# ilya16/isp-tts

Hardware: AMD Instinct MI355X
Metric: mel-frames/s (whole node), batch=64 x 512-frame utterances per GPU, full forward incl. MAS (higher is better)
Workload: dtype bf16; 1 GPU; BASELINE config 3: AcousticModel.forward (TextEncoder + Aligner/MAS + TemporalAdaptor 1 flow eval + MelDecoder + to_mel), fixed-length synthetic random-phoneme batch, random-init weights of the recipe architecture (23.2 M params); batch_per_gpu=64, global_batch=64, text_len=100, mel_len=512, parallelism=single GPU, device=gfx950:sramecc+:xnack-, compute_units=256, launch=HIP graph replay, batches_in_flight=1

## Files before the change

include/ispk.h:

```cpp
#ifndef ISPK_H
#define ISPK_H

#include <stdint.h>

#ifdef __cplusplus
extern "C" {
#endif

typedef struct ihipStream_t* ispk_stream_t;

#define ISPK_ABI_VERSION 2

#define ISPK_E_NULL (-1)
#define ISPK_E_SHAPE (-2)
#define ISPK_E_ALIGN (-3)
#define ISPK_E_UNSUPPORTED (-4)

int32_t ispk_abi_version(void);
const char* ispk_last_error_string(void);
int32_t ispk_device_info(char* name, int32_t cap);

int32_t ispk_mas_f32(const float* logits, const int64_t* text_len, const int64_t* mel_len, int16_t* attn_hard,
                     int64_t* dur, int16_t* path, int32_t B, int32_t M_max, int32_t L_max, int64_t stride_b,
                     int64_t stride_m, ispk_stream_t stream);

int32_t ispk_layernorm_f32(const float* x, int64_t ldx, const float* gamma, const float* beta, const float* ada_scale,
                           const float* ada_shift, int64_t ada_stride, int32_t rows_per_batch,
                           const uint8_t* row_mask, float* y, int64_t ldy, int32_t rows, int32_t D, float eps,
                           ispk_stream_t stream);
int32_t ispk_layernorm_f32_bf16(const float* x, int64_t ldx, const float* gamma, const float* beta,
                                const float* ada_scale, const float* ada_shift, int64_t ada_stride,
                                int32_t rows_per_batch, const uint8_t* row_mask, uint16_t* y, int64_t ldy, int32_t rows,
                                int32_t D, float eps, ispk_stream_t stream);

#define ISPK_EP_GELU 1u
#define ISPK_EP_SILU 2u
#define ISPK_EP_MASK_ACC 4u
#define ISPK_EP_MASK_OUT 8u
#define ISPK_EP_BIAS_ROW 16u
#define ISPK_EP_MASK_COL 32u
#define ISPK_EP_OUT_BF16 64u
#define ISPK_EP_RESID_BF16 128u
#define ISPK_EP_DUAL_GELU 1024u
#define ISPK_EP_GELU_BWD 2048u
#define ISPK_EP_OUT_SPLIT 512u
#define ISPK_EP_ROWS_T 256u

int32_t ispk_gemm_f32_tile(int32_t M, int32_t N, int32_t K);
int32_t ispk_gemm_f32(const float* A, int64_t lda, const float* W, int64_t ldw, float* C, int64_t ldc, const float* bias,
                      const float* resid, int64_t ldr, const uint8_t* mask, int32_t M, int32_t N, int32_t K,
                      uint32_t flags, int32_t cols_per_batch, int64_t batch_stride, ispk_stream_t stream);
int32_t ispk_gemm_f32_batched(const float* A, int64_t lda, int64_t stride_a, const float* W, int64_t ldw, int64_t stride_w,
                              float* C, int64_t ldc, int64_t stride_c, int32_t batch, int32_t M, int32_t N, int32_t K,
                              ispk_stream_t stream);
int32_t ispk_gemm_bf16_gelu_train(const uint16_t* A, int64_t lda, const uint16_t* W, int64_t ldw, uint16_t* u, int64_t ldu,
                                  uint16_t* a, int64_t ld_a, int32_t M, int32_t N, int32_t K, float dropout_p, uint64_t seed,
                                  ispk_stream_t stream);
int32_t ispk_gemm_bf16_gelu_bwd(const uint16_t* dY, int64_t lddy, const uint16_t* W2t, int64_t ldw, const uint16_t* u,
                                int64_t ldu, uint16_t* du, int64_t lddu, const uint8_t* row_mask, int32_t M, int32_t N,
                                int32_t K, float dropout_p, uint64_t seed, ispk_stream_t stream);
int32_t ispk_gemm_bf16_last_variant(void);
int32_t ispk_gemm_bf16(const uint16_t* A, int64_t lda, const uint16_t* W, int64_t ldw, void* C, int64_t ldc,
                       const float* bias, const void* resid, int64_t ldr, const uint8_t* mask, int32_t M, int32_t N,
                       int32_t K, uint32_t flags, int32_t cols_per_batch, int64_t batch_stride, ispk_stream_t stream);
int32_t ispk_gemm_bf16_splitk_plan(int32_t M, int32_t N, int32_t K, uint32_t flags);
int32_t ispk_gemm_bf16_splitk(const uint16_t* A, int64_t lda, const uint16_t* W, int64_t ldw, void* C, int64_t ldc,
                              const float* bias, const void* resid, int64_t ldr, const uint8_t* mask, int32_t M, int32_t N,
                              int32_t K, uint32_t flags, float* workspace, int32_t ksplit, ispk_stream_t stream);

int32_t ispk_ffn_bf16(const uint16_t* x, int64_t ldx, const uint16_t* W1, int64_t ldw1, const float* bias1,
                      const uint16_t* W2, int64_t ldw2, const float* bias2, const float* resid, int64_t ldr,
                      const uint8_t* mask, float* out, int64_t ldo, int32_t rows, int32_t dim, int32_t inner, uint32_t flags,
                      ispk_stream_t stream);

int32_t ispk_ffn_bf16_prenorm(const float* x, int64_t ldx, const float* norm_gamma, const float* norm_beta, float norm_eps,
                              const uint16_t* W1, int64_t ldw1, const uint16_t* W2_packed, const float* bias2,
                              const uint8_t* mask, float* out, int64_t ldo, int32_t rows, int32_t dim, int32_t inner,
                              uint32_t flags, float* row_stats, float stats_eps, ispk_stream_t stream);

int32_t ispk_ffn_chunk_w2_bf16(const uint16_t* W2, int64_t ldw2, int32_t dim, int32_t inner, uint16_t* out,
                               ispk_stream_t stream);
int32_t ispk_ffn_bf16_prenorm2_split(const float* x, int64_t ldx, const float* norm_gamma, const float* norm_beta,
                                     float norm_eps, const uint16_t* W1, const uint16_t* W2_chunks, float* parts,
                                     int64_t part_stride, int32_t splits, int32_t rows, int32_t dim, int32_t inner,
                                     ispk_stream_t stream);
int32_t ispk_ffn_combine_ln_f32(const float* x, int64_t ldx, const float* parts, int64_t part_stride, int32_t splits,
                                const uint8_t* mask, float* y, int64_t ldy, const float* ln_gamma, const float* ln_beta,
                                float ln_eps, int32_t ln_mask, void* ln_out, int64_t ld_ln, int32_t ln_bf16, int32_t rows,
                                int32_t dim, ispk_stream_t stream);
int32_t ispk_ffn_bf16_prenorm2(const float* x, int64_t ldx, const float* norm_gamma, const float* norm_beta, float norm_eps,
                               const uint16_t* W1, const uint16_t* W2_chunks, const uint8_t* mask, float* out, int64_t ldo,
                               int32_t rows, int32_t dim, int32_t inner, uint32_t flags, float* row_stats, float stats_eps,
                               ispk_stream_t stream);
int32_t ispk_attn_out_ffn_bf16(const float* x, int64_t ldx, const uint16_t* attn_out, int64_t ld_attn,
                               const uint16_t* Wo_chunks, const float* norm_gamma, const float* norm_beta, float norm_eps,
                               const uint16_t* W1, const uint16_t* W2_chunks, const uint8_t* mask, float* out, int64_t ldo,
                               int32_t rows, int32_t dim, int32_t inner, uint32_t flags, float* row_stats, float stats_eps,
                               ispk_stream_t stream);

int32_t ispk_attn_out_ffn_norm_bf16(const float* x, int64_t ldx, const uint16_t* attn_out, int64_t ld_attn,
                                    const uint16_t* Wo_chunks, const float* norm_gamma, const float* norm_beta, float norm_eps,
                                    const uint16_t* W1, const uint16_t* W2_chunks, const uint8_t* mask, float* out, int64_t ldo,
                                    int32_t rows, int32_t dim, int32_t inner, uint32_t flags, const float* final_gamma,
                                    const float* final_beta, float final_eps, int32_t ln_mask, void* ln_out, int64_t ld_ln,
                                    int32_t ln_bf16, ispk_stream_t stream);
int32_t ispk_attn_out_ffn_split_bf16(const float* x, int64_t ldx, const uint16_t* attn_out, int64_t ld_attn,
                                     const uint16_t* Wo_chunks, const float* norm_gamma, const float* norm_beta, float norm_eps,
                                     const uint16_t* W1, const uint16_t* W2_chunks, const uint8_t* mask, uint32_t flags,
                                     float* parts, int64_t part_stride, int32_t splits, int32_t rows, int32_t dim, int32_t inner,
                                     ispk_stream_t stream);
int32_t ispk_chunk_k16_bf16(const uint16_t* W, int64_t ldw, int32_t N, int32_t K, uint16_t* out, ispk_stream_t stream);
int32_t ispk_attn_out_ffn_qkv_bf16(const float* x, int64_t ldx, const uint16_t* attn_out, int64_t ld_attn,
                                   const uint16_t* Wo_chunks, const float* norm_gamma, const float* norm_beta, float norm_eps,
                                   const uint16_t* W1, const uint16_t* W2_chunks, const uint8_t* mask, float* out, int64_t ldo,
                                   int32_t rows, int32_t dim, int32_t inner, uint32_t flags, const float* next_gamma,
                                   const float* next_beta, float next_eps, const uint16_t* Wqkv_chunks, uint16_t* qkv,
                                   int64_t ld_qkv, ispk_stream_t stream);

int32_t ispk_gemm_bf16_lnin(const float* x, int64_t ldx, const float* row_stats, const float* ln_gamma, const float* ln_beta,
                            float ln_eps, const uint16_t* W, int64_t ldw, void* C, int64_t ldc, const float* bias, const void* resid,
                            int64_t ldr, const uint8_t* mask, int32_t M, int32_t N, int32_t K, uint32_t flags,
                            ispk_stream_t stream);

int32_t ispk_ffn_pack_w2_bf16(const uint16_t* W2, int64_t ldw2, int32_t dim, int32_t inner, uint16_t* packed,
                              ispk_stream_t stream);

int32_t ispk_linear_small_f32(const float* a, int64_t lda, const float* w, int64_t ldw, const float* bias,
                              const float* resid, int64_t ldr, float* out, int64_t ldo, int32_t M, int32_t N, int32_t K,
                              uint32_t act, ispk_stream_t stream);

int32_t ispk_alibi_mqa_attn_f32(const float* q, int64_t ldq, const float* k, const float* v, int64_t ldkv,
                                const float* slopes, const int64_t* key_len, float* out, int64_t ldo, int32_t B,
                                int32_t N, int32_t H, ispk_stream_t stream);
int32_t ispk_alibi_mqa_attn_bf16(const uint16_t* q, int64_t ldq, const uint16_t* k, const uint16_t* v, int64_t ldkv,
                                 const float* slopes, const int64_t* key_len, uint16_t* out, int64_t ldo, int32_t B,
                                 int32_t N, int32_t H, ispk_stream_t stream);
int32_t ispk_alibi_mqa_attn_bf16_tiles(const uint16_t* q, int64_t ldq, const uint16_t* k, const uint16_t* v, int64_t ldkv,
                                       const float* slopes, const int64_t* key_len, uint16_t* out, int64_t ldo, int32_t B,
                                       int32_t N, int32_t H, int32_t q_tiles_per_workgroup, ispk_stream_t stream);

int32_t ispk_attn_block_short_bf16(const uint16_t* x, int64_t ldx, const uint16_t* Wqkv_chunks, uint16_t* qkv, int64_t ld_qkv,
                                   const float* slopes, const int64_t* key_len, const uint16_t* Wo_chunks, const float* resid,
                                   int64_t ldr, const uint8_t* mask, float* out, int64_t ldo, int32_t B, int32_t N, int32_t H,
                                   ispk_stream_t stream);

int32_t ispk_pad_rows_f32(const float* x, int64_t stride_b, int64_t stride_t, int64_t stride_c, const int64_t* len,
                          void* out, int32_t out_bf16, int32_t B, int32_t T, int32_t C, ispk_stream_t stream);
int32_t ispk_masked_instnorm_f32(const float* y, const float* weight, const float* bias, const int64_t* len, void* out,
                                 int32_t out_bf16, int32_t B, int32_t T, int32_t C, float eps, ispk_stream_t stream);
int32_t ispk_aligner_scores_f32(const float* q_enc, int64_t q_stride_b, const float* k_enc, int64_t k_stride_b,
                                const int64_t* text_len, const int64_t* mel_len, float* attn_logits, float* attn_soft,
                                int32_t B, int32_t M, int32_t L, int32_t D, ispk_stream_t stream);
int32_t ispk_aligner_scores_fast_f32(const float* q_enc, int64_t q_stride_b, const float* k_enc, int64_t k_stride_b,
                                const int64_t* text_len, const int64_t* mel_len, float* attn_logits, float* attn_soft,
                                int32_t B, int32_t M, int32_t L, int32_t D, ispk_stream_t stream);
int32_t ispk_soft_average_f32(const float* attn_soft, const float* pitch, const float* energy, const int64_t* duration,
                              const int64_t* text_len, float* feats, int32_t B, int32_t M, int32_t L,
                              ispk_stream_t stream);

int32_t ispk_flow_head_f32(const float* y, int64_t ldy, const float* norm_gamma, const float* norm_beta, float norm_eps,
                           const float* W, const float* bias, const float* flow, const float* x0, const uint8_t* mask,
                           float* pred, float* duration, float* loss_ratio, float* loss_mean, float* workspace, int32_t B,
                           int32_t L, int32_t D, int32_t C, ispk_stream_t stream);
int32_t ispk_flow_euler_f32(const float* x_t, const float* velocity, float dt, const uint8_t* mask, float* out, int32_t B,
                            int32_t L, int32_t C, ispk_stream_t stream);
int32_t ispk_infer_features_f32(const float* pred, const float* duration_target_f32, const int64_t* duration_target_i64,
                                const float* pitch_target, const float* energy_target, float duration_factor, float pitch_factor,
                                float pitch_delta, float energy_factor, float energy_delta, float* duration, float* features,
                                int32_t B, int32_t L, ispk_stream_t stream);
int32_t ispk_infer_features_round_f32(const float* pred, const float* duration_target_f32, const int64_t* duration_target_i64,
                                      const float* pitch_target, const float* energy_target, float duration_factor,
                                      float pitch_factor, float pitch_delta, float energy_factor, float energy_delta,
                                      float* duration, float* features, int32_t B, int32_t L, ispk_stream_t stream);
int32_t ispk_infer_features_items_f32(const float* pred, const float* duration_target_f32, const int64_t* duration_target_i64,
                                      const float* pitch_target, const float* energy_target, const float* controls,
                                      int32_t round, float* duration, float* features, int64_t* frames_wanted, int32_t B,
                                      int32_t L, ispk_stream_t stream);
int32_t ispk_infer_features_tokens_f32(const float* pred, const float* duration_target_f32, const int64_t* duration_target_i64,
                                       const float* pitch_target, const float* energy_target, const float* controls,
                                       int32_t round, float* duration, float* features, int64_t* frames_wanted, int32_t B,
                                       int32_t L, ispk_stream_t stream);
int32_t ispk_flow_mix_f32(const float* x0, const float* x1, const float* t, float sigma, float* x_t, float* flow, int32_t B,
                          int32_t L, int32_t C, ispk_stream_t stream);
int32_t ispk_flow_finish_f32(const float* pred_raw, const float* flow, const float* x0, const uint8_t* mask, float* pred,
                             float* duration, float* loss_ratio, float* loss_mean, int32_t B, int32_t L, int32_t C,
                             ispk_stream_t stream);

int32_t ispk_embed_tokens_f32(const int64_t* text, const float* table, int64_t ld_table, int32_t vocab,
                              const int64_t* text_len, float* emb, uint8_t* mask, int32_t B, int32_t L, int32_t D,
                              ispk_stream_t stream);
int32_t ispk_embed_tokens_qkv(const int64_t* text, const float* table, int64_t ld_table, int32_t vocab, const int64_t* text_len,
                              float* emb, uint8_t* mask, const uint16_t* qkv_table, int64_t ld_qkv_table, uint16_t* qkv,
                              int32_t B, int32_t L, int32_t D, int32_t N, ispk_stream_t stream);
int32_t ispk_add_speaker_f32(float* x, const float* table, int64_t ld_table, int32_t speakers, const int64_t* speaker,
                             int32_t id_stride, int32_t B, int32_t L, int32_t D, ispk_stream_t stream);
int32_t ispk_add_speaker_out_f32(const float* x, float* out, const float* table, int64_t ld_table, int32_t speakers,
                                 const int64_t* speaker, int32_t id_stride, int32_t B, int32_t L, int32_t D, ispk_stream_t stream);
int32_t ispk_speaker_grad_f32(const float* d_x, const int64_t* speaker, int32_t id_stride, const int64_t* text_len,
                              float* workspace, int64_t workspace_floats, float* d_table, int64_t ld_table, int32_t speakers,
                              int32_t B, int32_t L, int32_t D, int32_t accumulate, ispk_stream_t stream);
int32_t ispk_time_embedding_f32(const float* t, int32_t n, const float* inv_freq, const float* freq_scale, int32_t half_dim,
                                const float* w0, const float* b0, const float* w1, const float* b1, int32_t emb_dim,
                                float* out, ispk_stream_t stream);
int32_t ispk_length_regulate_f32(const float* alignment, const float* dur_f32, const int64_t* dur_i64, const int64_t* enc_len,
                                 const float* x, int64_t ldx, float* out, int64_t* dec_len, uint8_t* dec_mask, int32_t B,
                                 int32_t M, int32_t L, int32_t D, int32_t max_len, int32_t dur_cols, ispk_stream_t stream);
int32_t ispk_length_regulate_split_bf16(const float* alignment, const float* dur_f32, const int64_t* dur_i64, const int64_t* enc_len,
                                 const float* x, int64_t ldx, float* out, int64_t* dec_len, uint8_t* dec_mask, int32_t B,
                                 int32_t M, int32_t L, int32_t D, int32_t max_len, int32_t dur_cols, ispk_stream_t stream);
int32_t ispk_length_regulate_qkv_bf16(const float* alignment, const float* dur_f32, const int64_t* dur_i64, const int64_t* enc_len,
                                      const float* x, int64_t ldx, float* out, int64_t* dec_len, uint8_t* dec_mask,
                                      const float* norm_gamma, const float* norm_beta, float norm_eps, const uint16_t* Wqkv_chunks,
                                      uint16_t* qkv, int64_t ld_qkv, int32_t B, int32_t M, int32_t L, int32_t D, int32_t max_len,
                                      int32_t dur_cols, ispk_stream_t stream);
int32_t ispk_length_regulate_split_f16(const float* alignment, const float* dur_f32, const int64_t* dur_i64, const int64_t* enc_len,
                                const float* x, int64_t ldx, float* out, int64_t* dec_len, uint8_t* dec_mask, int32_t B,
                                int32_t M, int32_t L, int32_t D, int32_t max_len, int32_t dur_cols, ispk_stream_t stream);

int32_t ispk_hard_regulate_f32(const float* dur_f32, const int64_t* dur_i64, const float* x, int64_t ldx, float* out,
                               int64_t* dec_len, uint8_t* dec_mask, int32_t B, int32_t frames, int32_t L, int32_t D,
                               int32_t max_len, ispk_stream_t stream);
int32_t ispk_hard_regulate_bwd_f32(const float* dur_f32, const int64_t* dur_i64, const float* d_out, float* d_x, int32_t B,
                                   int32_t rows, int32_t L, int32_t D, int32_t max_len, ispk_stream_t stream);
int32_t ispk_hard_average_f32(const float* pitch, const float* energy, const int64_t* duration, const int64_t* text_len,
                              float* feats, int32_t B, int32_t M, int32_t L, ispk_stream_t stream);

int32_t ispk_transpose_f32(const float* x, int64_t ldx, float* y, int64_t ldy, int32_t rows, int32_t cols,
                           ispk_stream_t stream);
int32_t ispk_gemm_tn_f32(const float* A, int64_t lda, const float* B, int64_t ldb, float* C, int64_t ldc, int32_t M,
                         int32_t N1, int32_t N2, const uint8_t* row_mask, int32_t accumulate, float* workspace,
                         int64_t workspace_floats, ispk_stream_t stream);
int32_t ispk_gemm_tn_bf16(const float* A, int64_t lda, const float* B, int64_t ldb, float* C, int64_t ldc, int32_t M,
                          int32_t N1, int32_t N2, const uint8_t* row_mask, int32_t accumulate, float* workspace,
                          int64_t workspace_floats, ispk_stream_t stream);
int32_t ispk_gemm_tn_b16(const uint16_t* A, int64_t lda, const uint16_t* B, int64_t ldb, float* C, int64_t ldc, int32_t M,
                         int32_t N1, int32_t N2, const uint8_t* row_mask, int32_t accumulate, float* workspace,
                         int64_t workspace_floats, ispk_stream_t stream);
int32_t ispk_gemm_tn_last_plan(int32_t* splits, int32_t* rows_per_split);
int32_t ispk_gemm_tn_batched_f32(const float* A, int64_t lda, int64_t stride_a, const float* B, int64_t ldb, int64_t stride_b,
                                 float* C, int64_t ldc, int64_t stride_c, int32_t batch, int32_t M, int32_t N1, int32_t N2,
                                 const uint8_t* row_mask, int32_t accumulate, float* workspace, int64_t workspace_floats,
                                 ispk_stream_t stream);
int32_t ispk_layernorm_bwd_f32(const float* x, int64_t ldx, const float* dy, int64_t lddy, const float* gamma,
                               const uint8_t* row_mask, float* dx, int64_t lddx, int32_t add_to_dx, float* dgamma,
                               float* dbeta, float* workspace, int64_t workspace_floats, int64_t rows, int32_t dim,
                               float eps, ispk_stream_t stream);
int32_t ispk_layernorm_bwd_dual_f32(const float* x, int64_t ldx, const float* dy, int64_t lddy, const float* gamma,
                                    const uint8_t* row_mask, float* dx, int64_t lddx, int32_t add_to_dx, float* dgamma,
                                    float* dbeta, float* workspace, int64_t workspace_floats, int64_t rows, int32_t dim,
                                    float eps, uint16_t* dx_bf16, int64_t ld_dx_bf16, ispk_stream_t stream);
int32_t ispk_gelu_f32(const float* u, float* a, int64_t n, float dropout_p, uint64_t seed, ispk_stream_t stream);
int32_t ispk_gelu_bwd_f32(const float* da, const float* u, float* du, int64_t n, float dropout_p, uint64_t seed,
                          ispk_stream_t stream);
int32_t ispk_gelu_f32_bf16(const float* u, uint16_t* a, int64_t n, float dropout_p, uint64_t seed, ispk_stream_t stream);
int32_t ispk_gelu_bwd_bf16(const uint16_t* da, const float* u, uint16_t* du, int64_t n, float dropout_p, uint64_t seed,
                           ispk_stream_t stream);
int32_t ispk_gelu_bf16(const uint16_t* u, uint16_t* a, int64_t n, float dropout_p, uint64_t seed, ispk_stream_t stream);
int32_t ispk_gelu_bwd_b16(const uint16_t* da, const uint16_t* u, uint16_t* du, int64_t n, float dropout_p, uint64_t seed,
                          ispk_stream_t stream);
int32_t ispk_dropout_mask_u8(uint8_t* out, int64_t n, float dropout_p, uint64_t seed, ispk_stream_t stream);
int32_t ispk_alibi_mqa_attn_train_f32(const float* qkv, int64_t ld_qkv, const float* slopes, const int64_t* key_len, float* o,
                                      int64_t ld_o, float* lse, int32_t B, int32_t N, int32_t H, float dropout_p, uint64_t seed,
                                      ispk_stream_t stream);
int32_t ispk_alibi_mqa_attn_bwd_f32(const float* qkv, int64_t ld_qkv, const float* o, const float* d_o, int64_t ld_o,
                                    const float* slopes, const int64_t* key_len, float* dqkv, float* dlogslopes,
                                    float* workspace, int64_t workspace_floats, int32_t B, int32_t N, int32_t H,
                                    const float* lse_in, float dropout_p, uint64_t seed, ispk_stream_t stream);
int32_t ispk_alibi_mqa_attn_train_bf16(const uint16_t* qkv, int64_t ld_qkv, const float* slopes, const int64_t* key_len,
                                       uint16_t* o, int64_t ld_o, float* lse, int32_t B, int32_t N, int32_t H, float dropout_p,
                                       uint64_t seed, ispk_stream_t stream);
int32_t ispk_alibi_mqa_attn_bwd_bf16(const uint16_t* qkv, int64_t ld_qkv, const uint16_t* o, const uint16_t* d_o, int64_t ld_o,
                                     const float* slopes, const int64_t* key_len, const float* lse, uint16_t* dqkv,
                                     float* dlogslopes, float* workspace, int64_t workspace_floats, int32_t B, int32_t N,
                                     int32_t H, float dropout_p, uint64_t seed, ispk_stream_t stream);
int32_t ispk_mel_loss_f32(const float* mel_out, const float* mel_target, const int64_t* mel_len, float* ratio, float* loss,
                          float* grad, float grad_out, int32_t B, int32_t C, int32_t T, ispk_stream_t stream);
int32_t ispk_acoustic_metrics_f32(const float* mel_out, int64_t out_sb, int64_t out_sc, int64_t out_st, const float* mel_target,
                                  int64_t tgt_sb, int64_t tgt_sc, int64_t tgt_st, const int64_t* mel_len, const int64_t* text_len,
                                  const float* attn_soft, int64_t attn_sb, int64_t attn_st, const float* dct, float* workspace,
                                  int64_t workspace_floats, float* out, int32_t B, int32_t C, int32_t T, int32_t L,
                                  int32_t n_mfcc, ispk_stream_t stream);
int32_t ispk_dtw_f32(const float* cost, int64_t cost_sb, int64_t cost_sn, const int64_t* n_len, const int64_t* m_len,
                     float* total, int32_t* steps, int16_t* path, float* workspace, int64_t workspace_floats, int32_t B,
                     int32_t N, int32_t M, ispk_stream_t stream);
int32_t ispk_mcd_dtw_f32(const float* mel_out, int64_t out_sb, int64_t out_sc, int64_t out_st, const float* mel_target,
                         int64_t tgt_sb, int64_t tgt_sc, int64_t tgt_st, const float* dct, const int64_t* n_len,
                         const int64_t* m_len, const float* pitch_out, int64_t pitch_out_sb, const float* pitch_target,
                         int64_t pitch_target_sb, float* workspace, int64_t workspace_floats, float* per_item, float* means,
                         float* cost_out, int32_t B, int32_t C, int32_t N, int32_t M, int32_t n_mfcc, ispk_stream_t stream);
int32_t ispk_audio_features_f32(const float* audio, int64_t ld_audio, const int64_t* audio_len, const float* tables,
                                int64_t table_floats, const int32_t* fb_index, int32_t n_mels, float* mel, int64_t* mel_len, float* pitch, float* energy,
                                int32_t B, int32_t S, int32_t M, int32_t tau_min, int32_t tau_max, float sample_rate,
                                float threshold, float pitch_mean, float pitch_std, ispk_stream_t stream);
int32_t ispk_resample_f32(const float* audio, int64_t ld_b, int64_t ld_c, const int64_t* audio_len, const float* taps,
                          int64_t tap_floats, const int32_t* first, float* out, int64_t ld_out, int64_t* out_len, int32_t B,
                          int32_t C, int32_t S, int32_t S_out, int32_t orig, int32_t dest, int32_t width, int32_t T,
                          ispk_stream_t stream);
int32_t ispk_feature_stats_f64(const float* pitch, int64_t ld_pitch, const float* energy, int64_t ld_energy,
                               const int64_t* mel_len, double* partial, double* state, int32_t B, int32_t M, int32_t reset,
                               ispk_stream_t stream);
int32_t ispk_audio_measure_f64(const float* audio, int64_t ld_audio, const int64_t* audio_len, const double* table,
                               int64_t table_doubles, int64_t* bounds, double* loudness, float* peak, float* gain,
                               float* workspace, int64_t workspace_floats, int32_t B, int32_t S, int32_t sample_rate,
                               int32_t trim_mode, double trim_threshold, int32_t pad_frames, int32_t gain_mode,
                               double target_lufs, double peak_limit, ispk_stream_t stream);
int32_t ispk_audio_apply_f32(const float* audio, int64_t ld_audio, const int64_t* bounds, const float* gain, float* out,
                             int64_t ld_out, int64_t* out_len, int32_t B, int32_t S, int32_t S_out, ispk_stream_t stream);
int32_t ispk_pcm16(const float* audio, int64_t ld_audio, const int64_t* audio_len, int16_t* out, int64_t ld_out, int32_t B,
                   int32_t S, int32_t dither, uint64_t seed, ispk_stream_t stream);
int32_t ispk_vocoder_unfold(const void* mel, int32_t mel_f16, int64_t sb, int64_t sc, int64_t st, const int64_t* mel_len,
                            void* rows, int32_t rows_bf16, int64_t ldr, uint8_t* row_mask, int32_t B, int32_t C, int32_t T,
                            int32_t K, ispk_stream_t stream);
int32_t ispk_dwconv7_ln_f32(const float* x, int64_t ldx, const float* w, const float* bias, const float* gamma,
                            const float* beta, float eps, const int64_t* mel_len, void* y, int32_t y_bf16, int64_t ldy,
                            int32_t B, int32_t T, int32_t D, ispk_stream_t stream);
int32_t ispk_istft_head_f32(const float* h, int64_t ldh, const int64_t* mel_len, const float* tables, int64_t table_floats,
                            float* audio, int64_t ld_audio, int64_t* audio_len, int32_t B, int32_t T, int32_t S,
                            ispk_stream_t stream);
int32_t ispk_aligner_scores_bwd_f32(const float* attn_logits, const float* attn_soft, const float* d_soft, const float* d_logits,
                                    const int64_t* text_len, const int64_t* mel_len, float* dS, int64_t ld_s, float* dSt,
                                    int64_t ld_t, int32_t B, int32_t M, int32_t L, float scale, ispk_stream_t stream);
int32_t ispk_masked_instnorm_bwd_f32(const float* y, const float* d_out, const float* weight, const int64_t* lengths, float* d_y,
                                     float* d_weight, float* d_bias, float* workspace, int64_t workspace_floats, int32_t B,
                                     int32_t T, int32_t C, float eps, ispk_stream_t stream);
int32_t ispk_soft_average_bwd_f32(const float* attn_soft, const float* pitch, const float* energy, const float* d_feats,
                                  const int64_t* text_len, float* workspace, int64_t workspace_floats, float* d_attn,
                                  int32_t accumulate, int32_t B, int32_t M, int32_t L, ispk_stream_t stream);
int32_t ispk_flow_loss_bwd_f32(const float* pred_raw, const float* flow, const uint8_t* mask, float grad_out, float* d_raw, int32_t B,
                               int32_t L, int32_t C, ispk_stream_t stream);
int32_t ispk_adaln_bwd_f32(const float* x, int64_t ldx, const float* dy, int64_t lddy, const float* scale, int64_t ld_scale,
                           const uint8_t* row_mask, float* dx, int64_t lddx, int32_t add_to_dx, float* dscale, float* dshift,
                           int64_t ld_out, int32_t B, int32_t rows_per_batch, int32_t dim, float eps, ispk_stream_t stream);
int32_t ispk_time_embedding_bwd_f32(const float* t, int32_t n, const float* inv_freq, const float* freq_scale, int32_t half_dim,
                                    const float* w0, const float* b0, const float* w1, int32_t emb_dim, const float* d_out,
                                    float* dw0, float* db0, float* dw1, float* db1, ispk_stream_t stream);
int32_t ispk_attn_ctc_loss_f32(const float* attn_logits, const int64_t* text_len, const int64_t* mel_len, float blank_logprob,
                               float* workspace, int64_t workspace_floats, float* loss, float* grad, float grad_out, int32_t B,
                               int32_t M, int32_t L, ispk_stream_t stream);
int32_t ispk_attn_bin_loss_f32(const float* attn_soft, const int16_t* attn_hard, float eps, float* workspace, float* loss,
                               float* grad, float grad_out, int32_t B, int32_t M, int32_t L, ispk_stream_t stream);
int32_t ispk_mel_grad_rows_f32(const float* dmel, const uint8_t* mask, float* g, int32_t B, int32_t C, int32_t T,
                               ispk_stream_t stream);
int32_t ispk_colsum_f32(const float* x, int64_t ldx, int64_t rows, int32_t cols, const uint8_t* row_mask, float* workspace,
                        int64_t workspace_floats, float* out, ispk_stream_t stream);
int32_t ispk_smallk_wgrad_f32(const float* g, int64_t ldg, const float* x, int64_t ldx, int64_t rows, int32_t N, int32_t K,
                              float* workspace, int64_t workspace_floats, float* out, ispk_stream_t stream);
int32_t ispk_embedding_bwd_f32(const int64_t* ids, const float* d_emb, int64_t rows, int32_t dim, int32_t vocab,
                               int32_t padding_idx, float* d_table, int64_t ld_table, ispk_stream_t stream);
int32_t ispk_grad_sqnorm_f32(const float* g, int64_t n, float* partial, float* out, ispk_stream_t stream);
int32_t ispk_adamw_f32(float* p, const float* g, float* m, float* v, int64_t n, int64_t n_decay, float lr, float beta1,
                       float beta2, float eps, float weight_decay, int32_t step, const float* grad_sqnorm, float max_norm,
                       float grad_scale, ispk_stream_t stream);

int32_t ispk_split_f16(const float* x, int64_t ldx, uint16_t* hi, uint16_t* lo, int64_t ldy, int32_t rows, int32_t cols,
                       ispk_stream_t stream);
int32_t ispk_gemm_split_f16_tile(int32_t M, int32_t N, int32_t K);
int32_t ispk_gemm_split_f16(const uint16_t* A, int64_t lda, int64_t a_plane, const uint16_t* W, int64_t ldw, int64_t w_plane,
                            void* C, int64_t ldc, int64_t c_plane, const float* bias, const float* resid, int64_t ldr,
                            const uint8_t* mask, int32_t M, int32_t N, int32_t K, uint32_t flags, int32_t cols_per_batch,
                            int64_t batch_stride, ispk_stream_t stream);
int32_t ispk_layernorm_f32_split(const float* x, int64_t ldx, const float* gamma, const float* beta, const float* ada_scale,
                                 const float* ada_shift, int64_t ada_stride, int32_t rows_per_batch, const uint8_t* row_mask,
                                 uint16_t* y_hi, int64_t ldy, int64_t y_plane, int32_t rows, int32_t D, float eps,
                                 ispk_stream_t stream);
int32_t ispk_alibi_mqa_attn_split_f16(const float* q, int64_t ldq, const float* k, const float* v, int64_t ldkv,
                                      const float* slopes, const int64_t* key_len, void* out, int64_t ldo, int64_t o_plane,
                                      int32_t B, int32_t N, int32_t H, ispk_stream_t stream);

int32_t ispk_cast_f32_bf16(const float* x, int64_t ldx, uint16_t* y, int64_t ldy, int32_t rows, int32_t cols,
                           ispk_stream_t stream);

typedef struct { float f[10]; } ispk_adam_args_t;
int32_t ispk_set_dropout_seed_source(const uint64_t* device_word);
int32_t ispk_adam_args_f32(float lr, float beta1, float beta2, float eps, float weight_decay, int32_t step, float max_norm,
                           float grad_scale, ispk_adam_args_t* out);
int32_t ispk_adamw_f32_dev(float* p, const float* g, float* m, float* v, int64_t n, int64_t n_decay,
                           const ispk_adam_args_t* args_dev, const float* grad_sqnorm, ispk_stream_t stream);

typedef struct { const float* src; void* dst; int32_t rows, cols; int64_t ld_dst; int32_t flags; } ispk_stage_t;
int32_t ispk_stage_weights(const ispk_stage_t* segs, int32_t nseg, ispk_stream_t stream);
typedef struct { const float* src; void* dst; int64_t n; int32_t mode; } ispk_segment_t;
int32_t ispk_segments_f32(const ispk_segment_t* segs, int32_t nseg, ispk_stream_t stream);
int32_t ispk_fill_zero(void* p, int64_t bytes, ispk_stream_t stream);
int32_t ispk_scale_f32(float* x, int64_t n, const float* s_dev, float s_host, ispk_stream_t stream);
int32_t ispk_sum_scalars_f32(const float* const* terms, const float* weights, int32_t n, float* out, ispk_stream_t stream);
int32_t ispk_exp_pad_f32(const float* src, float* dst, int32_t n, int32_t total, ispk_stream_t stream);
int32_t ispk_sqrt_scale_f32(const float* src, float* dst, int32_t n, float scale, ispk_stream_t stream);
int32_t ispk_copy2d_f32(const float* src, int64_t ld_src, float* dst, int64_t ld_dst, int32_t rows, int32_t cols,
                        ispk_stream_t stream);
int32_t ispk_permute021_f32(const float* src, float* dst, int32_t A, int32_t B, int32_t C, ispk_stream_t stream);
int32_t ispk_conv_weight_flip_f32(const float* w, float* wf, int32_t O, int32_t C, int32_t K, ispk_stream_t stream);

int32_t ispk_hifigan_tile_rows(void);
int32_t ispk_hifigan_conv_f32(const float* x, int64_t ldx, const float* w, const float* bias, const float* resid, int64_t ldr,
                              float* out, int64_t ldo, const int64_t* len, int32_t len_mul, int32_t B, int32_t T, int32_t C_in,
                              int32_t C_out, int32_t k, int32_t dilation, float slope, float scale, int32_t accumulate,
                              ispk_stream_t stream);
int32_t ispk_hifigan_conv_bf16(const float* x, int64_t ldx, const uint16_t* w, const float* bias, const float* resid,
                               int64_t ldr, float* out, int64_t ldo, const int64_t* len, int32_t len_mul, int32_t B, int32_t T,
                               int32_t C_in, int32_t C_out, int32_t k, int32_t dilation, float slope, float scale,
                               int32_t accumulate, ispk_stream_t stream);
int32_t ispk_hifigan_upsample_f32(const float* x, int64_t ldx, const float* w, const float* bias, float* out, int64_t ldo,
                                  const int64_t* len, int32_t len_mul, int32_t B, int32_t T, int32_t C_in, int32_t C_out,
                                  int32_t k, int32_t stride, float slope, ispk_stream_t stream);
int32_t ispk_hifigan_upsample_bf16(const float* x, int64_t ldx, const uint16_t* w, const float* bias, float* out, int64_t ldo,
                                   const int64_t* len, int32_t len_mul, int32_t B, int32_t T, int32_t C_in, int32_t C_out,
                                   int32_t k, int32_t stride, float slope, ispk_stream_t stream);
int32_t ispk_hifigan_post_f32(const float* x, int64_t ldx, const float* w, const float* bias, const int64_t* len,
                              int32_t len_mul, float* audio, int64_t ld_audio, int64_t* audio_len, int32_t B, int32_t T,
                              int32_t S, int32_t C, float slope, ispk_stream_t stream);
int32_t ispk_hifigan_post_clamp_f32(const float* x, int64_t ldx, const float* w, const float* bias, const int64_t* len,
                                    int32_t len_mul, float* audio, int64_t ld_audio, int64_t* audio_len, int32_t B, int32_t T,
                                    int32_t S, int32_t C, float slope, ispk_stream_t stream);

int32_t ispk_istftnet_tile_frames(void);
int32_t ispk_istftnet_head_f32(const float* x, int64_t ldx, const float* w, const float* bias, const float* table,
                               int32_t table_floats, const int64_t* len, int32_t len_mul, float* audio, int64_t ld_audio,
                               int64_t* audio_len, int32_t B, int32_t T, int32_t S, int32_t C, int32_t n_fft, int32_t hop,
                               float slope, float phase_scale, ispk_stream_t stream);

int32_t ispk_snake_aa_tile_rows(void);
int32_t ispk_snake_aa_f32(const float* x, int64_t ldx, const float* al, const float* inv_b, const float* taps, float* out,
                          int64_t ldo, const int64_t* len, int32_t len_mul, int32_t B, int32_t T, int32_t C,
                          ispk_stream_t stream);

int32_t ispk_denoise_tile_samples(void);
int32_t ispk_denoise_f32(const float* audio, int64_t ld_audio, const int64_t* audio_len, const float* tables,
                         const float* bias, const float* strength_item, float strength, float* out, int64_t ld_out, int32_t B,
                         int32_t S, ispk_stream_t stream);

int32_t ispk_join_tile_samples(void);
int32_t ispk_join_plan_bytes(void);
int32_t ispk_join_plan(const int64_t* audio_len, const int64_t* doc, const int64_t* pos, const int64_t* pause,
                       const int64_t* bounds, void* plan, int64_t plan_bytes, int64_t* item_offset, int64_t* item_len,
                       int64_t* doc_len, int64_t* wanted_len, int32_t B, int32_t S, int32_t D, int32_t S_out, int32_t fade,
                       ispk_stream_t stream);
int32_t ispk_join_f32(const float* audio, int64_t ld_audio, const float* gain, const void* plan, const int64_t* doc_len,
                      float* out, int64_t ld_out, int32_t B, int32_t S, int32_t D, int32_t S_out, ispk_stream_t stream);

int32_t ispk_speech_marks(const float* duration, int64_t ld_duration, const int64_t* text_len, const int64_t* audio_len,
                          const int64_t* bounds, const int64_t* item_offset, const int64_t* doc, const int64_t* doc_len,
                          const int64_t* doc_bounds, const int64_t* word_id, int64_t* token_marks, int64_t* word_marks,
                          int32_t hop, int32_t round, int32_t B, int32_t L, int32_t S, int32_t D, int32_t W,
                          ispk_stream_t stream);

int32_t ispk_gain_envelope_tile_samples(void);
int32_t ispk_gain_envelope_f32(const float* audio, int64_t ld_audio, const int64_t* audio_len, const int64_t* token_marks,
                               const float* token_gain, int32_t ramp, float* out, int64_t ld_out, int32_t B, int32_t L,
                               int32_t S, ispk_stream_t stream);

int32_t ispk_limit_tile_samples(void);
int32_t ispk_limit_f32(const float* audio, int64_t ld_audio, const int64_t* audio_len, const int64_t* bounds, const float* gain,
                       const float* taps, float ceiling, int32_t lookahead, float* out, int64_t ld_out, int64_t* out_len,
                       float* true_peak, float* reduction, int32_t B, int32_t S, ispk_stream_t stream);

int32_t ispk_equalize_segment_samples(void);
int32_t ispk_equalize_f32(const float* audio, int64_t ld_audio, const int64_t* audio_len, const double* table,
                          int64_t table_doubles, int32_t sections, float* out, int64_t ld_out, int64_t* out_len,
                          double* workspace, int64_t workspace_doubles, int32_t B, int32_t S, ispk_stream_t stream);

int32_t ispk_segment_workspace_bytes(int32_t B, int32_t S, int64_t* bytes);
int32_t ispk_segment_plan(const float* audio, int64_t ld_audio, const int64_t* audio_len, double factor, int32_t ref_mode,
                          double ref, int32_t pad, int32_t min_silence_frames, int64_t target_samples, int64_t max_samples,
                          int64_t min_samples, int64_t* segments, int32_t* flags, int32_t* count, int32_t* wanted,
                          int32_t* frames, int32_t* speech_frames, double* speech_power, double* noise_power, void* workspace,
                          int64_t workspace_bytes, int32_t B, int32_t S, int32_t K, ispk_stream_t stream);
int32_t ispk_segment_gather_f32(const float* audio, int64_t ld_audio, const int64_t* segments, const int32_t* flags,
                                const int32_t* count, int32_t drop, float* out, int64_t ld_out, int64_t* out_len, int32_t* item,
                                int32_t* index, int64_t* bounds, int32_t* row_flags, int32_t* rows, int32_t* rows_wanted,
                                int32_t B, int32_t S, int32_t K, int32_t R, int32_t S_out, ispk_stream_t stream);

int32_t ispk_screen_tile_samples(void);
int32_t ispk_screen_workspace_bytes(int32_t B, int32_t S, int64_t* bytes);
int32_t ispk_screen_f64(const float* audio, int64_t ld_audio, const int64_t* audio_len, const float* tables, int32_t parts,
                        int32_t rail_mode, float rail, float rail_ratio, int32_t min_run, int32_t min_dropout, double band_factor,
                        int32_t min_band_bin, double max_dc, double min_peak, int32_t* nonfinite, float* peak, double* dc,
                        double* power, int32_t* clip_runs, int64_t* clip_samples, int64_t* clip_longest, int64_t* clip_first,
                        int32_t* dropout_runs, int64_t* dropout_samples, int64_t* dropout_longest, double* ltas, int32_t* band_bin,
                        int32_t* flags, void* workspace, int64_t workspace_bytes, int32_t B, int32_t S, ispk_stream_t stream);

int32_t ispk_declip_max_unknowns(void);
int32_t ispk_declip_workspace_bytes(int32_t B, int32_t S, int64_t* bytes);
int32_t ispk_declip_f64(const float* audio, int64_t ld_audio, const int64_t* audio_len, const int32_t* in_flags, int32_t rail_mode,
                        float rail, float rail_ratio, int32_t min_run, int32_t order, int32_t iterations, float* out, int64_t ld_out,
                        int64_t* out_len, float* thr, float* peak, int64_t* clip_samples, int64_t* restored, int32_t* windows,
                        int32_t* dense, int32_t* flags, void* workspace, int64_t workspace_bytes, int32_t B, int32_t S,
                        ispk_stream_t stream);

int32_t ispk_noise_tile_samples(void);
int32_t ispk_noise_workspace_bytes(int32_t B, int32_t S, int64_t* bytes);
int32_t ispk_noise_profile_f64(const float* audio, int64_t ld_audio, const int64_t* audio_len, const float* tables, double factor,
                               int32_t ref_mode, double ref, int32_t guard, int32_t min_noise_frames, double* noise,
                               int32_t* noise_frames, int32_t* frames, int32_t* flags, void* workspace, int64_t workspace_bytes,
                               int32_t B, int32_t S, ispk_stream_t stream);
int32_t ispk_noise_reduce_f32(const float* audio, int64_t ld_audio, const int64_t* audio_len, const float* tables,
                              const double* noise, int32_t P, const int32_t* index, const int32_t* flags, double over,
                              double g_min, int32_t smooth_frames, int32_t smooth_bins, float* out, int64_t ld_out, int32_t B,
                              int32_t S, ispk_stream_t stream);

int32_t ispk_stretch_tile_samples(void);
int32_t ispk_stretch_workspace_bytes(int32_t B, int32_t S, int32_t out_samples, int64_t* bytes);
int32_t ispk_stretch_f32(const float* audio, int64_t ld_audio, const int64_t* audio_len, const float* tables, double rate,
                         const double* rates, float* out, int64_t ld_out, int32_t out_samples, int64_t* out_len, int64_t* wanted,
                         int32_t* flags, void* workspace, int64_t workspace_bytes, int32_t B, int32_t S, ispk_stream_t stream);

#define ISPK_PYIN_THRESHOLDS 100
#define ISPK_PYIN_MAX_BINS 1024
#define ISPK_PYIN_TABLE_DOUBLES 1326
int32_t ispk_pyin_frames_per_block(void);
int32_t ispk_pyin_workspace_bytes(int32_t B, int32_t M, int32_t NB, int64_t* bytes);
int32_t ispk_pyin_observe_f32(const float* audio, int64_t ld_audio, const int64_t* audio_len, const float* tables,
                              const double* prior, float* obs, int64_t* frames, int32_t B, int32_t S, int32_t M, int32_t NB,
                              int32_t min_period, int32_t max_period, double sample_rate, double f_min,
                              int32_t bins_per_semitone, ispk_stream_t stream);
int32_t ispk_pyin_decode_f64(const void* obs, int32_t obs_is_log, const int64_t* obs_len, const double* trans, int32_t width,
                             double f_min, int32_t bins_per_semitone, float pitch_mean, float pitch_std, int32_t* state,
                             float* f0, int32_t* voiced, float* voiced_prob, float* pitch, int64_t* frames, double* log_prob,
                             void* workspace, int64_t workspace_bytes, int32_t B, int32_t M, int32_t NB, ispk_stream_t stream);

#define ISPK_GRIFFINLIM_STEP 0
#define ISPK_GRIFFINLIM_INIT 1
int32_t ispk_griffinlim_tile_samples(void);
int32_t ispk_mel_to_linear_f32(const void* mel, int32_t mel_f16, int64_t mel_sb, int64_t mel_sc, int64_t mel_st,
                               const int64_t* mel_len, const float* pinv_t, float* mag, int64_t ld_mag, int32_t B,
                               int32_t n_mels, int32_t T, ispk_stream_t stream);
int32_t ispk_griffinlim_step_f32(const float* audio, int64_t ld_audio, const float* mag, int64_t ld_mag,
                                 const int64_t* mel_len, const float* tables, float* out, int64_t ld_out, int64_t* audio_len,
                                 int32_t B, int32_t T, int32_t mode, uint64_t seed, ispk_stream_t stream);
int32_t ispk_griffinlim_fast_step_f32(const float* audio, int64_t ld_audio, const float* prev, int64_t ld_prev, float alpha,
                                      const float* mag, int64_t ld_mag, const int64_t* mel_len, const float* tables,
                                      float* out, int64_t ld_out, int64_t* audio_len, int32_t B, int32_t T, ispk_stream_t stream);
int32_t ispk_griffinlim_error_f32(const float* audio, int64_t ld_audio, const float* mag, int64_t ld_mag,
                                  const int64_t* mel_len, const float* tables, float* work, int64_t ld_work, float* err,
                                  int32_t B, int32_t T, ispk_stream_t stream);

#ifdef __cplusplus
}
#endif
#endif
```

isp_tts_amd/acoustic/alignment.py:

```python
from __future__ import annotations

from collections.abc import Sequence
from typing import NamedTuple, Optional

import torch
import torch.nn as nn
from torch import Tensor

from .. import runtime
from ..staging import StagedWeights
from ..modules.aligner import mas_device
from ..modules.constructor import Constructor


_NOT_A_PATH = ("{} only owns parameters (the reference's state_dict names); its arithmetic runs inside the fused HIP "
               "kernels that ConvAttention launches (csrc/aligner.hip) - there is no PyTorch/MIOpen path to fall back to")


class MaskedInstanceNorm1d(nn.Module):

    def __init__(self, num_features: int, eps: float = 1e-5):
        super().__init__()
        self.eps = eps
        self.weight = nn.Parameter(torch.ones(num_features))
        self.bias = nn.Parameter(torch.zeros(num_features))

    def forward(self, *args, **kwargs):
        raise NotImplementedError(_NOT_A_PATH.format("MaskedInstanceNorm1d"))


class ConvBlock1D(nn.Module):

    def __init__(self, in_channels: int, out_channels: int, kernel_size: int = 1, activation: str = "relu",
                 normalization: Optional[str] = "batch", bias: bool = True):
        super().__init__()
        if normalization not in (None, "instance"):
            raise NotImplementedError("only instance normalisation (the recipes' choice) is built")
        if activation not in ("gelu", "linear"):
            raise NotImplementedError("only gelu / linear activations (the recipes' choice) are built")
        self.conv = nn.Conv1d(in_channels, out_channels, kernel_size=kernel_size, padding=(kernel_size - 1) // 2,
                              bias=bias and normalization is None)
        self.gelu = activation == "gelu"
        self.norm = MaskedInstanceNorm1d(out_channels) if normalization is not None else None

    def forward(self, *args, **kwargs):
        raise NotImplementedError(_NOT_A_PATH.format("ConvBlock1D"))


class ConvAttention(nn.Module, Constructor):
    def __init__(self, mel_dim: int, text_dim: int = 512, attention_dim: int = 80, key_kernel_size: int = 3,
                 query_kernel_size=(3, 3), dropout: float = 0.0, normalization: Optional[str] = "instance",
                 activation: str = "relu", attention_prior: bool = True):
        super().__init__()
        self.mel_dim, self.text_dim = mel_dim, text_dim
        self.scale = attention_dim ** -0.5
        if isinstance(query_kernel_size, int):
            query_kernel_size = [query_kernel_size] * 2
        self.key_proj = nn.ModuleList([
            ConvBlock1D(text_dim, text_dim * 2, key_kernel_size, activation, normalization, bias=False),
            ConvBlock1D(text_dim * 2, attention_dim, 1, "linear", None, bias=False)])
        self.query_proj = nn.ModuleList([
            ConvBlock1D(mel_dim, mel_dim * 2, query_kernel_size[0], activation, normalization, bias=False),
            ConvBlock1D(mel_dim * 2, mel_dim, query_kernel_size[1], activation, normalization, bias=False),
            ConvBlock1D(mel_dim, attention_dim, 1, "linear", None, bias=False)])
        self.attention_prior = attention_prior
        self.compute_dtype = torch.float32
        self._cache = StagedWeights()

    def _staged(self):
        ps = [c.conv.weight for c in list(self.key_proj) + list(self.query_proj)]
        dt = self.compute_dtype

        def build():
            if dt == torch.float16:
                w2d = [runtime.split_f16(p.detach().permute(0, 2, 1).reshape(p.shape[0], -1).float().contiguous()) for p in ps]
            else:
                w2d = [p.detach().permute(0, 2, 1).reshape(p.shape[0], -1).to(dt).contiguous() for p in ps]
            return w2d[:2], w2d[2:]
        return self._cache.get(dt, ps, build)

    def project_queries(self, queries: Tensor, query_len: Tensor) -> Tensor:
        _, wq = self._staged()
        gelu, dt = runtime.EP_GELU, self.compute_dtype
        if dt == torch.float16:
            q = runtime.pad_rows(queries.float(), query_len, channel_first=True, out_dtype=dt)
            for i in (0, 1):
                q = runtime.conv5_padded_split(q, wq[i], gelu)
                q = runtime.masked_instnorm(q, self.query_proj[i].norm.weight, self.query_proj[i].norm.bias, query_len,
                                            out_dtype=dt)
            return runtime.conv5_padded_split(q, wq[2])
        q = runtime.pad_rows(queries.float(), query_len, channel_first=True, out_dtype=dt)
        q = runtime.conv5_padded(q, wq[0], gelu)
        q = runtime.masked_instnorm(q, self.query_proj[0].norm.weight, self.query_proj[0].norm.bias, query_len,
                                    out_dtype=dt)
        q = runtime.conv5_padded(q, wq[1], gelu)
        q = runtime.masked_instnorm(q, self.query_proj[1].norm.weight, self.query_proj[1].norm.bias, query_len,
                                    out_dtype=dt)
        return runtime.conv5_padded(q, wq[2])

    def forward(self, queries: Tensor, keys: Tensor, query_len: Tensor, key_len: Tensor, q_proj: Optional[Tensor] = None):
        if not self.attention_prior:
            raise NotImplementedError("the aligner is built with its diagonal prior (recipes: attention_prior default)")
        wk, _ = self._staged()
        max_q, max_k = queries.shape[2], keys.shape[2]
        gelu, dt = runtime.EP_GELU, self.compute_dtype
        if dt == torch.float16:
            k = runtime.pad_rows(keys.float(), key_len, channel_first=True, out_dtype=dt)
            k = runtime.conv5_padded_split(k, wk[0], gelu)
            k = runtime.masked_instnorm(k, self.key_proj[0].norm.weight, self.key_proj[0].norm.bias, key_len, out_dtype=dt)
            k = runtime.conv5_padded_split(k, wk[1])
            q = q_proj if q_proj is not None else self.project_queries(queries, query_len)
            return runtime.aligner_scores(q, k, key_len, query_len, max_q, max_k)
        k = runtime.pad_rows(keys.float(), key_len, channel_first=True, out_dtype=dt)
        k = runtime.conv5_padded(k, wk[0], gelu)
        k = runtime.masked_instnorm(k, self.key_proj[0].norm.weight, self.key_proj[0].norm.bias, key_len, out_dtype=dt)
        k = runtime.conv5_padded(k, wk[1])
        q = q_proj if q_proj is not None else self.project_queries(queries, query_len)
        return runtime.aligner_scores(q, k, key_len, query_len, max_q, max_k, fast=dt == torch.bfloat16)


class AlignerOutput(NamedTuple):
    attn_soft: Tensor
    attn_logits: Tensor
    attn_hard: Tensor
    attn_hard_duration: Tensor


class Aligner(nn.Module, Constructor):
    def __init__(self, mel_dim: int, text_dim: int = 512, attention_dim: int = 80, key_kernel_size: int = 3,
                 query_kernel_size=(3, 3), dropout: float = 0.0, normalization: Optional[str] = "instance",
                 activation: str = "relu", attention_prior: bool = True):
        super().__init__()
        self.attention = ConvAttention(mel_dim=mel_dim, text_dim=text_dim, attention_dim=attention_dim,
                                       key_kernel_size=key_kernel_size, query_kernel_size=query_kernel_size,
                                       dropout=dropout, normalization=normalization, activation=activation,
                                       attention_prior=attention_prior)

    def forward(self, mel: Tensor, enc_text: Tensor, mel_len: Tensor, text_len: Tensor,
                q_proj: Optional[Tensor] = None, mas_stream=None) -> AlignerOutput:
        attn_soft, attn_logits = self.attention(mel, enc_text, mel_len, text_len, q_proj=q_proj)
        if mas_stream is not None and attn_logits.is_cuda:
            mas_stream.wait_stream(torch.cuda.current_stream())
            with torch.cuda.stream(mas_stream):
                attn_hard, dur = self.binarize_attention_parallel(attn_logits, text_len, mel_len, return_duration=True)
            attn_logits.record_stream(mas_stream)
        else:
            attn_hard, dur = self.binarize_attention_parallel(attn_logits, text_len, mel_len, return_duration=True)
        return AlignerOutput(attn_soft=attn_soft, attn_logits=attn_logits, attn_hard=attn_hard, attn_hard_duration=dur)

    @torch.no_grad()
    def binarize_attention_parallel(self, attn_logits: Tensor, text_len: Tensor, mel_len: Tensor,
                                    return_duration: bool = False):
        hard, dur, _ = mas_device(attn_logits.detach(), text_len, mel_len, want_dur=return_duration)
        return (hard, dur) if return_duration else hard
```

isp_tts_amd/acoustic/model.py:

```python
from __future__ import annotations

import warnings
from typing import NamedTuple, Optional

import torch
import torch.nn as nn
import torch.nn.functional as F
from torch import Tensor

from .. import runtime
from ..staging import StagedWeights
from ..modules.constructor import Constructor
from ..modules.transformer import Transformer
from ..modules.transformer.plan import Hand, Handed
from ..utils import get_mask_from_lengths
from .alignment import Aligner, AlignerOutput
from .temporal_adaptor import FlowTemporalAdaptor, TemporalAdaptorOutput


class AcousticModelOutput(NamedTuple):
    mel: Tensor
    adaptor_output: TemporalAdaptorOutput
    aligner_output: AlignerOutput
    loss: Optional[Tensor] = None
    losses: Optional[dict] = None


class AcousticModel(nn.Module, Constructor):
    def __init__(self, encoding_map: dict, mel_dim: int, text_dim: int = 384, encoder=None, decoder=None,
                 temporal_adaptor=None, aligner=None, num_speakers: Optional[int] = 0, pitch_mean=None, pitch_std=None,
                 speaker_in_forward: bool = False):
        super().__init__()
        self.encoding_map = dict(encoding_map)
        self.mel_dim, self.text_dim = mel_dim, text_dim
        self.text_embedding = nn.Embedding(len(encoding_map), text_dim, padding_idx=0)
        self.encoder = Transformer.init(encoder, emb_dim=text_dim)
        enc_dim = self.encoder.dim
        self.aligner = Aligner.init(aligner, mel_dim=mel_dim, text_dim=enc_dim)
        self.speaker_embedding = None
        if (num_speakers or 0) > 0:
            self.speaker_embedding = nn.Embedding(num_speakers, enc_dim)
            nn.init.xavier_uniform_(self.speaker_embedding.weight)
        self.speaker_in_forward = bool(speaker_in_forward)
        self.train_amp: Optional[bool] = None
        self.temporal_adaptor = FlowTemporalAdaptor.init(temporal_adaptor, encoder_dim=enc_dim)
        self.decoder = Transformer.init(decoder, emb_dim=enc_dim)
        self.to_mel = nn.Linear(self.decoder.dim, mel_dim)
        self.token_qkv_table = True
        self.overlap_streams = True
        self._side_streams: dict = {}
        self.register_buffer("pitch_mean", torch.tensor(float(pitch_mean or 0.)))
        self.register_buffer("pitch_std", torch.tensor(float(pitch_std or 1.)))
        self.compute_dtype = torch.float32
        self._cache = StagedWeights()

    def set_compute_dtype(self, dtype: torch.dtype, *, alignment_dtype: Optional[torch.dtype] = None):
        chain = alignment_dtype if alignment_dtype is not None else dtype
        assert chain in (torch.float32, torch.bfloat16, torch.float16)
        self.encoder.set_compute_dtype(chain)
        self.decoder.set_compute_dtype(dtype)
        self.temporal_adaptor.predictor.transformer.set_compute_dtype(dtype)
        self.temporal_adaptor.embedding.transformer.set_compute_dtype(dtype)
        self.aligner.attention.compute_dtype = chain
        self.temporal_adaptor.length_regulator.split_bf16 = (True if dtype == torch.bfloat16 else
                                                             "f16" if dtype == torch.float16 else False)
        self.compute_dtype = dtype
        return self

    def _to_mel(self, dec_out: Tensor, dec_mask: Optional[Tensor]) -> Tensor:
        w = self.to_mel.weight
        if dec_out.dtype == torch.float16:
            ws = self._cache.get(torch.float16, (w,), lambda: runtime.split_f16(w.detach().float().contiguous()))
            return runtime.to_mel_split(dec_out, ws, self.to_mel.bias, dec_mask)
        if dec_out.dtype == torch.bfloat16:
            w = self._cache.get(torch.bfloat16, (w,), lambda: w.detach().to(torch.bfloat16).contiguous())
        return runtime.to_mel(dec_out, w, self.to_mel.bias, dec_mask)

    def _embed(self, text: Tensor, text_len: Optional[Tensor], want_mask: bool = True):
        table, enc = self.text_embedding.weight, self.encoder
        first = enc.layers[0]
        norm, att = first.attention_norm, first.attention
        if not (self.token_qkv_table and text.is_cuda and att.compute_dtype == torch.bfloat16 and not first.adaptive_norm
                and norm.weight is not None and norm.bias is not None and isinstance(enc.project_emb, nn.Identity)
                and (att.heads * 64 + 128) % 8 == 0):
            return (*runtime.embed_tokens(text, table, text_len, want_mask=want_mask), Handed())

        def build():
            with torch.no_grad():
                rows = runtime.layernorm(table.detach().float().contiguous(), norm.weight, norm.bias, eps=norm.eps,
                                         out_dtype=torch.bfloat16)
                return runtime.gemm(rows, att._staged(torch.bfloat16)[0])
        qkv_table = self._cache.get("token_qkv", (table, norm.weight, norm.bias, att.to_q.weight, att.to_kv.weight), build)
        emb, mask, qkv = runtime.embed_tokens_qkv(text, table, qkv_table, text_len, want_mask=want_mask)
        return emb, mask, Handed(Hand.QKV, qkv)

    def _decoder_first(self):
        dec = self.decoder
        first = dec.layers[0]
        norm, att = first.attention_norm, first.attention
        ok = (att.compute_dtype == torch.bfloat16 and not first.adaptive_norm and norm.weight is not None and norm.bias is not None
              and isinstance(dec.project_emb, nn.Identity) and dec.dim == 384 and att.heads * 64 + 128 == 512)
        return first if ok else None

    def _decoder_handed(self) -> Handed:
        qkv = self.temporal_adaptor.length_regulator.qkv
        return Handed(Hand.QKV, qkv) if qkv is not None else Handed()

    def forward(self, text: Tensor, text_len: Tensor, mel: Tensor, mel_len: Tensor, pitch: Optional[Tensor] = None,
                energy: Optional[Tensor] = None, speaker: Optional[Tensor] = None, sigma: float = 0., steps: int = 1, *,
                flow_noise: Optional[Tensor] = None, flow_time: Optional[Tensor] = None) -> AcousticModelOutput:
        if self.speaker_embedding is None:
            speaker = None
        elif not self.speaker_in_forward:
            raise AttributeError(f"'{type(self).__name__}' object has no attribute 'speaker_encoder'")
        elif speaker is None:
            raise ValueError("speaker_in_forward is on and the model has a speaker table: forward() needs `speaker` "
                             "([B, 1] int64 ids, or a single id for the whole batch)")
        if torch.is_grad_enabled() and text.is_cuda and any(p.requires_grad for p in self.parameters()):
            from ..train.model import acoustic_train_outputs
            amp = self.train_amp if self.train_amp is not None else torch.is_autocast_enabled("cuda")
            train_aligner = any(p.requires_grad for p in self.aligner.parameters())
            with torch.autocast("cuda", enabled=False):
                return acoustic_train_outputs(self, text, text_len, mel, mel_len, pitch, energy, flow_noise, flow_time, amp=amp,
                                              train_aligner=train_aligner, speaker=speaker)
        with torch.no_grad():
            return self._forward_values(text, text_len, mel, mel_len, pitch, energy, flow_noise=flow_noise, flow_time=flow_time,
                                        speaker=speaker)

    def _forward_values(self, text: Tensor, text_len: Tensor, mel: Tensor, mel_len: Tensor, pitch: Optional[Tensor] = None,
                        energy: Optional[Tensor] = None, *, flow_noise: Optional[Tensor] = None,
                        flow_time: Optional[Tensor] = None, speaker: Optional[Tensor] = None) -> AcousticModelOutput:
        q_proj = None
        if mel.is_cuda and self.overlap_streams:
            main = torch.cuda.current_stream()
            side = self._side_streams.setdefault(mel.device, torch.cuda.Stream(device=mel.device))
            side.wait_stream(main)
            with torch.cuda.stream(side):
                q_proj = self.aligner.attention.project_queries(mel, mel_len)
        token_emb, enc_mask, handed = self._embed(text, text_len)
        enc_out = self.encoder(token_emb, mask=enc_mask, key_len=text_len, handed=handed).out
        if q_proj is not None:
            main.wait_stream(side)
            q_proj.record_stream(main)
        branch = side if q_proj is not None else None
        hard = not self.temporal_adaptor.soft_duration
        aligner_output = self.aligner(mel=mel, enc_text=enc_out.transpose(1, 2).detach(), mel_len=mel_len,
                                      text_len=text_len, q_proj=q_proj, mas_stream=None if hard else branch)
        if speaker is not None:
            enc_out = runtime.add_speaker(enc_out, self.speaker_embedding.weight, speaker)
        adaptor_output = self.temporal_adaptor(
            enc_out=enc_out, enc_mask=enc_mask, max_dec_len=mel.size(2),
            duration_target=aligner_output.attn_hard_duration, alignment=aligner_output.attn_soft,
            pitch_target_dense=pitch, energy_target_dense=energy, noise=flow_noise, time_steps=flow_time,
            enc_len=text_len, predictor_stream=branch, duration_sum=mel_len if branch is not None and not hard else None,
            qkv_for=self._decoder_first())
        dec_len = adaptor_output.dec_lengths
        dec_mask = adaptor_output.dec_mask
        dec_out = self.decoder(adaptor_output.enc_out, mask=dec_mask, key_len=dec_len, out_dtype=self.compute_dtype,
                               handed=self._decoder_handed()).out
        mel_out = self._to_mel(dec_out, dec_mask)
        if q_proj is not None:
            main.wait_stream(side)
            for t in (adaptor_output.log_duration, adaptor_output.duration, adaptor_output.pitch, adaptor_output.energy,
                      aligner_output.attn_hard, aligner_output.attn_hard_duration, *(adaptor_output.losses or {}).values()):
                if isinstance(t, Tensor):
                    t.record_stream(main)
        return AcousticModelOutput(mel=mel_out, adaptor_output=adaptor_output, aligner_output=aligner_output)

    @torch.no_grad()
    def forward_front(self, text: Tensor, text_len: Tensor, mel: Tensor, mel_len: Tensor, pitch: Tensor, energy: Tensor):
        main = torch.cuda.current_stream()
        side = self._side_streams.setdefault(mel.device, torch.cuda.Stream(device=mel.device))
        side.wait_stream(main)
        with torch.cuda.stream(side):
            q_proj = self.aligner.attention.project_queries(mel, mel_len)
        token_emb, enc_mask, handed = self._embed(text, text_len)
        enc_out = self.encoder(token_emb, mask=enc_mask, key_len=text_len, handed=handed).out
        main.wait_stream(side)
        q_proj.record_stream(main)
        attn_soft, attn_logits = self.aligner.attention(mel, enc_out.transpose(1, 2).detach(), mel_len, text_len,
                                                        q_proj=q_proj)
        feats = runtime.soft_average(attn_soft, pitch, energy, None, text_len)
        return {"enc_out": enc_out, "enc_mask": enc_mask, "attn_soft": attn_soft, "attn_logits": attn_logits, "feats": feats}

    @torch.no_grad()
    def forward_side(self, st: dict, text_len: Tensor, mel_len: Tensor, pitch: Tensor, energy: Tensor,
                     flow_noise: Optional[Tensor], flow_time: Optional[Tensor]):
        attn_hard, dur = self.aligner.binarize_attention_parallel(st["attn_logits"], text_len, mel_len, return_duration=True)
        ad = self.temporal_adaptor
        targets = runtime.soft_average(st["attn_soft"], pitch, energy, dur, text_len)
        pred, losses = ad.predictor(st["enc_out"], targets, st["enc_mask"][..., None], noise=flow_noise, time_steps=flow_time,
                                    key_len=text_len)
        return {"attn_hard": attn_hard, "dur": dur, "pred": pred, "losses": losses,
                "duration_pred": ad.predictor._duration_estimate}

    @torch.no_grad()
    def forward_back(self, st: dict, text_len: Tensor, mel_len: Tensor, max_dec_len: int):
        ad = self.temporal_adaptor
        feats = st["feats"]
        x = ad.embedding(feats[..., 1:3], mask=st["enc_mask"][..., None], key_len=text_len, residual=st["enc_out"])
        dec_in, dec_len = ad.length_regulator(x, mel_len.view(-1, 1), max_len=max_dec_len, alignment=st["attn_soft"],
                                              qkv_for=self._decoder_first())
        dec_mask = ad.length_regulator.dec_mask
        dec_out = self.decoder(dec_in, mask=dec_mask, key_len=dec_len, out_dtype=self.compute_dtype,
                               handed=self._decoder_handed()).out
        return {"mel": self._to_mel(dec_out, dec_mask), "dec_in": dec_in, "dec_len": dec_len, "dec_mask": dec_mask}

    @staticmethod
    def assemble_output(front: dict, side: dict, back: dict) -> AcousticModelOutput:
        feats, pred = front["feats"], side["pred"]
        adaptor = TemporalAdaptorOutput(enc_out=back["dec_in"], log_duration=pred[..., 0], duration=side["duration_pred"],
                                        dec_lengths=back["dec_len"], pitch=pred[..., 1], energy=pred[..., 2],
                                        pitch_target=feats[..., 1], energy_target=feats[..., 2], losses=side["losses"],
                                        dec_mask=back["dec_mask"])
        aligner = AlignerOutput(attn_soft=front["attn_soft"], attn_logits=front["attn_logits"], attn_hard=side["attn_hard"],
                                attn_hard_duration=side["dur"])
        return AcousticModelOutput(mel=back["mel"], adaptor_output=adaptor, aligner_output=aligner)

    @torch.no_grad()
    def infer(self, input_sequence: Tensor, text_lengths: Optional[Tensor] = None,
              duration_target: Optional[Tensor] = None, duration_factor: float = 1.0,
              pitch_target: Optional[Tensor] = None, pitch_factor: float = 1.0, pitch_delta: float = 0.,
              pitch_normalize: bool = False, energy_target: Optional[Tensor] = None, steps: int = 4,
              speaker: Optional[Tensor] = None, *, flow_noise: Optional[Tensor] = None,
              max_dec_len: Optional[int] = None, controls: Optional[Tensor] = None):
        if controls is not None and (duration_factor, pitch_factor, pitch_delta) != (1.0, 1.0, 0.0):
            raise ValueError("infer: with `controls` the scalar controls stay at their defaults, got duration_factor="
                             f"{duration_factor}, pitch_factor={pitch_factor}, pitch_delta={pitch_delta}")
        if controls is not None and controls.ndim == 3:
            B, L = input_sequence.shape
            if controls.dtype != torch.float32 or tuple(controls.shape) != (B, L, 5):
                raise ValueError(f"controls: fp32 [{B}, {L}, 5], got {controls.dtype} {tuple(controls.shape)}")
        batch_infer = input_sequence.shape[0] > 1
        token_emb, enc_mask, handed = self._embed(input_sequence, text_lengths if batch_infer else None, want_mask=batch_infer)
        enc_out = self.encoder(token_emb, mask=enc_mask, key_len=text_lengths if batch_infer else None, handed=handed).out
        if self.speaker_embedding is not None and speaker is not None:
            enc_out = runtime.add_speaker_(enc_out, self.speaker_embedding.weight, speaker)
        if pitch_normalize:
            if pitch_target is not None:
                pitch_target = (pitch_target - self.pitch_mean) / self.pitch_std
            pitch_delta = pitch_delta / self.pitch_std
        adaptor_output = self.temporal_adaptor.infer(
            enc_out=enc_out, enc_mask=enc_mask, duration_target=duration_target, pitch_target=pitch_target,
            energy_target=energy_target, duration_factor=duration_factor, pitch_factor=pitch_factor,
            pitch_delta=pitch_delta, steps=steps, noise=flow_noise, max_dec_len=max_dec_len,
            enc_len=text_lengths if batch_infer else None, qkv_for=self._decoder_first(),
            **({} if controls is None else {"controls": controls}))
        dec_mask = adaptor_output.dec_mask if batch_infer else None
        dec_out = self.decoder(adaptor_output.enc_out, mask=dec_mask, key_len=adaptor_output.dec_lengths if batch_infer else None,
                               out_dtype=self.compute_dtype, handed=self._decoder_handed()).out
        return self._to_mel(dec_out, dec_mask), adaptor_output

    @classmethod
    def from_pretrained(cls, checkpoint_path: str, strict: bool = True) -> "AcousticModel":
        checkpoint = torch.load(checkpoint_path, map_location="cpu", weights_only=False)
        model = cls.init(checkpoint["model"]["config"])
        state_dict = dict(checkpoint["model"]["state_dict"])
        for key, weight in model.state_dict().items():
            if key not in state_dict:
                state_dict[key] = weight
        model.load_state_dict(state_dict, strict=strict)
        return model

    def load(self, state_dict: dict, ignore_layers: Optional[list] = None, ignore_mismatched_keys: bool = False):
        own = self.state_dict()
        extra = [k for k in state_dict if k not in own]
        if extra:
            warnings.warn(f"checkpoint keys absent from the model are ignored: {extra}")
        kept = {k: v for k, v in state_dict.items() if k in own}
        ignored = []
        if ignore_mismatched_keys:
            ignored += [k for k, v in kept.items() if v.shape != own[k].shape]
        if ignore_layers:
            ignored += [k for k in kept if any(layer in k for layer in ignore_layers)]
        kept = {k: v for k, v in kept.items() if k not in ignored}
        own.update(kept)
        self.load_state_dict(own)
        return self

    def freeze(self, exception_list: Optional[list] = None):
        exception_list = exception_list or []
        for name, param in self.named_parameters():
            param.requires_grad = any(name.startswith(layer) for layer in exception_list)
        return self

    def extend_speakers(self, count: int) -> int:
        if self.speaker_embedding is None:
            raise ValueError("extend_speakers: the model has no speaker table (num_speakers = 0)")
        if count < 1:
            raise ValueError(f"extend_speakers: count = {count}")
        old = self.speaker_embedding.weight
        first = old.shape[0]
        table = nn.Embedding(first + count, old.shape[1], device=old.device, dtype=old.dtype)
        with torch.no_grad():
            table.weight[:first] = old
            table.weight[first:] = old.double().mean(dim=0).to(old.dtype)
        table.weight.requires_grad_(old.requires_grad)
        self.speaker_embedding = table
        return first

    def prepare_inputs(self, inputs: dict) -> dict:
        return {"text": inputs["text_vector"], "text_len": inputs["text_vector_len"], "mel": inputs["mel"],
                "mel_len": inputs["mel_len"], "pitch": inputs["pitch"], "energy": inputs["energy"],
                "speaker": inputs.get("speaker")}
```

isp_tts_amd/acoustic/temporal_adaptor.py:

```python
from __future__ import annotations

from typing import NamedTuple, Optional

import torch
import torch.nn as nn
import torch.nn.functional as F
from torch import Tensor

from .. import runtime
from ..staging import StagedWeights
from ..modules.constructor import Constructor
from ..modules.transformer import Transformer, TimePositionalEmbedding
from ..utils import get_float_mask_from_lengths, get_mask_3d, masked_mean


class TransformerTemporalModule(nn.Module, Constructor):

    def __init__(self, input_dim: int = 256, output_dim: int = 256, transformer=None, detach_inputs: bool = False):
        super().__init__()
        self.transformer = Transformer.init(transformer, emb_dim=input_dim)
        for layer in self.transformer.layers:
            layer.attention.short_block = False
        self.linear_layer = nn.Linear(self.transformer.dim, output_dim, bias=True)
        self.detach_inputs = detach_inputs
        self._cache = StagedWeights()

    def _weight(self, dtype: torch.dtype) -> Tensor:
        w = self.linear_layer.weight
        if dtype == torch.float16:
            return self._cache.get(dtype, (w,), lambda: runtime.split_f16(w.detach().float().contiguous()))
        return self._cache.get(dtype, (w,), lambda: w.detach().to(dtype).contiguous())

    def forward(self, x: Tensor, mask: Optional[Tensor] = None, *, key_len: Optional[Tensor] = None,
                residual: Optional[Tensor] = None) -> Tensor:
        m2 = mask[..., 0] if mask is not None else None
        cdt = self.transformer.layers[0].attention.compute_dtype
        out = self.transformer(x, mask=m2, out_dtype=cdt, key_len=key_len if m2 is not None else None).out
        flags = runtime.EP_MASK_ACC if m2 is not None else 0
        if cdt == torch.float16:
            return runtime.gemm_split(out, self._weight(cdt), bias=self.linear_layer.bias, mask=m2, flags=flags, resid=residual)
        return runtime.gemm(out, self._weight(cdt), bias=self.linear_layer.bias, mask=m2, flags=flags, resid=residual,
                            out_dtype=torch.float32)

    def infer(self, x: Tensor, mask: Optional[Tensor] = None, steps: int = 4) -> Tensor:
        return self.forward(x, mask)


class FlowTransformerTemporalModule(nn.Module, Constructor):

    def __init__(self, input_dim: int = 256, output_dim: int = 256, transformer=None,
                 time_embedding_dim: Optional[int] = None, sigma: float = 1e-5, detach_inputs: bool = False):
        super().__init__()
        time_embedding_dim = time_embedding_dim or input_dim
        self.time_embedding = TimePositionalEmbedding(freq_dim=64, emb_dim=time_embedding_dim, with_steps=True)
        self.transformer = Transformer.init(transformer, emb_dim=output_dim + input_dim, adaptive_norm=True,
                                            condition_dim=time_embedding_dim)
        self.linear_layer = nn.Linear(self.transformer.dim, output_dim, bias=True)
        self.output_dim, self.sigma, self.detach_inputs = output_dim, sigma, detach_inputs
        self.fused_head = True
        self._cache = StagedWeights()
        self._grids: dict = {}

    def _cond_weight(self, dtype: torch.dtype) -> Tensor:
        w = self.transformer.project_emb.weight
        if dtype == torch.float16:
            return self._cache.get(dtype, (w,), lambda: runtime.split_f16(w.detach()[:, self.output_dim:].float().contiguous()))
        return self._cache.get(dtype, (w,), lambda: w.detach()[:, self.output_dim:].to(dtype).contiguous())

    def _project(self, x_t: Tensor, cond_proj: Tensor) -> Tensor:
        w = self.transformer.project_emb.weight
        return runtime.linear_small(x_t.contiguous(), w[:, :self.output_dim], None, resid=cond_proj)

    def _cond_projection(self, cond: Tensor) -> Tensor:
        cdt = self.transformer.layers[0].attention.compute_dtype
        c = cond.float().contiguous()
        if cdt == torch.float16:
            return runtime.gemm_split(runtime.split_f16(c), self._cond_weight(cdt), bias=self.transformer.project_emb.bias)
        if cdt == torch.bfloat16:
            c = runtime.cast_bf16(c)
        return runtime.gemm(c, self._cond_weight(cdt), bias=self.transformer.project_emb.bias, out_dtype=torch.float32)

    def forward(self, x: Tensor, targets: Tensor, mask: Optional[Tensor] = None, *, noise: Optional[Tensor] = None,
                time_steps: Optional[Tensor] = None, key_len: Optional[Tensor] = None):
        cond = x
        have_mask = mask is not None
        if mask is None:
            mask = torch.ones(x.shape[:2], dtype=torch.bool, device=x.device)
        elif mask.ndim == 3:
            mask = mask[..., 0]
        x1 = targets.detach()
        x0 = torch.randn_like(x1) if noise is None else noise.to(x1)
        t = torch.rand((x1.shape[0],), dtype=x1.dtype, device=x1.device) if time_steps is None else time_steps.to(x1)
        time_emb = self.time_embedding(t)
        x_t, flow = runtime.flow_mix(x0, x1, t, self.sigma)
        proj = self._project(x_t, self._cond_projection(cond))
        tr = self.transformer
        head = (self.fused_head and tr.dim == 256 and self.output_dim == 3 and tr.norm.weight is not None and tr.norm.bias is not None
                and self.linear_layer.bias is not None)
        out = tr(None, mask=mask, adaptive_condition=time_emb, projected=proj, key_len=key_len if have_mask else None,
                 final_norm=not head).out
        if head:
            pred, self._duration_estimate, _, loss = runtime.flow_head(out, tr.norm.weight, tr.norm.bias, tr.norm.eps,
                                                                       self.linear_layer.weight, self.linear_layer.bias, flow, x0, mask)
            return pred, {"flow_loss": loss}
        raw = runtime.linear_small(out, self.linear_layer.weight, self.linear_layer.bias)
        pred, self._duration_estimate, _, loss = runtime.flow_finish(raw, flow, x0, mask)
        return pred, {"flow_loss": loss}

    def euler_grid(self, steps: int, step_factor: float, device=None) -> Tensor:
        assert step_factor <= 1.
        key = (int(steps), float(step_factor))
        grid = self._grids.get(key)
        if grid is None:
            if step_factor == 1.:
                grid = torch.linspace(0, 1, steps + 1)
            else:
                ts = -torch.diff(torch.logspace(0, steps, steps + 1, base=step_factor))
                ts = torch.cat([torch.zeros(1), ts])
                grid = torch.cumsum(ts / ts.sum(), dim=0)
            self._grids[key] = grid
        return grid if device is None else grid.to(device)

    def infer(self, x: Tensor, mask: Optional[Tensor] = None, steps: int = 4, step_factor: float = 0.75, *,
              noise: Optional[Tensor] = None, key_len: Optional[Tensor] = None) -> Tensor:
        dev = x.device
        if mask is not None and mask.ndim == 3:
            mask = mask.squeeze(-1)
        x_t = (torch.randn(x.shape[0], x.shape[1], self.output_dim, device=dev) if noise is None
               else noise.to(device=dev, dtype=torch.float32))
        dts = self._grids.get(("dt", int(steps), float(step_factor)))
        if dts is None:
            ts = self.euler_grid(steps, step_factor)
            dts = self._grids[("dt", int(steps), float(step_factor))] = (ts[1:] - ts[:-1]).tolist()
        temb = self.time_embedding(self._grid_on(dev, steps, step_factor)[:steps])
        cond_proj = self._cond_projection(x)
        if mask is not None and key_len is None:
            key_len = mask.sum(dim=1)
        for i in range(steps):
            out = self.transformer(None, mask=mask, adaptive_condition=temb[i].view(1, 1, -1),
                                   projected=self._project(x_t, cond_proj), key_len=key_len).out
            vel = runtime.linear_small(out, self.linear_layer.weight, self.linear_layer.bias)
            x_t = runtime.flow_euler(x_t, vel, dts[i], mask if i == steps - 1 else None)
        return x_t

    def _grid_on(self, device, steps: int, step_factor: float) -> Tensor:
        key = (str(device), int(steps), float(step_factor))
        g = self._grids.get(key)
        if g is None:
            g = self._grids[key] = self.euler_grid(steps, step_factor).to(device)
        return g


class TemporalAdaptorOutput(NamedTuple):
    enc_out: Tensor
    log_duration: Optional[Tensor]
    duration: Tensor
    dec_lengths: Tensor
    pitch: Optional[Tensor]
    energy: Optional[Tensor]
    pitch_target: Optional[Tensor]
    energy_target: Optional[Tensor]
    losses: Optional[dict] = None
    dec_mask: Optional[Tensor] = None


class LengthRegulator(nn.Module):
    split_bf16 = False
    hand_qkv = True
    qkv: Optional[Tensor] = None

    def forward(self, x: Tensor, durations: Tensor, max_len: Optional[int] = None, alignment: Optional[Tensor] = None, *,
                enc_len: Optional[Tensor] = None, frames: Optional[int] = None, hard: bool = False, qkv_for=None):
        self.qkv = None
        if alignment is None and (hard or frames is None or durations.dtype == torch.int64):
            if frames is None:
                frames = int((durations.float() + 0.5).long().sum(dim=1).max().item())
            if max_len is not None:
                frames = min(frames, max_len)
            if frames == 0:
                self.dec_mask = torch.zeros((x.shape[0], 0), dtype=torch.bool, device=x.device)
                return x.new_zeros((x.shape[0], 0, x.shape[2])), torch.zeros((x.shape[0],), dtype=torch.int64, device=x.device)
            out, dec_lens, self.dec_mask = runtime.hard_regulate(x.float(), durations, frames,
                                                                 max_len=-1 if max_len is None else max_len)
            return out, dec_lens
        rows = alignment.shape[1] if alignment is not None else frames
        if max_len is not None and alignment is not None:
            rows = min(rows, max_len)
            alignment = alignment[:, :rows]
        if self.hand_qkv and qkv_for is not None and self.split_bf16 is True and x.is_cuda and x.shape[-1] == 384:
            norm, att = qkv_for.attention_norm, qkv_for.attention
            out, dec_lens, self.dec_mask, self.qkv = runtime.length_regulate(
                x.float(), durations, alignment, rows, max_len=-1 if max_len is None else max_len, enc_len=enc_len,
                split_bf16=True, next_qkv=(norm.weight, norm.bias, norm.eps, att._chunked_wqkv()))
            return out, dec_lens
        out, dec_lens, self.dec_mask = runtime.length_regulate(x.float(), durations, alignment, rows,
                                                               max_len=-1 if max_len is None else max_len, enc_len=enc_len,
                                                               split_bf16=self.split_bf16)
        return out, dec_lens


class TemporalAverager(nn.Module):

    def forward(self, x: Tensor, durations: Tensor, alignment: Optional[Tensor] = None) -> Tensor:
        if alignment is None:
            b, c, _ = x.shape
            if durations.dtype != torch.int64:
                ends = torch.cumsum(durations, dim=1).long()
                durations = torch.diff(ends, dim=1, prepend=torch.zeros_like(ends[:, :1]))
            every = torch.full((b,), durations.shape[1], dtype=torch.int64, device=x.device)
            cols = []
            for i in range(0, c, 2):
                f = runtime.hard_average(x[:, i], x[:, min(i + 1, c - 1)], durations, every)
                cols.append(f[..., 1:min(3, 1 + c - i)])
            return torch.cat(cols, dim=-1).transpose(1, 2)
        return x @ alignment / (alignment.sum(dim=1, keepdim=True) + 1e-5)


def generate_soft_path(duration: Tensor, mask: Tensor) -> Tensor:
    b, t_x, t_y = mask.shape
    cum = torch.cumsum(duration, 1).view(b * t_x)
    path = get_float_mask_from_lengths(cum, t_y).to(mask.dtype).view(b, t_x, t_y)
    path = path - F.pad(path, [0, 0, 1, 0, 0, 0])[:, :-1]
    return path * mask


class FlowTemporalAdaptor(nn.Module, Constructor):
    predictor_first = False

    def __init__(self, encoder_dim: int = 384, predictor=None, embedding=None, pitch: bool = True, energy: bool = True,
                 soft_duration: bool = False):
        super().__init__()
        if not (pitch and energy):
            raise NotImplementedError("built with pitch and energy both on (either duration mode): without one of them the "
                                      "feature tensors change shape")
        self.length_regulator = LengthRegulator()
        self.averager = TemporalAverager()
        self.encoder_dim = encoder_dim
        self.feature_dim = 3
        self.pitch, self.energy, self.soft_duration = pitch, energy, soft_duration
        self.pitch_idx, self.energy_idx = 1, 2
        self.predictor = FlowTransformerTemporalModule.init(predictor, input_dim=encoder_dim, output_dim=self.feature_dim)
        self.embedding = TransformerTemporalModule.init(embedding, input_dim=self.feature_dim - 1, output_dim=encoder_dim)

    def _process_target(self, dense: Tensor, duration_target: Tensor, alignment: Tensor, enc_mask: Tensor) -> Tensor:
        if dense.ndim == 2:
            dense = dense[:, None]
        return self.averager(dense, duration_target, alignment).transpose(1, 2) * enc_mask

    def forward(self, enc_out: Tensor, enc_mask: Tensor, max_dec_len: int, duration_target: Optional[Tensor] = None,
                alignment: Optional[Tensor] = None, pitch_target_dense: Optional[Tensor] = None,
                energy_target_dense: Optional[Tensor] = None, *, noise: Optional[Tensor] = None,
                time_steps: Optional[Tensor] = None, enc_len: Optional[Tensor] = None,
                predictor_stream=None, duration_sum: Optional[Tensor] = None, qkv_for=None) -> TemporalAdaptorOutput:
        assert duration_target is not None and (alignment is not None or not self.soft_duration)
        assert pitch_target_dense is not None and energy_target_dense is not None
        hard = not self.soft_duration
        m3 = enc_mask[..., None]
        if enc_len is None:
            enc_len = enc_mask.sum(dim=1)
        side = predictor_stream if (predictor_stream is not None and enc_out.is_cuda) else None
        cond = enc_out
        if hard:
            alignment = None
            targets = runtime.hard_average(pitch_target_dense, energy_target_dense, duration_target, enc_len)
            feats = targets
            len_src = duration_target
        elif side is None or duration_sum is None:
            targets = runtime.soft_average(alignment, pitch_target_dense, energy_target_dense, duration_target, enc_len)
            feats = targets
            len_src = duration_target
        else:
            feats = runtime.soft_average(alignment, pitch_target_dense, energy_target_dense, None, enc_len)
            targets = None
            len_src = duration_sum.view(-1, 1)
        if side is not None:
            ready = torch.cuda.Event()
            ready.record()
        pitch_target, energy_target = feats[..., 1:2], feats[..., 2:3]
        features = feats[..., 1:3]

        def decoder_input(enc_out_):
            enc_out_ = self.embedding(features, mask=m3, key_len=enc_len, residual=enc_out_)
            return self.length_regulator(enc_out_, len_src, max_len=max_dec_len, alignment=alignment,
                                         frames=max_dec_len if hard else None, qkv_for=qkv_for)

        if not (side is not None and self.predictor_first):
            enc_out, dec_lens = decoder_input(enc_out)

        def predict():
            tg = targets
            if tg is None:
                tg = runtime.soft_average(alignment, pitch_target_dense, energy_target_dense, duration_target, enc_len)
            pred_, losses_ = self.predictor(cond, tg, m3, noise=noise, time_steps=time_steps, key_len=enc_len)
            return pred_, losses_, self.predictor._duration_estimate

        if side is not None:
            side.wait_event(ready)
            with torch.cuda.stream(side):
                pred, losses, duration_pred = predict()
            for t in (cond, feats, alignment, pitch_target_dense, energy_target_dense):
                if t is not None:
                    t.record_stream(side)
            if self.predictor_first:
                enc_out, dec_lens = decoder_input(enc_out)
        else:
            pred, losses, duration_pred = predict()
        log_duration_pred = pred[..., 0]
        return TemporalAdaptorOutput(enc_out=enc_out, log_duration=log_duration_pred, duration=duration_pred,
                                     dec_lengths=dec_lens, pitch=pred[..., 1], energy=pred[..., 2],
                                     pitch_target=pitch_target.squeeze(-1), energy_target=energy_target.squeeze(-1),
                                     losses=losses, dec_mask=self.length_regulator.dec_mask)

    def infer(self, enc_out: Tensor, enc_mask: Optional[Tensor] = None, duration_target: Optional[Tensor] = None,
              duration_factor: float = 1.0, pitch_target: Optional[Tensor] = None, pitch_factor: float = 1.0,
              pitch_delta: float = 0., energy_target: Optional[Tensor] = None, energy_factor: float = 1.0,
              energy_delta: float = 0., steps: int = 4, *, noise: Optional[Tensor] = None,
              max_dec_len: Optional[int] = None, enc_len: Optional[Tensor] = None, qkv_for=None,
              controls: Optional[Tensor] = None) -> TemporalAdaptorOutput:
        if controls is not None:
            return self._infer_items(enc_out, enc_mask, duration_target, pitch_target, energy_target, controls, steps, noise,
                                     max_dec_len, enc_len, qkv_for,
                                     (duration_factor, pitch_factor, pitch_delta, energy_factor, energy_delta))
        m3 = enc_mask[..., None] if enc_mask is not None else None
        pred = self.predictor.infer(enc_out, mask=m3, steps=steps, noise=noise, key_len=enc_len)
        duration_pred, feats = runtime.infer_features(pred, duration_target, pitch_target, energy_target, duration_factor,
                                                      pitch_factor, pitch_delta, energy_factor, energy_delta,
                                                      round_duration=not self.soft_duration)
        pitch, energy = feats[..., 0:1], feats[..., 1:2]
        enc_out = self.embedding(feats, residual=enc_out)
        enc_lens = enc_len
        if enc_lens is None and enc_mask is not None:
            enc_lens = enc_mask.sum(dim=1)
        if not self.soft_duration:
            enc_out, dec_lens = self.length_regulator(enc_out, duration_pred, alignment=None, frames=max_dec_len, hard=True)
            return TemporalAdaptorOutput(enc_out=enc_out, log_duration=None, duration=duration_pred, dec_lengths=dec_lens,
                                         pitch=pitch.squeeze(-1), energy=energy.squeeze(-1), pitch_target=pitch_target,
                                         energy_target=energy_target, dec_mask=self.length_regulator.dec_mask)
        if max_dec_len is None:
            max_dec_len = int((duration_pred.sum(dim=1) + 0.5).long().max().item())
        enc_out, dec_lens = self.length_regulator(enc_out, duration_pred, alignment=None, enc_len=enc_lens,
                                                  frames=max_dec_len, qkv_for=qkv_for)
        return TemporalAdaptorOutput(enc_out=enc_out, log_duration=None, duration=duration_pred, dec_lengths=dec_lens,
                                     pitch=pitch.squeeze(-1), energy=energy.squeeze(-1), pitch_target=pitch_target,
                                     energy_target=energy_target, dec_mask=self.length_regulator.dec_mask)

    frames_wanted: Optional[Tensor] = None

    def _infer_items(self, enc_out, enc_mask, duration_target, pitch_target, energy_target, controls, steps, noise, max_dec_len,
                     enc_len, qkv_for, scalars) -> TemporalAdaptorOutput:
        if tuple(float(v) for v in scalars) != (1.0, 1.0, 0.0, 1.0, 0.0):
            raise ValueError("infer: with `controls` the scalar controls stay at their defaults (duration_factor, pitch_factor, "
                             f"pitch_delta, energy_factor, energy_delta = 1, 1, 0, 1, 0), got {tuple(scalars)}")
        per_token = controls.ndim == 3
        if per_token:
            B, L = enc_out.shape[:2]
            if controls.dtype != torch.float32 or tuple(controls.shape) != (B, L, 5):
                raise ValueError(f"controls: fp32 [{B}, {L}, 5], got {controls.dtype} {tuple(controls.shape)}")
        elif controls.dtype != torch.float32 or tuple(controls.shape) != (enc_out.shape[0], 5):
            raise ValueError(f"controls: fp32 [{enc_out.shape[0]}, 5], got {controls.dtype} {tuple(controls.shape)}")
        m3 = enc_mask[..., None] if enc_mask is not None else None
        pred = self.predictor.infer(enc_out, mask=m3, steps=steps, noise=noise, key_len=enc_len)
        entry = runtime.infer_features_tokens if per_token else runtime.infer_features_items
        duration_pred, feats, self.frames_wanted = entry(
            pred, duration_target, pitch_target, energy_target, controls, round_duration=not self.soft_duration)
        pitch, energy = feats[..., 0:1], feats[..., 1:2]
        enc_out = self.embedding(feats, residual=enc_out)
        enc_lens = enc_len
        if enc_lens is None and enc_mask is not None:
            enc_lens = enc_mask.sum(dim=1)
        if not self.soft_duration:
            enc_out, dec_lens = self.length_regulator(enc_out, duration_pred, max_len=max_dec_len, alignment=None,
                                                      frames=max_dec_len, hard=True)
        else:
            if max_dec_len is None:
                max_dec_len = int(self.frames_wanted.max().item())
            enc_out, dec_lens = self.length_regulator(enc_out, duration_pred, max_len=max_dec_len, alignment=None,
                                                      enc_len=enc_lens, frames=max_dec_len, qkv_for=qkv_for)
        return TemporalAdaptorOutput(enc_out=enc_out, log_duration=None, duration=duration_pred, dec_lengths=dec_lens,
                                     pitch=pitch.squeeze(-1), energy=energy.squeeze(-1), pitch_target=pitch_target,
                                     energy_target=energy_target, dec_mask=self.length_regulator.dec_mask)
```

isp_tts_amd/bindings/adaptor.py:

```python
from typing import Optional

import torch
from torch import Tensor

from .. import runtime as _rt

__all__ = ["mas", "pad_rows", "conv5_padded", "masked_instnorm", "aligner_scores", "soft_average", "flow_mix", "flow_finish",
           "flow_head", "flow_euler", "infer_features", "infer_features_items", "infer_features_tokens", "embed_tokens", "embed_tokens_qkv", "_speaker_ids", "add_speaker_",
           "add_speaker", "speaker_grad", "time_embedding", "length_regulate", "_hard_durations", "hard_regulate",
           "hard_regulate_bwd", "hard_average"]


def mas(logits: Tensor, text_len: Tensor, mel_len: Tensor, want_dur: bool = True, want_path: bool = False):
    _rt._dev(logits, text_len, mel_len)
    assert logits.dtype == torch.float32 and logits.ndim == 3
    if logits.stride(2) != 1:
        logits = logits.contiguous()
    B, M, L = logits.shape
    text_len = _rt._i64(text_len)
    mel_len = _rt._i64(mel_len)
    hard = torch.empty((B, M, L), dtype=torch.int16, device=logits.device)
    dur = torch.empty((B, L), dtype=torch.int64, device=logits.device) if want_dur else None
    path = torch.empty((B, M), dtype=torch.int16, device=logits.device) if want_path else None
    _rt._launch(f"mas_kernel<{(L + 63) // 64}>", 0.0, 6.0 * B * M * L, _rt.lib().ispk_mas_f32, logits.data_ptr(),
                text_len.data_ptr(), mel_len.data_ptr(), hard.data_ptr(), _rt._ptr(dur), _rt._ptr(path), B, M, L, logits.stride(0),
                logits.stride(1), _rt._stream())
    return hard, dur, path


def pad_rows(x: Tensor, lengths: Tensor, channel_first: bool = False, out_dtype: torch.dtype = torch.float32) -> Tensor:
    _rt._dev(x, lengths)
    assert x.dtype == torch.float32 and x.ndim == 3
    if channel_first:
        B, C, T = x.shape
        sb, sc, st = x.stride()
    else:
        B, T, C = x.shape
        sb, st, sc = x.stride()
    lengths = _rt._i64(lengths)
    split = out_dtype == torch.float16
    out = torch.empty((2, B, T + 4, C) if split else (B, T + 4, C), dtype=out_dtype, device=x.device)
    _rt._launch("pad_rows_kernel", 0.0, 8.0 * B * T * C, _rt.lib().ispk_pad_rows_f32, x.data_ptr(), sb, st, sc,
                lengths.data_ptr(), out.data_ptr(), 2 if split else int(out_dtype == torch.bfloat16), B, T, C, _rt._stream())
    return out


def conv5_padded(xpad: Tensor, w2d: Tensor, flags: int = 0) -> Tensor:
    _rt._dev(xpad, w2d)
    B, TP, C = xpad.shape
    O, K = w2d.shape
    taps = K // C
    assert taps * C == K and taps in (1, 5) and xpad.is_contiguous() and w2d.is_contiguous()
    assert xpad.dtype == w2d.dtype
    bf16 = xpad.dtype == torch.bfloat16
    out = torch.empty((B, TP, O), dtype=torch.float32, device=xpad.device)
    a_ptr = xpad.data_ptr() + (0 if taps == 5 else 2 * C * xpad.element_size())
    M = B * TP - 4
    fn = _rt.lib().ispk_gemm_bf16 if bf16 else _rt.lib().ispk_gemm_f32
    _rt._launch(_rt._gemm_label(bf16, M, O, K), 2.0 * M * O * K, float(xpad.element_size()) * (M * C + O * K) + 4.0 * M * O, fn,
                a_ptr, C, w2d.data_ptr(), K, out.data_ptr(), O, None, None, 0, None, M, O, K, flags, 0, 0, _rt._stream())
    return out


def masked_instnorm(y: Tensor, weight: Tensor, bias: Tensor, lengths: Tensor, eps: float = 1e-5,
                    out_dtype: torch.dtype = torch.float32) -> Tensor:
    _rt._dev(y, weight, bias, lengths)
    B, TP, C = y.shape
    split = out_dtype == torch.float16
    out = torch.empty((2, *y.shape) if split else y.shape, dtype=out_dtype, device=y.device)
    lengths = _rt._i64(lengths)
    _rt._launch("masked_instnorm_kernel", 0.0, 16.0 * B * TP * C, _rt.lib().ispk_masked_instnorm_f32, y.data_ptr(),
                weight.data_ptr(), bias.data_ptr(), lengths.data_ptr(), out.data_ptr(), 2 if split else int(out_dtype == torch.bfloat16), B,
                TP - 4, C, eps, _rt._stream())
    return out


def aligner_scores(q_enc: Tensor, k_enc: Tensor, text_len: Tensor, mel_len: Tensor, M: int, L: int, fast: bool = False):
    _rt._dev(q_enc, k_enc, text_len, mel_len)
    B, D = q_enc.shape[0], q_enc.shape[2]
    logits = torch.empty((B, M, L), dtype=torch.float32, device=q_enc.device)
    soft = torch.empty((B, M, L), dtype=torch.float32, device=q_enc.device)
    text_len = _rt._i64(text_len)
    mel_len = _rt._i64(mel_len)
    _rt._launch("aligner_scores_kernel<bf16x3>" if fast else "aligner_scores_kernel", 2.0 * B * M * L * D, 4.0 * B * (M * D + L * D + 2 * M * L),
                _rt.lib().ispk_aligner_scores_fast_f32 if fast else _rt.lib().ispk_aligner_scores_f32, q_enc.data_ptr(), q_enc.stride(0),
                k_enc.data_ptr(), k_enc.stride(0), text_len.data_ptr(), mel_len.data_ptr(), logits.data_ptr(), soft.data_ptr(), B, M, L, D,
                _rt._stream())
    return soft, logits


def soft_average(attn_soft: Tensor, pitch: Tensor, energy: Tensor, duration: Optional[Tensor], text_len: Tensor) -> Tensor:
    _rt._dev(attn_soft, pitch, energy, duration, text_len)
    B, M, L = attn_soft.shape
    feats = torch.empty((B, L, 3), dtype=torch.float32, device=attn_soft.device)
    dur = _rt._i64(duration)
    if B == 0:
        return feats
    _rt._launch("soft_average_kernel", 0.0, 4.0 * B * M * L, _rt.lib().ispk_soft_average_f32, attn_soft.contiguous().data_ptr(),
                pitch.contiguous().data_ptr(), energy.contiguous().data_ptr(), _rt._ptr(dur),
                _rt._i64(text_len).data_ptr(), feats.data_ptr(), B, M, L, _rt._stream())
    return feats


def flow_mix(x0: Tensor, x1: Tensor, t: Tensor, sigma: float):
    _rt._dev(x0, x1, t)
    B, L, C = x1.shape
    x0c, x1c, tc = x0.float().contiguous(), x1.float().contiguous(), t.float().contiguous()
    xt, flow = torch.empty_like(x1c), torch.empty_like(x1c)
    if B == 0:
        return xt, flow
    _rt._launch("flow_mix_kernel", 0.0, 16.0 * B * L * C, _rt.lib().ispk_flow_mix_f32, x0c.data_ptr(), x1c.data_ptr(), tc.data_ptr(),
                float(sigma), xt.data_ptr(), flow.data_ptr(), B, L, C, _rt._stream())
    return xt, flow


def flow_finish(pred_raw: Tensor, flow: Tensor, x0: Tensor, mask: Tensor):
    _rt._dev(pred_raw, flow, x0, mask)
    B, L, C = pred_raw.shape
    assert mask.dtype == torch.bool and mask.shape == (B, L)
    pr, fl, x0c, mk = pred_raw.float().contiguous(), flow.contiguous(), x0.float().contiguous(), mask.contiguous()
    pred = torch.empty_like(pr)
    dur = torch.empty((B, L), dtype=torch.float32, device=pr.device)
    ratio = torch.empty((B,), dtype=torch.float32, device=pr.device)
    loss = torch.empty((), dtype=torch.float32, device=pr.device)
    if B == 0:
        return pred, dur, ratio, loss.fill_(float("nan"))
    _rt._launch("flow_finish_kernel", 0.0, 20.0 * B * L * C, _rt.lib().ispk_flow_finish_f32, pr.data_ptr(), fl.data_ptr(),
                x0c.data_ptr(), mk.data_ptr(), pred.data_ptr(), dur.data_ptr(), ratio.data_ptr(), loss.data_ptr(), B, L, C,
                _rt._stream())
    return pred, dur, ratio, loss


def flow_head(y: Tensor, norm_weight: Tensor, norm_bias: Tensor, norm_eps: float, weight: Tensor, bias: Tensor, flow: Tensor,
              x0: Tensor, mask: Tensor):
    _rt._dev(y, norm_weight, norm_bias, weight, bias, flow, x0, mask)
    B, L, D = y.shape
    C = weight.shape[0]
    assert y.dtype == torch.float32 and y.stride(2) == 1 and y.stride(0) == L * y.stride(1) and weight.shape == (C, D) and weight.is_contiguous()
    assert mask.dtype == torch.bool and mask.shape == (B, L)
    fl, x0c, mk = flow.contiguous(), x0.float().contiguous(), mask.contiguous()
    pred = torch.empty((B, L, C), dtype=torch.float32, device=y.device)
    dur = torch.empty((B, L), dtype=torch.float32, device=y.device)
    ratio = torch.empty((B,), dtype=torch.float32, device=y.device)
    loss = torch.empty((), dtype=torch.float32, device=y.device)
    if B == 0:
        return pred, dur, ratio, loss.fill_(float("nan"))
    ws = torch.empty((2 * B * ((L + 15) // 16),), dtype=torch.float32, device=y.device)
    _rt._launch("flow_head_kernels", 0.0, 4.0 * B * L * D, _rt.lib().ispk_flow_head_f32, y.data_ptr(), y.stride(1), norm_weight.data_ptr(),
                norm_bias.data_ptr(), float(norm_eps), weight.data_ptr(), bias.data_ptr(), fl.data_ptr(), x0c.data_ptr(), mk.data_ptr(),
                pred.data_ptr(), dur.data_ptr(), ratio.data_ptr(), loss.data_ptr(), ws.data_ptr(), B, L, D, C, _rt._stream())
    return pred, dur, ratio, loss


def flow_euler(x_t: Tensor, velocity: Tensor, dt: float, mask: Optional[Tensor] = None) -> Tensor:
    _rt._dev(x_t, velocity, mask)
    B, L, C = x_t.shape
    xc, vc = x_t.float().contiguous(), velocity.float().contiguous()
    out = torch.empty_like(xc)
    if mask is not None:
        mask = mask.contiguous()
        assert mask.dtype == torch.bool and mask.shape == (B, L)
    if B == 0:
        return out
    _rt._launch("flow_euler_kernel", 0.0, 12.0 * B * L * C, _rt.lib().ispk_flow_euler_f32, xc.data_ptr(), vc.data_ptr(), float(dt),
                _rt._ptr(mask), out.data_ptr(), B, L, C, _rt._stream())
    return out


def infer_features(pred: Tensor, duration_target: Optional[Tensor], pitch_target: Optional[Tensor],
                   energy_target: Optional[Tensor], duration_factor: float = 1.0, pitch_factor: float = 1.0,
                   pitch_delta: float = 0.0, energy_factor: float = 1.0, energy_delta: float = 0.0, round_duration: bool = False):
    _rt._dev(pred, duration_target, pitch_target, energy_target)
    B, L, C = pred.shape
    assert C == 3 and pred.dtype == torch.float32
    pc = pred.contiguous()
    dur_f = dur_i = None
    if duration_target is not None:
        assert duration_target.shape == (B, L)
        if duration_target.dtype == torch.int64:
            dur_i = duration_target.contiguous()
        else:
            dur_f = duration_target.float().contiguous()
    pt = None if pitch_target is None else pitch_target.float().reshape(B, L).contiguous()
    et = None if energy_target is None else energy_target.float().reshape(B, L).contiguous()
    duration = torch.empty((B, L), dtype=torch.float32, device=pred.device)
    feats = torch.empty((B, L, 2), dtype=torch.float32, device=pred.device)
    if B == 0:
        return duration, feats
    _rt._launch("infer_features_kernel<round>" if round_duration else "infer_features_kernel", 0.0, 24.0 * B * L,
                _rt.lib().ispk_infer_features_round_f32 if round_duration else _rt.lib().ispk_infer_features_f32, pc.data_ptr(), _rt._ptr(dur_f),
                _rt._ptr(dur_i), _rt._ptr(pt), _rt._ptr(et), float(duration_factor), float(pitch_factor), float(pitch_delta), float(energy_factor),
                float(energy_delta), duration.data_ptr(), feats.data_ptr(), B, L, _rt._stream())
    return duration, feats


def infer_features_items(pred: Tensor, duration_target: Optional[Tensor], pitch_target: Optional[Tensor],
                         energy_target: Optional[Tensor], controls: Tensor, round_duration: bool = False,
                         want_frames: bool = True):
    _rt._dev(pred, duration_target, pitch_target, energy_target, controls)
    B, L, C = pred.shape
    assert C == 3 and pred.dtype == torch.float32
    if controls.dtype != torch.float32 or tuple(controls.shape) != (B, 5):
        raise ValueError(f"controls: fp32 [{B}, 5], got {controls.dtype} {tuple(controls.shape)}")
    pc, cc = pred.contiguous(), controls.contiguous()
    dur_f = dur_i = None
    if duration_target is not None:
        assert duration_target.shape == (B, L)
        if duration_target.dtype == torch.int64:
            dur_i = duration_target.contiguous()
        else:
            dur_f = duration_target.float().contiguous()
    pt = None if pitch_target is None else pitch_target.float().reshape(B, L).contiguous()
    et = None if energy_target is None else energy_target.float().reshape(B, L).contiguous()
    duration = torch.empty((B, L), dtype=torch.float32, device=pred.device)
    feats = torch.empty((B, L, 2), dtype=torch.float32, device=pred.device)
    frames = torch.empty((B,), dtype=torch.int64, device=pred.device) if want_frames else None
    if B == 0:
        return duration, feats, frames
    _rt._launch("infer_features_items_kernel<round>" if round_duration else "infer_features_items_kernel", 0.0, 24.0 * B * L,
                _rt.lib().ispk_infer_features_items_f32, pc.data_ptr(), _rt._ptr(dur_f), _rt._ptr(dur_i), _rt._ptr(pt), _rt._ptr(et),
                cc.data_ptr(), int(bool(round_duration)), duration.data_ptr(), feats.data_ptr(), _rt._ptr(frames), B, L, _rt._stream())
    return duration, feats, frames


def infer_features_tokens(pred: Tensor, duration_target: Optional[Tensor], pitch_target: Optional[Tensor],
                          energy_target: Optional[Tensor], controls: Tensor, round_duration: bool = False,
                          want_frames: bool = True):
    _rt._dev(pred, duration_target, pitch_target, energy_target, controls)
    B, L, C = pred.shape
    assert C == 3 and pred.dtype == torch.float32
    if controls.dtype != torch.float32 or tuple(controls.shape) != (B, L, 5):
        raise ValueError(f"controls: fp32 [{B}, {L}, 5], got {controls.dtype} {tuple(controls.shape)}")
    pc, cc = pred.contiguous(), controls.contiguous()
    dur_f = dur_i = None
    if duration_target is not None:
        assert duration_target.shape == (B, L)
        if duration_target.dtype == torch.int64:
            dur_i = duration_target.contiguous()
        else:
            dur_f = duration_target.float().contiguous()
    pt = None if pitch_target is None else pitch_target.float().reshape(B, L).contiguous()
    et = None if energy_target is None else energy_target.float().reshape(B, L).contiguous()
    duration = torch.empty((B, L), dtype=torch.float32, device=pred.device)
    feats = torch.empty((B, L, 2), dtype=torch.float32, device=pred.device)
    frames = torch.empty((B,), dtype=torch.int64, device=pred.device) if want_frames else None
    if B == 0:
        return duration, feats, frames
    _rt._launch("infer_features_tokens_kernel<round>" if round_duration else "infer_features_tokens_kernel", 0.0, 44.0 * B * L,
                _rt.lib().ispk_infer_features_tokens_f32, pc.data_ptr(), _rt._ptr(dur_f), _rt._ptr(dur_i), _rt._ptr(pt), _rt._ptr(et),
                cc.data_ptr(), int(bool(round_duration)), duration.data_ptr(), feats.data_ptr(), _rt._ptr(frames), B, L, _rt._stream())
    return duration, feats, frames


def embed_tokens(text: Tensor, table: Tensor, text_len: Optional[Tensor] = None, want_mask: bool = True):
    _rt._dev(text, table, text_len)
    assert text.dtype == torch.int64 and text.ndim == 2 and table.dtype == torch.float32 and table.stride(1) == 1
    B, L = text.shape
    V, D = table.shape
    text = text.contiguous()
    emb = torch.empty((B, L, D), dtype=torch.float32, device=text.device)
    mask = torch.empty((B, L), dtype=torch.bool, device=text.device) if want_mask else None
    text_len = _rt._i64(text_len)
    if B == 0:
        return emb, mask
    _rt._launch("embed_tokens_kernel", 0.0, 8.0 * B * L * D, _rt.lib().ispk_embed_tokens_f32, text.data_ptr(), table.data_ptr(),
                table.stride(0), V, _rt._ptr(text_len), emb.data_ptr(), _rt._ptr(mask), B, L, D, _rt._stream())
    return emb, mask


def embed_tokens_qkv(text: Tensor, table: Tensor, qkv_table: Tensor, text_len: Optional[Tensor] = None, want_mask: bool = True):
    _rt._dev(text, table, qkv_table, text_len)
    assert text.dtype == torch.int64 and text.ndim == 2 and table.dtype == torch.float32 and table.stride(1) == 1
    B, L = text.shape
    V, D = table.shape
    N = qkv_table.shape[1]
    assert qkv_table.dtype == torch.bfloat16 and qkv_table.shape == (V, N) and qkv_table.stride(1) == 1
    text = text.contiguous()
    emb = torch.empty((B, L, D), dtype=torch.float32, device=text.device)
    qkv = torch.empty((B, L, N), dtype=torch.bfloat16, device=text.device)
    mask = torch.empty((B, L), dtype=torch.bool, device=text.device) if want_mask else None
    text_len = _rt._i64(text_len)
    _rt._launch("embed_tokens_qkv_kernel", 0.0, B * L * (8.0 * D + 4.0 * N), _rt.lib().ispk_embed_tokens_qkv, text.data_ptr(),
                table.data_ptr(), table.stride(0), V, _rt._ptr(text_len), emb.data_ptr(), _rt._ptr(mask), qkv_table.data_ptr(),
                qkv_table.stride(0), qkv.data_ptr(), B, L, D, N, _rt._stream())
    return emb, mask, qkv


def _speaker_ids(speaker: Tensor, B: int):
    assert speaker.dtype == torch.int64
    if speaker.numel() == 1:
        return speaker.contiguous(), 0
    if speaker.ndim == 2 and tuple(speaker.shape) == (B, 1):
        return speaker.contiguous(), 1
    raise ValueError(f"speaker of shape {tuple(speaker.shape)} does not broadcast against enc_out [B={B}, L, D] "
                     "(the reference takes [B, 1] ids or a single id)")


def add_speaker_(x: Tensor, table: Tensor, speaker: Tensor) -> Tensor:
    _rt._dev(x, table, speaker)
    assert x.dtype == torch.float32 and x.ndim == 3 and x.is_contiguous() and table.dtype == torch.float32 and table.stride(1) == 1
    B, L, D = x.shape
    assert table.shape[1] == D
    speaker, stride = _speaker_ids(speaker, B)
    _rt._launch("add_speaker_kernel", 0.0, 8.0 * B * L * D, _rt.lib().ispk_add_speaker_f32, x.data_ptr(), table.data_ptr(), table.stride(0),
                table.shape[0], speaker.data_ptr(), stride, B, L, D, _rt._stream())
    return x


def add_speaker(x: Tensor, table: Tensor, speaker: Tensor) -> Tensor:
    _rt._dev(x, table, speaker)
    assert x.dtype == torch.float32 and x.ndim == 3 and x.is_contiguous() and table.dtype == torch.float32 and table.stride(1) == 1
    B, L, D = x.shape
    assert table.shape[1] == D
    speaker, stride = _speaker_ids(speaker, B)
    out = torch.empty_like(x)
    _rt._launch("add_speaker_out_kernel", 0.0, 8.0 * B * L * D, _rt.lib().ispk_add_speaker_out_f32, x.data_ptr(), out.data_ptr(),
                table.data_ptr(), table.stride(0), table.shape[0], speaker.data_ptr(), stride, B, L, D, _rt._stream())
    return out


def speaker_grad(d_x: Tensor, speaker: Tensor, speakers: int, text_len: Optional[Tensor] = None, out: Optional[Tensor] = None,
                 accumulate: bool = False) -> Tensor:
    _rt._dev(d_x, speaker, text_len, out)
    assert d_x.dtype == torch.float32 and d_x.ndim == 3
    d_x = d_x.contiguous()
    B, L, D = d_x.shape
    speaker, stride = _speaker_ids(speaker, B)
    if text_len is not None:
        text_len = _rt._i64(text_len)
        assert text_len.numel() == B
    if out is None:
        assert not accumulate
        out = torch.empty((speakers, D), dtype=torch.float32, device=d_x.device)
    assert out.dtype == torch.float32 and tuple(out.shape) == (speakers, D) and out.stride(1) == 1
    ws = _rt.workspace(d_x.device, B * -(-L // 16) * D)
    _rt._launch("speaker_grad_kernels", 1.0 * B * L * D, 4.0 * B * L * D + 4.0 * speakers * D, _rt.lib().ispk_speaker_grad_f32, d_x.data_ptr(),
                speaker.data_ptr(), stride, _rt._ptr(text_len), ws.data_ptr(), ws.numel(), out.data_ptr(), out.stride(0), speakers, B, L, D,
                1 if accumulate else 0, _rt._stream())
    return out


def time_embedding(t: Tensor, inv_freq: Tensor, freq_scale: Tensor, w0: Tensor, b0: Tensor, w1: Tensor, b1: Tensor) -> Tensor:
    _rt._dev(t, inv_freq, freq_scale, w0, b0, w1, b1)
    tf = t.to(torch.float32).contiguous()
    E, H = w1.shape[0], inv_freq.numel()
    assert w0.shape == (E, 1 + 2 * H) and w1.shape == (E, E) and w0.is_contiguous() and w1.is_contiguous()
    out = torch.empty((*t.shape, E), dtype=torch.float32, device=t.device)
    if tf.numel() == 0:
        return out
    _rt._launch("time_embedding_kernel", 0.0, 0.0, _rt.lib().ispk_time_embedding_f32, tf.data_ptr(), tf.numel(), inv_freq.data_ptr(),
                freq_scale.data_ptr(), H, w0.data_ptr(), b0.data_ptr(), w1.data_ptr(), b1.data_ptr(), E, out.data_ptr(),
                _rt._stream())
    return out


def length_regulate(x: Tensor, durations: Tensor, alignment: Optional[Tensor], frames: int, max_len: int = -1,
                    enc_len: Optional[Tensor] = None, want_mask: bool = True, split_bf16=False, next_qkv: Optional[tuple] = None):
    _rt._dev(x, durations, alignment, enc_len)
    assert x.dtype == torch.float32 and x.ndim == 3
    if x.stride(2) != 1 or x.stride(0) != x.shape[1] * x.stride(1):
        x = x.contiguous()
    B, L, D = x.shape
    if alignment is not None:
        assert alignment.dtype == torch.float32 and alignment.shape == (B, frames, L)
        alignment = alignment.contiguous()
    dur_f = dur_i = None
    dur_cols = L
    if durations.dtype == torch.int64:
        assert alignment is not None, "the soft path is generated from fp32 durations"
        dur_i = durations.reshape(B, -1 if B else max(durations.shape[-1], 1)).contiguous()
        dur_cols = dur_i.shape[1]
    else:
        dur_f = durations.to(torch.float32).contiguous()
        assert dur_f.shape == (B, L)
    enc_len = _rt._i64(enc_len)
    out = torch.empty((B, frames, D), dtype=torch.float32, device=x.device)
    dec_len = torch.empty((B,), dtype=torch.int64, device=x.device)
    mask = torch.empty((B, frames), dtype=torch.bool, device=x.device) if want_mask else None
    nb = 4.0 * B * (frames * D + L * D + (frames * L if alignment is not None else 0))
    if B == 0:
        qkv = () if next_qkv is None else (torch.empty((B, frames, 512), dtype=torch.bfloat16, device=x.device),)
        return (out, dec_len, mask, *qkv)
    if next_qkv is not None:
        gamma, beta, eps, wqc = next_qkv
        _rt._dev(gamma, beta, wqc)
        assert split_bf16 is True and D == 384, "the q/kv epilogue is built for the bf16 path at dim 384"
        assert wqc.dtype == torch.bfloat16 and wqc.shape == (D // 16, 512, 16) and wqc.is_contiguous()
        assert gamma.dtype == beta.dtype == torch.float32 and gamma.numel() == beta.numel() == D
        qkv = torch.empty((B, frames, 512), dtype=torch.bfloat16, device=x.device)
        _rt._launch("length_regulate_qkv_kernel", 2.0 * B * frames * (L + 512) * D, nb + 2.0 * (B * frames * 512 + 512 * D),
                    _rt.lib().ispk_length_regulate_qkv_bf16, _rt._ptr(alignment), _rt._ptr(dur_f), _rt._ptr(dur_i), _rt._ptr(enc_len), x.data_ptr(),
                    x.stride(1), out.data_ptr(), dec_len.data_ptr(), _rt._ptr(mask), gamma.data_ptr(), beta.data_ptr(), float(eps),
                    wqc.data_ptr(), qkv.data_ptr(), 512, B, frames, L, D, max_len, dur_cols, _rt._stream())
        return out, dec_len, mask, qkv
    fn = (_rt.lib().ispk_length_regulate_split_f16 if split_bf16 == "f16" else
          _rt.lib().ispk_length_regulate_split_bf16 if split_bf16 else _rt.lib().ispk_length_regulate_f32)
    _rt._launch("length_regulate_kernel<split_f16>" if split_bf16 == "f16" else "length_regulate_kernel<bf16x3>" if split_bf16
                else "length_regulate_kernel", 2.0 * B * frames * L * D, nb, fn, _rt._ptr(alignment),
                _rt._ptr(dur_f), _rt._ptr(dur_i), _rt._ptr(enc_len), x.data_ptr(), x.stride(1), out.data_ptr(), dec_len.data_ptr(),
                _rt._ptr(mask), B, frames, L, D, max_len, dur_cols, _rt._stream())
    return out, dec_len, mask


def _hard_durations(durations: Tensor, B: int, L: int):
    assert durations.shape == (B, L), f"durations {tuple(durations.shape)}: one per token, [{B}, {L}]"
    if durations.dtype == torch.int64:
        return None, durations.contiguous()
    return durations.to(torch.float32).contiguous(), None


def hard_regulate(x: Tensor, durations: Tensor, frames: int, max_len: int = -1, want_mask: bool = True):
    _rt._dev(x, durations)
    assert x.dtype == torch.float32 and x.ndim == 3
    if x.stride(2) != 1 or x.stride(0) != x.shape[1] * x.stride(1):
        x = x.contiguous()
    B, L, D = x.shape
    dur_f, dur_i = _hard_durations(durations, B, L)
    out = torch.empty((B, frames, D), dtype=torch.float32, device=x.device)
    dec_len = torch.empty((B,), dtype=torch.int64, device=x.device)
    mask = torch.empty((B, frames), dtype=torch.bool, device=x.device) if want_mask else None
    _rt._launch("hard_regulate_kernel", 0.0, 4.0 * B * D * (frames + L), _rt.lib().ispk_hard_regulate_f32, _rt._ptr(dur_f), _rt._ptr(dur_i),
                x.data_ptr(), x.stride(1), out.data_ptr(), dec_len.data_ptr(), _rt._ptr(mask), B, frames, L, D, max_len, _rt._stream())
    return out, dec_len, mask


def hard_regulate_bwd(d_out: Tensor, durations: Tensor, max_len: int = -1) -> Tensor:
    _rt._dev(d_out, durations)
    assert d_out.dtype == torch.float32 and d_out.ndim == 3
    d_out = d_out.contiguous()
    B, rows, D = d_out.shape
    L = durations.shape[1]
    dur_f, dur_i = _hard_durations(durations, B, L)
    d_x = torch.empty((B, L, D), dtype=torch.float32, device=d_out.device)
    _rt._launch("hard_regulate_bwd_kernel", 1.0 * B * rows * D, 4.0 * B * D * (rows + L), _rt.lib().ispk_hard_regulate_bwd_f32, _rt._ptr(dur_f),
                _rt._ptr(dur_i), d_out.data_ptr(), d_x.data_ptr(), B, rows, L, D, max_len, _rt._stream())
    return d_x


def hard_average(pitch: Tensor, energy: Tensor, duration: Tensor, text_len: Tensor) -> Tensor:
    _rt._dev(pitch, energy, duration, text_len)
    B, M = pitch.shape
    L = duration.shape[1]
    assert duration.dtype == torch.int64 and duration.shape == (B, L) and energy.shape == (B, M)
    feats = torch.empty((B, L, 3), dtype=torch.float32, device=pitch.device)
    pc, ec, dc, tc = pitch.float().contiguous(), energy.float().contiguous(), duration.contiguous(), _rt._i64(text_len)
    _rt._launch("hard_average_kernel", 0.0, 8.0 * B * M + 20.0 * B * L, _rt.lib().ispk_hard_average_f32, pc.data_ptr(), ec.data_ptr(),
                dc.data_ptr(), tc.data_ptr(), feats.data_ptr(), B, M, L, _rt._stream())
    return feats
```

isp_tts_amd/csrc/aligner.hip:

```cpp
#include "common.h"
#include "dec_len.h"

namespace {

template <typename T_> __device__ __forceinline__ void put(T_* p, float v);
template <> __device__ __forceinline__ void put<float>(float* p, float v) { *p = v; }
template <> __device__ __forceinline__ void put<uint16_t>(uint16_t* p, float v) { *p = f32_to_bf16(v); }
__device__ __forceinline__ void put_split(_Float16* p, float v, int64_t plane) {
    v = __builtin_amdgcn_fmed3f(v, -65504.0f, 65504.0f);
    const _Float16 hi = (_Float16)v;
    p[0] = hi;
    p[plane] = (_Float16)(v - (float)hi);
}
template <typename OutT> __device__ __forceinline__ void put_any(OutT* p, float v, int64_t plane) {
    if constexpr (std::is_same<OutT, _Float16>::value) put_split(p, v, plane);
    else put<OutT>(p, v);
}

template <typename OutT>
__global__ __launch_bounds__(256) void pad_rows_kernel(const float* __restrict__ x, int64_t sb, int64_t st, int64_t sc,
                                                       const int64_t* __restrict__ len, OutT* __restrict__ out, int T,
                                                       int C, int64_t total, int64_t plane) {
    const int64_t idx = (int64_t)blockIdx.x * 256 + threadIdx.x;
    if (idx >= total) return;
    const int c = (int)(idx % C);
    const int64_t row = idx / C;
    const int tp = (int)(row % (T + 4)), b = (int)(row / (T + 4));
    const int t = tp - 2;
    float v = 0.f;
    if (t >= 0 && t < T && t < (int)len[b]) v = x[b * sb + t * st + c * sc];
    put_any<OutT>(out + idx, v, plane);
}

template <typename OutT>
__global__ __launch_bounds__(256) void pad_rows_cf_kernel(const float* __restrict__ x, int64_t sb, int64_t sc,
                                                          const int64_t* __restrict__ len, OutT* __restrict__ out, int T,
                                                          int C, int64_t plane) {
    __shared__ float tile[32][33];
    const int tx = threadIdx.x, ty = threadIdx.y, b = blockIdx.z;
    const int tp0 = blockIdx.x * 32, c0 = blockIdx.y * 32;
    int n = (int)len[b];
    n = n < T ? n : T;
#pragma unroll
    for (int k = 0; k < 4; ++k) {
        const int c = c0 + ty + 8 * k, t = tp0 + tx - 2;
        tile[ty + 8 * k][tx] = (c < C && t >= 0 && t < n) ? x[b * sb + c * sc + t] : 0.f;
    }
    __syncthreads();
#pragma unroll
    for (int k = 0; k < 4; ++k) {
        const int tp = tp0 + ty + 8 * k, c = c0 + tx;
        if (tp < T + 4 && c < C) put_any<OutT>(out + ((int64_t)b * (T + 4) + tp) * C + c, tile[tx][ty + 8 * k], plane);
    }
}

constexpr int kTL = 16;
template <typename OutT>
__global__ __launch_bounds__(1024) void masked_instnorm_kernel(const float* __restrict__ y, const float* __restrict__ w,
                                                               const float* __restrict__ bias,
                                                               const int64_t* __restrict__ len, OutT* __restrict__ out,
                                                               int T, int C, float eps, int64_t plane) {
    __shared__ float red[kTL][64];
    const int cl = threadIdx.x & 63, tl = threadIdx.x >> 6;
    const int b = blockIdx.y, c = blockIdx.x * 64 + cl;
    const bool cok = c < C;
    int n = (int)len[b];
    n = n < 1 ? 1 : (n > T ? T : n);
    const float* yb = y + (int64_t)b * (T + 4) * C;
    OutT* ob = out + (int64_t)b * (T + 4) * C;
    auto total = [&]() {
        float v = 0.f;
#pragma unroll
        for (int i = 0; i < kTL; ++i) v += red[i][cl];
        return v;
    };
    float s = 0.f;
    if (cok) {
        int t = tl;
        for (; t + 7 * kTL < n; t += 8 * kTL) {
            float v[8];
#pragma unroll
            for (int u = 0; u < 8; ++u) v[u] = yb[(int64_t)(t + u * kTL) * C + c];
#pragma unroll
            for (int u = 0; u < 8; ++u) s += v[u];
        }
        for (; t < n; t += kTL) s += yb[(int64_t)t * C + c];
    }
    red[tl][cl] = s;
    __syncthreads();
    const float mean = total() / (float)n;
    __syncthreads();
    float ss = 0.f;
    if (cok) {
        int t = tl;
        for (; t + 7 * kTL < n; t += 8 * kTL) {
            float v[8];
#pragma unroll
            for (int u = 0; u < 8; ++u) v[u] = yb[(int64_t)(t + u * kTL) * C + c];
#pragma unroll
            for (int u = 0; u < 8; ++u) {
                const float d = v[u] - mean;
                ss += d * d;
            }
        }
        for (; t < n; t += kTL) {
            const float d = yb[(int64_t)t * C + c] - mean;
            ss += d * d;
        }
    }
    red[tl][cl] = ss;
    __syncthreads();
    const float var = total() / (float)n;
    if (!cok) return;
    const float rstd = 1.0f / sqrtf(var + eps);
    const float g = w[c], be = bias[c];
#pragma unroll 8
    for (int tp = tl; tp < T + 4; tp += kTL) {
        const int t = tp - 2;
        const int tc = t < 0 ? 0 : (t < n ? t : n - 1);
        const float raw = yb[(int64_t)tc * C + c];
        const float v = (t >= 0 && t < n) ? (raw - mean) * rstd * g + be : 0.f;
        put_any<OutT>(ob + (int64_t)tp * C + c, v, plane);
    }
}

constexpr int kAD = 128;
__device__ __forceinline__ int ks_off(int row, int chunk) { return row * kAD + ((chunk ^ (row & 31)) << 2); }

constexpr int kAsWaves = 2;
typedef uint32_t as_u32x4 __attribute__((ext_vector_type(4)));
__device__ __forceinline__ void as_split8(const float (&v)[8], bf16x8& hi, bf16x8& lo) {
    union { as_u32x4 u; bf16x8 f; } h, l;
#pragma unroll
    for (int e = 0; e < 4; ++e) {
        const float a0 = v[2 * e], a1 = v[2 * e + 1];
        const uint32_t ph = pack_bf16x2(a0, a1);
        h.u[e] = ph;
        l.u[e] = pack_bf16x2(a0 - __builtin_bit_cast(float, ph << 16), a1 - __builtin_bit_cast(float, ph & 0xffff0000u));
    }
    hi = h.f;
    lo = l.f;
}
template <bool kFast>
__device__ __forceinline__ float as_exp(float x) {
    if constexpr (kFast) return __builtin_amdgcn_exp2f(x * 1.4426950408889634f);
    else return expf(x);
}
template <bool kFast>
__device__ __forceinline__ float as_log(float x) {
    if constexpr (kFast) return __builtin_amdgcn_logf(x) * 0.6931471805599453f;
    else return logf(x);
}

template <int NB, bool kFast = false>
__global__ __launch_bounds__(64 * kAsWaves) void aligner_scores_kernel(const float* __restrict__ qe, int64_t q_stride_b,
                                                             const float* __restrict__ ke, int64_t k_stride_b,
                                                             const int64_t* __restrict__ text_len,
                                                             const int64_t* __restrict__ mel_len,
                                                             float* __restrict__ logits, float* __restrict__ soft,
                                                             int M, int L, float scale) {
    extern __shared__ __attribute__((aligned(16))) char smem_raw[];
    float* Ks = reinterpret_cast<float*>(smem_raw);
    char* stage = smem_raw + (threadIdx.x >> 6) * (32 * 144);

    const int tid = threadIdx.x, lane = tid & 63, wave = __builtin_amdgcn_readfirstlane(tid >> 6);
    const int l31 = lane & 31, h = lane >> 5;
    const int b = blockIdx.y;
    const int m0 = blockIdx.x * (32 * kAsWaves) + wave * 32;
    int tl = (int)text_len[b], ml = (int)mel_len[b];
    tl = tl < 1 ? 1 : (tl > L ? L : tl);
    ml = ml < 1 ? 1 : (ml > M ? M : ml);
    const float ninf = -__builtin_huge_valf();

    const float* kb = ke + (int64_t)b * k_stride_b;
    {
        constexpr int kPieces = NB * 32 * (kAD / 4) / (64 * kAsWaves), kBatch = 8;
        static_assert(kPieces % kBatch == 0, "key tile pieces per thread");
        for (int i0 = 0; i0 < kPieces; i0 += kBatch) {
            float4 v[kBatch];
#pragma unroll
            for (int u = 0; u < kBatch; ++u) {
                const int idx = tid + (i0 + u) * (64 * kAsWaves);
                const int row = idx / (kAD / 4), c4 = (idx - row * (kAD / 4)) * 4;
                const int rr = row < L ? row : L - 1;
                v[u] = *reinterpret_cast<const float4*>(kb + (int64_t)rr * kAD + c4);
            }
#pragma unroll
            for (int u = 0; u < kBatch; ++u) {
                const int idx = tid + (i0 + u) * (64 * kAsWaves);
                const int row = idx / (kAD / 4), c4 = (idx - row * (kAD / 4)) * 4;
                *reinterpret_cast<float4*>(Ks + ks_off(row, c4 >> 2)) = row < L ? v[u] : make_float4(0.f, 0.f, 0.f, 0.f);
            }
        }
    }
    const int m = m0 + l31;
    const int mrow = m < M ? m : M - 1;
    f32x4 qf[16];
    {
        const float* qp = qe + (int64_t)b * q_stride_b + (int64_t)mrow * kAD + h * 64;
#pragma unroll
        for (int c = 0; c < 16; ++c) qf[c] = *reinterpret_cast<const f32x4*>(qp + c * 4);
    }
    __syncthreads();

    f32x16 s[NB];
    if constexpr (kFast) {
        bf16x8 qh[8], ql[8];
#pragma unroll
        for (int st = 0; st < 8; ++st) {
            float v[8];
#pragma unroll
            for (int e = 0; e < 4; ++e) { v[e] = qf[2 * st][e]; v[4 + e] = qf[2 * st + 1][e]; }
            as_split8(v, qh[st], ql[st]);
        }
#pragma unroll
        for (int kb_ = 0; kb_ < NB; ++kb_) {
#pragma unroll
            for (int r = 0; r < 16; ++r) s[kb_][r] = 0.f;
#pragma unroll
            for (int st = 0; st < 8; ++st) {
                const f32x4 k0 = *reinterpret_cast<const f32x4*>(Ks + ks_off(kb_ * 32 + l31, h * 16 + 2 * st));
                const f32x4 k1 = *reinterpret_cast<const f32x4*>(Ks + ks_off(kb_ * 32 + l31, h * 16 + 2 * st + 1));
                float v[8];
#pragma unroll
                for (int e = 0; e < 4; ++e) { v[e] = k0[e]; v[4 + e] = k1[e]; }
                bf16x8 kh, kl;
                as_split8(v, kh, kl);
                s[kb_] = __builtin_amdgcn_mfma_f32_32x32x16_bf16(kl, qh[st], s[kb_], 0, 0, 0);
                s[kb_] = __builtin_amdgcn_mfma_f32_32x32x16_bf16(kh, ql[st], s[kb_], 0, 0, 0);
                s[kb_] = __builtin_amdgcn_mfma_f32_32x32x16_bf16(kh, qh[st], s[kb_], 0, 0, 0);
            }
        }
    } else {
#pragma unroll
    for (int kb_ = 0; kb_ < NB; ++kb_) {
#pragma unroll
        for (int r = 0; r < 16; ++r) s[kb_][r] = 0.f;
#pragma unroll
        for (int c = 0; c < 16; ++c) {
            const f32x4 kf = *reinterpret_cast<const f32x4*>(Ks + ks_off(kb_ * 32 + l31, h * 16 + c));
#pragma unroll
            for (int e = 0; e < 4; ++e) s[kb_] = __builtin_amdgcn_mfma_f32_32x32x2f32(kf[e], qf[c][e], s[kb_], 0, 0, 0);
        }
    }
    }

    __syncthreads();

    float rmax = ninf;
#pragma unroll
    for (int kb_ = 0; kb_ < NB; ++kb_)
#pragma unroll
        for (int r = 0; r < 16; ++r) {
            const int key = kb_ * 32 + (r & 3) + 8 * (r >> 2) + 4 * h;
            float v = fminf(s[kb_][r] * scale, 3.4028234663852886e+38f);
            v = key < L ? v : ninf;
            s[kb_][r] = v;
            rmax = fmaxf(rmax, v);
        }
    rmax = fmaxf(rmax, __shfl_xor(rmax, 32, 64));
    float rsum = 0.f, psum = 0.f;
    const float mq = (float)m / (float)ml;
    float pe[NB][16];
#pragma unroll
    for (int kb_ = 0; kb_ < NB; ++kb_)
#pragma unroll
        for (int r = 0; r < 16; ++r) {
            const int key = kb_ * 32 + (r & 3) + 8 * (r >> 2) + 4 * h;
            rsum += as_exp<kFast>(s[kb_][r] - rmax);
            pe[kb_][r] = 0.f;
            if (key < tl && m < ml) {
                const float g = (float)key / (float)tl - mq;
                pe[kb_][r] = as_exp<kFast>(-(g * g) / (2.0f * 0.1f * 0.1f));
                psum += pe[kb_][r];
            }
        }
    rsum += __shfl_xor(rsum, 32, 64);
    psum += __shfl_xor(psum, 32, 64);
    const float lse = rmax + as_log<kFast>(rsum);
    const float pinv = 1.0f / (psum + 1e-5f);

    float smax = ninf;
#pragma unroll
    for (int kb_ = 0; kb_ < NB; ++kb_)
#pragma unroll
        for (int r = 0; r < 16; ++r) {
            const int key = kb_ * 32 + (r & 3) + 8 * (r >> 2) + 4 * h;
            float pr = 0.f;
            if (key < tl && m < ml) {
                pr = pe[kb_][r] * pinv;
                pr = pr < 1e-4f ? 0.f : pr;
            }
            const float lg = (s[kb_][r] - lse) + as_log<kFast>(pr + 1e-6f);
            s[kb_][r] = lg;
            if (key < tl) smax = fmaxf(smax, lg);
        }
    smax = fmaxf(smax, __shfl_xor(smax, 32, 64));
    float esum = 0.f;
#pragma unroll
    for (int kb_ = 0; kb_ < NB; ++kb_)
#pragma unroll
        for (int r = 0; r < 16; ++r) {
            const int key = kb_ * 32 + (r & 3) + 8 * (r >> 2) + 4 * h;
            if (key < tl) esum += as_exp<kFast>(s[kb_][r] - smax);
        }
    esum += __shfl_xor(esum, 32, 64);
    const float einv = (m < ml) ? 1.0f / esum : 0.f;

    float* lb = logits + (int64_t)b * M * L;
    float* sbp = soft + (int64_t)b * M * L;
    const int c = lane & 7;
    const bool vec = (L % 4) == 0;
#pragma unroll
    for (int kb_ = 0; kb_ < NB; ++kb_) {
#pragma unroll
        for (int pass = 0; pass < 2; ++pass) {
#pragma unroll
            for (int g = 0; g < 4; ++g) {
                float4 v;
                float* pv = &v.x;
#pragma unroll
                for (int e = 0; e < 4; ++e) {
                    const int key = kb_ * 32 + 8 * g + 4 * h + e;
                    const float lg = s[kb_][4 * g + e];
                    pv[e] = pass == 0 ? lg : (key < tl ? as_exp<kFast>(lg - smax) * einv : 0.f);
                }
                *reinterpret_cast<float4*>(stage + l31 * 144 + (8 * g + 4 * h) * 4) = v;
            }
            float* dst = pass == 0 ? lb : sbp;
#pragma unroll
            for (int i = 0; i < 4; ++i) {
                const int r = 8 * i + (lane >> 3), mm = m0 + r, key = kb_ * 32 + 4 * c;
                const float4 v = *reinterpret_cast<const float4*>(stage + r * 144 + c * 16);
                if (mm < M && key < L) {
                    float* o = dst + (int64_t)mm * L + key;
                    if (vec) {
                        *reinterpret_cast<float4*>(o) = v;
                    } else {
                        const float* pv = &v.x;
                        for (int e = 0; e < 4 && key + e < L; ++e) o[e] = pv[e];
                    }
                }
            }
        }
    }
}

constexpr int kSaLanes = 16;
__global__ __launch_bounds__(64 * kSaLanes) void soft_average_kernel(const float* __restrict__ attn,
                                                                     const float* __restrict__ pitch,
                                                                     const float* __restrict__ energy,
                                                                     const int64_t* __restrict__ dur,
                                                                     const int64_t* __restrict__ text_len,
                                                                     float* __restrict__ feats, int M, int L) {
    __shared__ float red[3][kSaLanes][64];
    const int b = blockIdx.y, j = threadIdx.x & 63, l = blockIdx.x * 64 + j, ml = threadIdx.x >> 6;
    const bool ok = l < L;
    const float* ab = attn + (int64_t)b * M * L;
    const float* pb = pitch + (int64_t)b * M;
    const float* eb = energy + (int64_t)b * M;
    float sa = 0.f, sp = 0.f, se = 0.f;
    if (ok) {
        int mm = ml;
        for (; mm + 7 * kSaLanes < M; mm += 8 * kSaLanes) {
            float a[8], pv[8], ev[8];
#pragma unroll
            for (int u = 0; u < 8; ++u) {
                a[u] = ab[(int64_t)(mm + u * kSaLanes) * L + l];
                pv[u] = pb[mm + u * kSaLanes];
                ev[u] = eb[mm + u * kSaLanes];
            }
#pragma unroll
            for (int u = 0; u < 8; ++u) {
                sa += a[u];
                sp = fmaf(pv[u], a[u], sp);
                se = fmaf(ev[u], a[u], se);
            }
        }
        for (; mm < M; mm += kSaLanes) {
            const float a = ab[(int64_t)mm * L + l];
            sa += a;
            sp = fmaf(pb[mm], a, sp);
            se = fmaf(eb[mm], a, se);
        }
    }
    red[0][ml][j] = sa;
    red[1][ml][j] = sp;
    red[2][ml][j] = se;
    __syncthreads();
    if (ml == 0 && ok) {
        float a = 0.f, pp = 0.f, ee = 0.f;
#pragma unroll
        for (int u = 0; u < kSaLanes; ++u) {
            a += red[0][u][j];
            pp += red[1][u][j];
            ee += red[2][u][j];
        }
        const float mk = l < (int)text_len[b] ? 1.0f : 0.0f;
        float* f = feats + ((int64_t)b * L + l) * 3;
        f[0] = dur ? log1pf((float)dur[(int64_t)b * L + l]) : 0.0f;
        f[1] = pp / (a + 1e-5f) * mk;
        f[2] = ee / (a + 1e-5f) * mk;
    }
}


__global__ __launch_bounds__(256) void flow_mix_kernel(const float* __restrict__ x0, const float* __restrict__ x1,
                                                       const float* __restrict__ t, float s, float* __restrict__ xt,
                                                       float* __restrict__ flow, int per_batch, int64_t total) {
#pragma clang fp contract(off)
    const int64_t i = (int64_t)blockIdx.x * 256 + threadIdx.x;
    if (i >= total) return;
    const float tb = t[i / per_batch], a = x0[i], b = x1[i];
    const float w0 = 1.0f - s * tb;
    const float p0 = w0 * a, p1 = tb * b;
    xt[i] = p0 + p1;
    const float sa = s * a;
    flow[i] = b - sa;
}

__global__ __launch_bounds__(1024) void flow_finish_kernel(const float* __restrict__ raw, const float* __restrict__ flow,
                                                           const float* __restrict__ x0, const uint8_t* __restrict__ mask,
                                                           float* __restrict__ pred, float* __restrict__ dur,
                                                           float* __restrict__ ratio, float* __restrict__ loss, int B, int L,
                                                           int C) {
    __shared__ float sratio[1024];
    const int tid = threadIdx.x, sub = tid & 15, grp = tid >> 4;
    const int n = L * C;
    for (int b0 = 0; b0 < B; b0 += 64) {
        const int b = b0 + grp;
        float num = 0.f, den = 0.f;
        if (b < B) {
            const float* rb = raw + (int64_t)b * n;
            const float* fb = flow + (int64_t)b * n;
            const float* xb = x0 + (int64_t)b * n;
            const uint8_t* mb = mask + (int64_t)b * L;
            float* pb = pred + (int64_t)b * n;
#pragma unroll 4
            for (int e = sub; e < n; e += 16) {
                const int l = e / C, c = e - l * C;
                const bool m = mb[l] != 0;
                const float r = rb[e], f = fb[e], x = xb[e];
                const float pf = m ? r : 0.f;
                const float pr = m ? x + pf : 0.f;
                pb[e] = pr;
                if (c == 0) dur[(int64_t)b * L + l] = fmaxf(expf(pr) - 1.0f, 0.f);
                const float d = pf - f;
                num += m ? d * d : 0.f;
                den += m ? 1.0f : 0.f;
            }
        }
#pragma unroll
        for (int off = 8; off > 0; off >>= 1) {
            num += __shfl_xor(num, off, 64);
            den += __shfl_xor(den, off, 64);
        }
        if (b < B && sub == 0) {
            const float q = num / fmaxf(den, 1e-5f);
            ratio[b] = q;
            if (b < 1024) sratio[b] = q;
        }
    }
    __syncthreads();
    if (loss && tid == 0) {
        float s = 0.f;
        if (B <= 1024) {
            for (int b = 0; b < B; ++b) s += sratio[b];
        } else {
            for (int b = 0; b < B; ++b) s += ratio[b];
        }
        loss[0] = s / (float)B;
    }
}


constexpr int kFhRows = 16;
__global__ __launch_bounds__(256) void flow_head_kernel(const float* __restrict__ y, int64_t ldy, const float* __restrict__ gamma,
                                                        const float* __restrict__ beta, float eps, const float* __restrict__ W,
                                                        const float* __restrict__ bias, const float* __restrict__ flow,
                                                        const float* __restrict__ x0, const uint8_t* __restrict__ mask,
                                                        float* __restrict__ pred, float* __restrict__ dur,
                                                        float* __restrict__ part, int L, int nblk) {
#pragma clang fp contract(off)
    __shared__ float sp[4][2];
    const int lane = threadIdx.x & 63, wave = threadIdx.x >> 6;
    const int b = blockIdx.y, blk = blockIdx.x;
    const f32x4 g4 = *reinterpret_cast<const f32x4*>(gamma + 4 * lane), b4 = *reinterpret_cast<const f32x4*>(beta + 4 * lane);
    f32x4 w4[3];
#pragma unroll
    for (int c = 0; c < 3; ++c) w4[c] = *reinterpret_cast<const f32x4*>(W + c * 256 + 4 * lane);
    const float bc[3] = {bias[0], bias[1], bias[2]};
    float num = 0.f, den = 0.f;
    const int l0 = blk * kFhRows + wave * 4;
    f32x4 v[4];
#pragma unroll
    for (int i = 0; i < 4; ++i) {
        const int l = l0 + i < L ? l0 + i : L - 1;
        v[i] = *reinterpret_cast<const f32x4*>(y + ((int64_t)b * L + l) * ldy + 4 * lane);
    }
#pragma unroll
    for (int i = 0; i < 4; ++i) {
        const int l = l0 + i;
        const bool live = l < L;
        const int64_t r = (int64_t)b * L + (live ? l : L - 1);
        const bool m = mask[r] != 0;
        const float mean = wave_sum((v[i][0] + v[i][1]) + (v[i][2] + v[i][3])) * (1.0f / 256.0f);
        float q = 0.f;
#pragma unroll
        for (int e = 0; e < 4; ++e) {
            const float d = v[i][e] - mean;
            q = fmaf(d, d, q);
        }
        const float rstd = 1.0f / sqrtf(wave_sum(q) * (1.0f / 256.0f) + eps);
        float h[4];
#pragma unroll
        for (int e = 0; e < 4; ++e) h[e] = m ? fmaf((v[i][e] - mean) * rstd, g4[e], b4[e]) : 0.f;
        float raw[3];
#pragma unroll
        for (int c = 0; c < 3; ++c) {
            float a = 0.f;
#pragma unroll
            for (int e = 0; e < 4; ++e) a = fmaf(h[e], w4[c][e], a);
            raw[c] = wave_sum(a) + bc[c];
        }
        if (live) {
#pragma unroll
            for (int c = 0; c < 3; ++c) {
                const float f = flow[r * 3 + c], x = x0[r * 3 + c];
                const float pf = m ? raw[c] : 0.f;
                const float pr = m ? x + pf : 0.f;
                if (lane == c) pred[r * 3 + c] = pr;
                if (c == 0 && lane == 0) dur[r] = fmaxf(expf(pr) - 1.0f, 0.f);
                const float d = pf - f;
                num += m ? d * d : 0.f;
                den += m ? 1.0f : 0.f;
            }
        }
    }
    if (lane == 0) { sp[wave][0] = num; sp[wave][1] = den; }
    __syncthreads();
    if (threadIdx.x == 0) {
        const int64_t o = ((int64_t)b * nblk + blk) * 2;
        part[o] = (sp[0][0] + sp[1][0]) + (sp[2][0] + sp[3][0]);
        part[o + 1] = (sp[0][1] + sp[1][1]) + (sp[2][1] + sp[3][1]);
    }
}
__global__ __launch_bounds__(1024) void flow_head_finalize_kernel(const float* __restrict__ part, int nblk, float* __restrict__ ratio,
                                                                  float* __restrict__ loss, int B) {
    __shared__ float sratio[1024];
    const int tid = threadIdx.x;
    float s = 0.f;
    for (int b0 = 0; b0 < B; b0 += 1024) {
        const int b = b0 + tid;
        if (b < B) {
            float num = 0.f, den = 0.f;
            for (int k = 0; k < nblk; ++k) {
                num += part[((int64_t)b * nblk + k) * 2];
                den += part[((int64_t)b * nblk + k) * 2 + 1];
            }
            const float q = num / fmaxf(den, 1e-5f);
            ratio[b] = q;
            sratio[tid] = q;
        }
        __syncthreads();
        if (tid == 0) {
            const int n = B - b0 < 1024 ? B - b0 : 1024;
            for (int i = 0; i < n; ++i) s += sratio[i];
        }
        __syncthreads();
    }
    if (loss && tid == 0) loss[0] = s / (float)B;
}

__global__ __launch_bounds__(256) void flow_euler_kernel(const float* __restrict__ xt, const float* __restrict__ vel, float dt,
                                                         const uint8_t* __restrict__ mask, float* __restrict__ out, int C,
                                                         int64_t total) {
#pragma clang fp contract(off)
    const int64_t i = (int64_t)blockIdx.x * 256 + threadIdx.x;
    if (i >= total) return;
    const float step = vel[i] * dt;
    float v = xt[i] + step;
    if (mask) v = mask[i / C] ? v : v * 0.0f;
    out[i] = v;
}

template <bool kRound>
__device__ __forceinline__ float infer_features_token(const float* __restrict__ pred, const float* __restrict__ dur_f,
                                                      const int64_t* __restrict__ dur_i, const float* __restrict__ pitch_t,
                                                      const float* __restrict__ energy_t, float df, float pf, float pd, float ef,
                                                      float ed, float* __restrict__ feats, int64_t i) {
#pragma clang fp contract(off)
    const float e = expf(pred[3 * i]) - 1.0f;
    const float scaled = df * e;
    float d = fmaxf(kRound ? rintf(scaled) : scaled, 0.0f);
    if (dur_f) { const float t = dur_f[i]; d = t < 0.0f ? d : t; }
    if (dur_i) { const int64_t t = dur_i[i]; d = t < 0 ? d : (float)t; }
    const float p = pitch_t ? pitch_t[i] : pred[3 * i + 1], q = energy_t ? energy_t[i] : pred[3 * i + 2];
    const float pm = p * pf, qm = q * ef;
    feats[2 * i] = pm + pd;
    feats[2 * i + 1] = qm + ed;
    return d;
}

template <bool kRound>
__global__ __launch_bounds__(256) void infer_features_kernel(const float* __restrict__ pred, const float* __restrict__ dur_f,
                                                             const int64_t* __restrict__ dur_i, const float* __restrict__ pitch_t,
                                                             const float* __restrict__ energy_t, float df, float pf, float pd,
                                                             float ef, float ed, float* __restrict__ duration,
                                                             float* __restrict__ feats, int64_t n) {
    const int64_t i = (int64_t)blockIdx.x * 256 + threadIdx.x;
    if (i >= n) return;
    duration[i] = infer_features_token<kRound>(pred, dur_f, dur_i, pitch_t, energy_t, df, pf, pd, ef, ed, feats, i);
}

constexpr int kItemsChunk = 1024;
template <bool kRound, bool kTokens = false>
__global__ __launch_bounds__(256) void infer_features_items_kernel(const float* __restrict__ pred, const float* __restrict__ dur_f,
                                                                   const int64_t* __restrict__ dur_i,
                                                                   const float* __restrict__ pitch_t,
                                                                   const float* __restrict__ energy_t,
                                                                   const float* __restrict__ controls, float* __restrict__ duration,
                                                                   float* __restrict__ feats, int64_t* __restrict__ frames_wanted,
                                                                   int L) {
    __shared__ float dur_s[kItemsChunk];
    __shared__ int64_t reps_s[4];
    const int b = blockIdx.x, tid = threadIdx.x;
    float df = 0.f, pf = 0.f, pd = 0.f, ef = 0.f, ed = 0.f;
    if constexpr (!kTokens) {
        const float* c = controls + (int64_t)b * 5;
        df = c[0]; pf = c[1]; pd = c[2]; ef = c[3]; ed = c[4];
    }
    float s = 0.f;
    int64_t reps = 0;
    for (int base = 0; base < L; base += kItemsChunk) {
        const int n = L - base < kItemsChunk ? L - base : kItemsChunk;
        for (int l = tid; l < n; l += 256) {
            const int64_t i = (int64_t)b * L + base + l;
            if constexpr (kTokens) {
                const float* c = controls + i * 5;
                df = c[0]; pf = c[1]; pd = c[2]; ef = c[3]; ed = c[4];
            }
            const float d = infer_features_token<kRound>(pred, dur_f, dur_i, pitch_t, energy_t, df, pf, pd, ef, ed, feats, i);
            duration[i] = d;
            dur_s[l] = d;
            if constexpr (kRound) reps += hd_reps<true>(dur_s, nullptr, l);
        }
        if (!kRound && frames_wanted) {
            __syncthreads();
            if (tid == 0) s = soft_dur_sum<false>(dur_s, n, s, nullptr);
            __syncthreads();
        }
    }
    if (!frames_wanted) return;
    if constexpr (kRound) {
#pragma unroll
        for (int off = 32; off > 0; off >>= 1) reps += __shfl_xor(reps, off, 64);
        if ((tid & 63) == 0) reps_s[tid >> 6] = reps;
        __syncthreads();
        if (tid == 0) frames_wanted[b] = reps_s[0] + reps_s[1] + reps_s[2] + reps_s[3];
    } else {
        if (tid == 0) frames_wanted[b] = soft_dec_len(s);
    }
}

}

extern "C" int32_t ispk_pad_rows_f32(const float* x, int64_t stride_b, int64_t stride_t, int64_t stride_c,
                                     const int64_t* len, void* out, int32_t out_bf16, int32_t B, int32_t T, int32_t C,
                                     ispk_stream_t stream) {
    ISPK_REQUIRE(x && len && out, ISPK_E_NULL, "pad_rows: null pointer");
    ISPK_REQUIRE(B >= 0 && T >= 1 && C >= 1, ISPK_E_SHAPE, "pad_rows: bad shape B=%d T=%d C=%d", B, T, C);
    if (B == 0) return 0;
    const int64_t total = (int64_t)B * (T + 4) * C;
    dim3 grid((unsigned)((total + 255) / 256));
    hipStream_t s = reinterpret_cast<hipStream_t>(stream);
    ISPK_REQUIRE(out_bf16 >= 0 && out_bf16 <= 2, ISPK_E_UNSUPPORTED, "pad_rows: output mode %d (0 fp32, 1 bf16, 2 split fp16 planes)", out_bf16);
    if (stride_t == 1 && stride_c > 1 && B <= 65535) {
        dim3 gcf((T + 4 + 31) / 32, (C + 31) / 32, B), bcf(32, 8);
        if (out_bf16 == 2)
            hipLaunchKernelGGL(pad_rows_cf_kernel<_Float16>, gcf, bcf, 0, s, x, stride_b, stride_c, len,
                               static_cast<_Float16*>(out), T, C, total);
        else if (out_bf16)
            hipLaunchKernelGGL(pad_rows_cf_kernel<uint16_t>, gcf, bcf, 0, s, x, stride_b, stride_c, len,
                               static_cast<uint16_t*>(out), T, C, (int64_t)0);
        else
            hipLaunchKernelGGL(pad_rows_cf_kernel<float>, gcf, bcf, 0, s, x, stride_b, stride_c, len,
                               static_cast<float*>(out), T, C, (int64_t)0);
        return ispk_launch_status();
    }
    if (out_bf16 == 2)
        hipLaunchKernelGGL(pad_rows_kernel<_Float16>, grid, dim3(256), 0, s, x, stride_b, stride_t, stride_c, len,
                           static_cast<_Float16*>(out), T, C, total, total);
    else if (out_bf16)
        hipLaunchKernelGGL(pad_rows_kernel<uint16_t>, grid, dim3(256), 0, s, x, stride_b, stride_t, stride_c, len,
                           static_cast<uint16_t*>(out), T, C, total, (int64_t)0);
    else
        hipLaunchKernelGGL(pad_rows_kernel<float>, grid, dim3(256), 0, s, x, stride_b, stride_t, stride_c, len,
                           static_cast<float*>(out), T, C, total, (int64_t)0);
    return ispk_launch_status();
}

extern "C" int32_t ispk_masked_instnorm_f32(const float* y, const float* weight, const float* bias, const int64_t* len,
                                            void* out, int32_t out_bf16, int32_t B, int32_t T, int32_t C, float eps,
                                            ispk_stream_t stream) {
    ISPK_REQUIRE(y && weight && bias && len && out, ISPK_E_NULL, "masked_instnorm: null pointer");
    ISPK_REQUIRE(B >= 0 && T >= 1 && C >= 1, ISPK_E_SHAPE, "masked_instnorm: bad shape B=%d T=%d C=%d", B, T, C);
    ISPK_REQUIRE(B <= 65535, ISPK_E_SHAPE, "masked_instnorm: B=%d exceeds the grid limit", B);
    if (B == 0) return 0;
    dim3 grid((C + 63) / 64, B);
    hipStream_t s = reinterpret_cast<hipStream_t>(stream);
    ISPK_REQUIRE(out_bf16 >= 0 && out_bf16 <= 2, ISPK_E_UNSUPPORTED, "masked_instnorm: output mode %d (0 fp32, 1 bf16, 2 split fp16 planes)", out_bf16);
    if (out_bf16 == 2)
        hipLaunchKernelGGL(masked_instnorm_kernel<_Float16>, grid, dim3(1024), 0, s, y, weight, bias, len,
                           static_cast<_Float16*>(out), T, C, eps, (int64_t)B * (T + 4) * C);
    else if (out_bf16)
        hipLaunchKernelGGL(masked_instnorm_kernel<uint16_t>, grid, dim3(1024), 0, s, y, weight, bias, len,
                           static_cast<uint16_t*>(out), T, C, eps, (int64_t)0);
    else
        hipLaunchKernelGGL(masked_instnorm_kernel<float>, grid, dim3(1024), 0, s, y, weight, bias, len,
                           static_cast<float*>(out), T, C, eps, (int64_t)0);
    return ispk_launch_status();
}

static int32_t aligner_scores_launch(const float* q_enc, int64_t q_stride_b, const float* k_enc, int64_t k_stride_b,
                                     const int64_t* text_len, const int64_t* mel_len, float* attn_logits, float* attn_soft,
                                     int32_t B, int32_t M, int32_t L, int32_t D, ispk_stream_t stream, bool fast) {
    ISPK_REQUIRE(q_enc && k_enc && text_len && mel_len && attn_logits && attn_soft, ISPK_E_NULL,
                 "aligner_scores: null pointer");
    ISPK_REQUIRE(D == kAD, ISPK_E_UNSUPPORTED, "aligner_scores: attention_dim %d (built for 128)", D);
    ISPK_REQUIRE(B >= 0 && M >= 1 && L >= 1 && L <= 320, ISPK_E_SHAPE, "aligner_scores: bad shape B=%d M=%d L=%d (L <= 320)",
                 B, M, L);
    ISPK_REQUIRE(B <= 65535, ISPK_E_SHAPE, "aligner_scores: B=%d exceeds the grid limit", B);
    ISPK_REQUIRE(ispk_aligned(q_enc, 16) && ispk_aligned(k_enc, 16) && ispk_aligned(attn_logits, 16) &&
                     ispk_aligned(attn_soft, 16) && q_stride_b % 4 == 0 && k_stride_b % 4 == 0,
                 ISPK_E_ALIGN, "aligner_scores: 16-byte alignment required");
    if (B == 0) return 0;
    const int nb = (L + 31) / 32;
    size_t lds = (size_t)nb * 32 * kAD * 4;
    if (lds < kAsWaves * 32 * 144) lds = kAsWaves * 32 * 144;
    const float scale = 1.0f / sqrtf((float)D);
    dim3 grid((M + 32 * kAsWaves - 1) / (32 * kAsWaves), B), block(64 * kAsWaves);
    hipStream_t s = reinterpret_cast<hipStream_t>(stream);
#define ISPK_AL_CASE(NB)                                                                                              \
    case NB:                                                                                                          \
        if (fast) {                                                                                                   \
            ISPK_RESERVE_LDS((&aligner_scores_kernel<NB, true>), lds, "aligner_scores");                              \
            hipLaunchKernelGGL((aligner_scores_kernel<NB, true>), grid, block, lds, s, q_enc, q_stride_b, k_enc,      \
                               k_stride_b, text_len, mel_len, attn_logits, attn_soft, M, L, scale);                   \
        } else {                                                                                                      \
            ISPK_RESERVE_LDS((&aligner_scores_kernel<NB, false>), lds, "aligner_scores");                             \
            hipLaunchKernelGGL((aligner_scores_kernel<NB, false>), grid, block, lds, s, q_enc, q_stride_b, k_enc,     \
                               k_stride_b, text_len, mel_len, attn_logits, attn_soft, M, L, scale);                   \
        }                                                                                                             \
        break;
    switch (nb) {
        ISPK_AL_CASE(1) ISPK_AL_CASE(2) ISPK_AL_CASE(3) ISPK_AL_CASE(4) ISPK_AL_CASE(5) ISPK_AL_CASE(6) ISPK_AL_CASE(7)
        ISPK_AL_CASE(8) ISPK_AL_CASE(9) ISPK_AL_CASE(10)
        default: ISPK_FAIL(ISPK_E_SHAPE, "aligner_scores: unsupported L=%d", L);
    }
#undef ISPK_AL_CASE
    return ispk_launch_status();
}

extern "C" int32_t ispk_aligner_scores_f32(const float* q_enc, int64_t q_stride_b, const float* k_enc,
                                           int64_t k_stride_b, const int64_t* text_len, const int64_t* mel_len,
                                           float* attn_logits, float* attn_soft, int32_t B, int32_t M, int32_t L,
                                           int32_t D, ispk_stream_t stream) {
    return aligner_scores_launch(q_enc, q_stride_b, k_enc, k_stride_b, text_len, mel_len, attn_logits, attn_soft, B, M, L, D, stream,
                                 false);
}

extern "C" int32_t ispk_aligner_scores_fast_f32(const float* q_enc, int64_t q_stride_b, const float* k_enc,
                                                int64_t k_stride_b, const int64_t* text_len, const int64_t* mel_len,
                                                float* attn_logits, float* attn_soft, int32_t B, int32_t M, int32_t L,
                                                int32_t D, ispk_stream_t stream) {
    return aligner_scores_launch(q_enc, q_stride_b, k_enc, k_stride_b, text_len, mel_len, attn_logits, attn_soft, B, M, L, D, stream,
                                 true);
}

extern "C" int32_t ispk_soft_average_f32(const float* attn_soft, const float* pitch, const float* energy,
                                         const int64_t* duration, const int64_t* text_len, float* feats, int32_t B,
                                         int32_t M, int32_t L, ispk_stream_t stream) {
    ISPK_REQUIRE(attn_soft && pitch && energy && text_len && feats, ISPK_E_NULL, "soft_average: null pointer");
    ISPK_REQUIRE(B >= 0 && M >= 1 && L >= 1 && B <= 65535, ISPK_E_SHAPE, "soft_average: bad shape B=%d M=%d L=%d", B, M, L);
    if (B == 0) return 0;
    hipLaunchKernelGGL(soft_average_kernel, dim3((L + 63) / 64, B), dim3(64 * kSaLanes), 0, reinterpret_cast<hipStream_t>(stream),
                       attn_soft, pitch, energy, duration, text_len, feats, M, L);
    return ispk_launch_status();
}

extern "C" int32_t ispk_flow_mix_f32(const float* x0, const float* x1, const float* t, float sigma, float* x_t, float* flow,
                                     int32_t B, int32_t L, int32_t C, ispk_stream_t stream) {
    ISPK_REQUIRE(x0 && x1 && t && x_t && flow, ISPK_E_NULL, "flow_mix: null pointer");
    ISPK_REQUIRE(B >= 0 && L >= 1 && C >= 1, ISPK_E_SHAPE, "flow_mix: bad shape B=%d L=%d C=%d", B, L, C);
    if (B == 0) return 0;
    const int64_t total = (int64_t)B * L * C;
    const float s = (float)(1.0 - (double)sigma);
    hipLaunchKernelGGL(flow_mix_kernel, dim3((unsigned)((total + 255) / 256)), dim3(256), 0,
                       reinterpret_cast<hipStream_t>(stream), x0, x1, t, s, x_t, flow, L * C, total);
    return ispk_launch_status();
}

extern "C" int32_t ispk_flow_finish_f32(const float* pred_raw, const float* flow, const float* x0, const uint8_t* mask,
                                        float* pred, float* duration, float* loss_ratio, float* loss_mean, int32_t B,
                                        int32_t L, int32_t C, ispk_stream_t stream) {
    ISPK_REQUIRE(pred_raw && flow && x0 && mask && pred && duration && loss_ratio, ISPK_E_NULL, "flow_finish: null pointer");
    ISPK_REQUIRE(B >= 0 && L >= 1 && C >= 1 && B <= 65535, ISPK_E_SHAPE, "flow_finish: bad shape B=%d L=%d C=%d", B, L, C);
    if (B == 0) return 0;
    hipLaunchKernelGGL(flow_finish_kernel, dim3(1), dim3(1024), 0, reinterpret_cast<hipStream_t>(stream), pred_raw, flow, x0,
                       mask, pred, duration, loss_ratio, loss_mean, B, L, C);
    return ispk_launch_status();
}

extern "C" int32_t ispk_flow_head_f32(const float* y, int64_t ldy, const float* norm_gamma, const float* norm_beta, float norm_eps,
                                      const float* W, const float* bias, const float* flow, const float* x0, const uint8_t* mask,
                                      float* pred, float* duration, float* loss_ratio, float* loss_mean, float* workspace,
                                      int32_t B, int32_t L, int32_t D, int32_t C, ispk_stream_t stream) {
    ISPK_REQUIRE(y && norm_gamma && norm_beta && W && bias && flow && x0 && mask && pred && duration && loss_ratio && workspace,
                 ISPK_E_NULL, "flow_head: null pointer");
    ISPK_REQUIRE(D == 256 && C == 3, ISPK_E_UNSUPPORTED, "flow_head: built for dim 256 -> 3 flow channels (got %d -> %d)", D, C);
    ISPK_REQUIRE(B >= 0 && L >= 1 && B <= 65535 && ldy >= D && ldy % 4 == 0, ISPK_E_SHAPE, "flow_head: bad shape B=%d L=%d", B, L);
    ISPK_REQUIRE(ispk_aligned(y, 16) && ispk_aligned(norm_gamma, 16) && ispk_aligned(norm_beta, 16) && ispk_aligned(W, 16), ISPK_E_ALIGN,
                 "flow_head: y / gamma / beta / W must be 16-byte aligned");
    if (B == 0) return 0;
    const int nblk = (L + kFhRows - 1) / kFhRows;
    hipStream_t s = reinterpret_cast<hipStream_t>(stream);
    hipLaunchKernelGGL(flow_head_kernel, dim3(nblk, B), dim3(256), 0, s, y, ldy, norm_gamma, norm_beta, norm_eps, W, bias, flow, x0, mask,
                       pred, duration, workspace, L, nblk);
    if (int32_t rc = ispk_launch_status()) return rc;
    hipLaunchKernelGGL(flow_head_finalize_kernel, dim3(1), dim3(1024), 0, s, workspace, nblk, loss_ratio, loss_mean, B);
    return ispk_launch_status();
}

extern "C" int32_t ispk_flow_euler_f32(const float* x_t, const float* velocity, float dt, const uint8_t* mask, float* out,
                                       int32_t B, int32_t L, int32_t C, ispk_stream_t stream) {
    ISPK_REQUIRE(x_t && velocity && out, ISPK_E_NULL, "flow_euler: null pointer");
    ISPK_REQUIRE(B >= 0 && L >= 1 && C >= 1, ISPK_E_SHAPE, "flow_euler: bad shape B=%d L=%d C=%d", B, L, C);
    if (B == 0) return 0;
    const int64_t total = (int64_t)B * L * C;
    hipLaunchKernelGGL(flow_euler_kernel, dim3((unsigned)((total + 255) / 256)), dim3(256), 0,
                       reinterpret_cast<hipStream_t>(stream), x_t, velocity, dt, mask, out, C, total);
    return ispk_launch_status();
}

static int32_t infer_features_launch(const float* pred, const float* duration_target_f32, const int64_t* duration_target_i64,
                                     const float* pitch_target, const float* energy_target, float duration_factor,
                                     float pitch_factor, float pitch_delta, float energy_factor, float energy_delta,
                                     float* duration, float* features, int32_t B, int32_t L, ispk_stream_t stream, bool round) {
    ISPK_REQUIRE(pred && duration && features, ISPK_E_NULL, "infer_features: null pointer");
    ISPK_REQUIRE(!(duration_target_f32 && duration_target_i64), ISPK_E_UNSUPPORTED, "infer_features: one duration target at most");
    ISPK_REQUIRE(B >= 0 && L >= 1, ISPK_E_SHAPE, "infer_features: bad shape B=%d L=%d", B, L);
    if (B == 0) return 0;
    const int64_t n = (int64_t)B * L;
    const dim3 grid((unsigned)((n + 255) / 256));
    hipStream_t s = reinterpret_cast<hipStream_t>(stream);
    if (round)
        hipLaunchKernelGGL(infer_features_kernel<true>, grid, dim3(256), 0, s, pred, duration_target_f32, duration_target_i64,
                           pitch_target, energy_target, duration_factor, pitch_factor, pitch_delta, energy_factor, energy_delta,
                           duration, features, n);
    else
        hipLaunchKernelGGL(infer_features_kernel<false>, grid, dim3(256), 0, s, pred, duration_target_f32, duration_target_i64,
                           pitch_target, energy_target, duration_factor, pitch_factor, pitch_delta, energy_factor, energy_delta,
                           duration, features, n);
    return ispk_launch_status();
}

extern "C" int32_t ispk_infer_features_f32(const float* pred, const float* duration_target_f32, const int64_t* duration_target_i64,
                                           const float* pitch_target, const float* energy_target, float duration_factor,
                                           float pitch_factor, float pitch_delta, float energy_factor, float energy_delta,
                                           float* duration, float* features, int32_t B, int32_t L, ispk_stream_t stream) {
    return infer_features_launch(pred, duration_target_f32, duration_target_i64, pitch_target, energy_target, duration_factor,
                                 pitch_factor, pitch_delta, energy_factor, energy_delta, duration, features, B, L, stream, false);
}

extern "C" int32_t ispk_infer_features_round_f32(const float* pred, const float* duration_target_f32,
                                                 const int64_t* duration_target_i64, const float* pitch_target,
                                                 const float* energy_target, float duration_factor, float pitch_factor,
                                                 float pitch_delta, float energy_factor, float energy_delta, float* duration,
                                                 float* features, int32_t B, int32_t L, ispk_stream_t stream) {
    return infer_features_launch(pred, duration_target_f32, duration_target_i64, pitch_target, energy_target, duration_factor,
                                 pitch_factor, pitch_delta, energy_factor, energy_delta, duration, features, B, L, stream, true);
}

extern "C" int32_t ispk_infer_features_items_f32(const float* pred, const float* duration_target_f32,
                                                 const int64_t* duration_target_i64, const float* pitch_target,
                                                 const float* energy_target, const float* controls, int32_t round, float* duration,
                                                 float* features, int64_t* frames_wanted, int32_t B, int32_t L,
                                                 ispk_stream_t stream) {
    ISPK_REQUIRE(pred && controls && duration && features, ISPK_E_NULL, "infer_features_items: null pointer");
    ISPK_REQUIRE(!(duration_target_f32 && duration_target_i64), ISPK_E_UNSUPPORTED,
                 "infer_features_items: one duration target at most");
    ISPK_REQUIRE(B >= 0 && L >= 1, ISPK_E_SHAPE, "infer_features_items: bad shape B=%d L=%d", B, L);
    if (B == 0) return 0;
    hipStream_t s = reinterpret_cast<hipStream_t>(stream);
    if (round)
        hipLaunchKernelGGL(infer_features_items_kernel<true>, dim3(B), dim3(256), 0, s, pred, duration_target_f32,
                           duration_target_i64, pitch_target, energy_target, controls, duration, features, frames_wanted, L);
    else
        hipLaunchKernelGGL(infer_features_items_kernel<false>, dim3(B), dim3(256), 0, s, pred, duration_target_f32,
                           duration_target_i64, pitch_target, energy_target, controls, duration, features, frames_wanted, L);
    return ispk_launch_status();
}

extern "C" int32_t ispk_infer_features_tokens_f32(const float* pred, const float* duration_target_f32,
                                                  const int64_t* duration_target_i64, const float* pitch_target,
                                                  const float* energy_target, const float* controls, int32_t round, float* duration,
                                                  float* features, int64_t* frames_wanted, int32_t B, int32_t L,
                                                  ispk_stream_t stream) {
    ISPK_REQUIRE(pred && controls && duration && features, ISPK_E_NULL, "infer_features_tokens: null pointer");
    ISPK_REQUIRE(!(duration_target_f32 && duration_target_i64), ISPK_E_UNSUPPORTED,
                 "infer_features_tokens: one duration target at most");
    ISPK_REQUIRE(B >= 0 && L >= 1, ISPK_E_SHAPE, "infer_features_tokens: bad shape B=%d L=%d", B, L);
    if (B == 0) return 0;
    hipStream_t s = reinterpret_cast<hipStream_t>(stream);
    if (round)
        hipLaunchKernelGGL((infer_features_items_kernel<true, true>), dim3(B), dim3(256), 0, s, pred, duration_target_f32,
                           duration_target_i64, pitch_target, energy_target, controls, duration, features, frames_wanted, L);
    else
        hipLaunchKernelGGL((infer_features_items_kernel<false, true>), dim3(B), dim3(256), 0, s, pred, duration_target_f32,
                           duration_target_i64, pitch_target, energy_target, controls, duration, features, frames_wanted, L);
    return ispk_launch_status();
}
```

isp_tts_amd/csrc/mas.hip:

```cpp
#include <stdlib.h>

#include "common.h"

namespace {

template <int NC> constexpr int rows_ahead() { return NC <= 2 ? 32 : (NC <= 4 ? 16 : 8); }

__device__ __forceinline__ float dpp_ror1(float src) {
    return __builtin_bit_cast(float, __builtin_amdgcn_update_dpp(0, __builtin_bit_cast(int, src), 0x13C, 0xf, 0xf, false));
}

constexpr int kBlk = 32;

template <int NC, int R>
__device__ __forceinline__ void mas_rows(float (&q)[NC], const float (&use)[R][NC], uint32_t (&h)[NC], float qnan) {
    static_for<0, R>([&](auto rc) {
        constexpr int r = decltype(rc)::value;
        float left[NC];
#pragma unroll
        for (int c = 0; c < NC; ++c) left[c] = dpp_shr1(q[c], c > 0 ? dpp_ror1(q[c - 1]) : qnan);
#pragma unroll
        for (int c = 0; c < NC; ++c) {
            const bool diag = left[c] >= q[c];
            h[c] = h[c] + h[c] + (diag ? 1u : 0u);
            q[c] = use[r][c] + (diag ? left[c] : q[c]);
        }
    });
}

__device__ __forceinline__ void walk_step(int& d, uint32_t& taken, uint64_t word) {
    uint32_t t;
    asm volatile("s_bitcmp1_b64 %3, %0\n\ts_cselect_b32 %2, 1, 0\n\ts_addc_u32 %0, %0, 0\n\ts_lshl1_add_u32 %1, %1, %2"
                 : "+s"(d), "+s"(taken), "=&s"(t)
                 : "s"(word)
                 : "scc");
}

template <int NC>
__global__ __launch_bounds__(256) void mas_kernel(const float* __restrict__ logits, const int64_t* __restrict__ text_len,
                                                  const int64_t* __restrict__ mel_len, int16_t* __restrict__ attn_hard,
                                                  int64_t* __restrict__ dur, int16_t* __restrict__ path_out, int M_max,
                                                  int L_max, int64_t stride_b, int64_t stride_m) {
    extern __shared__ __attribute__((aligned(16))) char smem[];
    const int nblk = (M_max + kBlk - 1) / kBlk;
    uint32_t* hist = reinterpret_cast<uint32_t*>(smem);
    int16_t* path = reinterpret_cast<int16_t*>(smem + (size_t)nblk * NC * 256);
    int* cnt = reinterpret_cast<int*>(smem + (size_t)nblk * NC * 256 + (((size_t)M_max * 2 + 15) & ~(size_t)15));

    const int b = blockIdx.x;
    const int tid = threadIdx.x;
    const int lane = tid & 63;
    const int wave = tid >> 6;
    int n = (int)mel_len[b];
    int m = (int)text_len[b];
    n = n < 1 ? 1 : (n > M_max ? M_max : n);
    m = m < 1 ? 1 : (m > L_max ? L_max : m);
    const float* lp = logits + (int64_t)b * stride_b;
    const float ninf = -__builtin_huge_valf();

    for (int j = tid; j < L_max; j += 256) cnt[j] = 0;
#ifdef ISPK_EXPERIMENTS
    const int abl = (int)(stride_m >> 40);
    stride_m &= ((int64_t)1 << 40) - 1;
#else
    constexpr int abl = 0;
#endif

    if (wave == 0) {
        float q[NC];
#pragma unroll
        for (int c = 0; c < NC; ++c) q[c] = (lane + 64 * c == 0) ? lp[0] : ninf;
        const auto rsrc = __builtin_amdgcn_make_buffer_rsrc(const_cast<float*>(lp), 0,
                                                            (int)((int64_t)M_max * stride_m * 4), 0x00020000);
        int voff[NC];
#pragma unroll
        for (int c = 0; c < NC; ++c) voff[c] = 4 * min(lane + 64 * c, m - 1);
        const int row_bytes = (int)(stride_m * 4), last_off = (n - 1) * row_bytes;
        constexpr int kRows = rows_ahead<NC>(), kSub = kBlk / kRows;
        float bufa[kRows][NC], bufb[kRows][NC];
        auto load_rows = [&](float (&dst)[kRows][NC], int base) __attribute__((always_inline)) {
            int off = base * row_bytes;
#pragma unroll
            for (int r = 0; r < kRows; ++r) {
                const int so = min(off, last_off);
#pragma unroll
                for (int c = 0; c < NC; ++c)
                    dst[r][c] = __builtin_bit_cast(float, __builtin_amdgcn_raw_buffer_load_b32(rsrc, voff[c], so, 0));
                off += row_bytes;
            }
        };
        const float qnan = __builtin_nanf("");
        load_rows(bufa, 1);
        uint32_t h[NC];
        for (int base = 1; base < n; base += 2 * kBlk) {
            static_for<0, 2 * kSub>([&](auto sc) {
                constexpr int sub = decltype(sc)::value, in_blk = sub % kSub;
                const int rows_base = base + sub * kRows;
                if (rows_base < n) {
                    if (sub % 2 == 0) load_rows(bufb, rows_base + kRows); else load_rows(bufa, rows_base + kRows);
                    if (in_blk == 0) {
#pragma unroll
                        for (int c = 0; c < NC; ++c) h[c] = 0u;
                    }
                    if (sub % 2 == 0) mas_rows<NC, kRows>(q, bufa, h, qnan); else mas_rows<NC, kRows>(q, bufb, h, qnan);
                    uint32_t* dst = hist + (size_t)((rows_base - 1) / kBlk) * NC * 64 + lane;
#pragma unroll
                    for (int c = 0; c < NC; ++c) dst[64 * c] = h[c] << (kRows * (kSub - 1 - in_blk));
                }
            });
        }
    }
    __syncthreads();

    if (wave == 0 && abl != 1) {
        int j0 = m - 1;
        for (int top = n - 1; top >= 1;) {
            const int blk = (top - 1) / kBlk, base = 1 + blk * kBlk, rows = top - base + 1;
            const int col = j0 - lane;
            uint32_t w = (col >= 0 && lane <= kBlk) ? hist[(size_t)blk * NC * 64 + col] : 0u;
            if (rows < kBlk) w &= ~((1u << (kBlk - rows)) - 1u);
            int d = 0;
            uint32_t taken = 0u;
#pragma unroll
            for (int r0 = kBlk - 16; r0 >= 0; r0 -= 16) {
                uint64_t word[16];
#pragma unroll
                for (int u = 0; u < 16; ++u) word[u] = __ballot(((w >> (kBlk - 1 - (r0 + u))) & 1u) != 0u);
#pragma unroll
                for (int u = 15; u >= 0; --u) walk_step(d, taken, word[u]);
            }
            const int myj = j0 - __builtin_popcountll((uint64_t)taken >> (lane + 1));
            if (lane < rows) path[base + lane] = (int16_t)myj;
            j0 -= d;
            top = base - 1;
        }
        if (lane == 0) path[0] = (int16_t)j0;
    }
    __syncthreads();

    if (abl == 1 || abl == 2) return;
    for (int i = tid; i < n; i += 256) atomicAdd(&cnt[path[i]], 1);
    if (path_out) {
        int16_t* po = path_out + (int64_t)b * M_max;
        for (int i = tid; i < M_max; i += 256) po[i] = i < n ? path[i] : (int16_t)-1;
    }
    const int64_t total = (int64_t)M_max * L_max;
    int16_t* out = attn_hard + (int64_t)b * total;
    if ((total & 7) == 0 && (((uintptr_t)attn_hard) & 15) == 0) {
        const uint32_t step_i = 2048u / (uint32_t)L_max, step_c = 2048u % (uint32_t)L_max;
        int gi = (int)((uint32_t)(tid * 8) / (uint32_t)L_max), gc = (int)((uint32_t)(tid * 8) % (uint32_t)L_max);
        for (int64_t e0 = (int64_t)tid * 8; e0 < total; e0 += 256 * 8) {
            int i = gi, col = gc;
            gi += (int)step_i;
            gc += (int)step_c;
            if (gc >= L_max) {
                gc -= L_max;
                ++gi;
            }
            int hot = i < n ? path[i] : -1;
            uint16_t v[8];
#pragma unroll
            for (int t = 0; t < 8; ++t) {
                v[t] = col == hot ? 1 : 0;
                if (++col == L_max) {
                    col = 0;
                    ++i;
                    hot = i < n ? path[i] : -1;
                }
            }
            uint4 pk;
            pk.x = v[0] | ((uint32_t)v[1] << 16);
            pk.y = v[2] | ((uint32_t)v[3] << 16);
            pk.z = v[4] | ((uint32_t)v[5] << 16);
            pk.w = v[6] | ((uint32_t)v[7] << 16);
            *reinterpret_cast<uint4*>(out + e0) = pk;
        }
    } else {
        for (int64_t e = tid; e < total; e += 256) {
            int i = (int)(e / L_max);
            int col = (int)(e - (int64_t)i * L_max);
            out[e] = (i < n && col == path[i]) ? 1 : 0;
        }
    }
    __syncthreads();
    if (dur) {
        int64_t* d = dur + (int64_t)b * L_max;
        const int64_t fix = mel_len[b] - (int64_t)n;
        for (int jx = tid; jx < L_max; jx += 256) d[jx] = cnt[jx] + (jx == 0 ? fix : 0);
    }
}

template <int NC>
int32_t launch(const float* logits, const int64_t* text_len, const int64_t* mel_len, int16_t* attn_hard, int64_t* dur,
               int16_t* path, int B, int M_max, int L_max, int64_t sb, int64_t sm, size_t lds, hipStream_t stream) {
    ISPK_RESERVE_LDS((&mas_kernel<NC>), lds, "mas");
#ifdef ISPK_EXPERIMENTS
    if (const char* e = ispk_knob("ISPK_MAS_ABLATE")) sm |= (int64_t)atoi(e) << 40;
#endif
    hipLaunchKernelGGL(mas_kernel<NC>, dim3(B), dim3(256), lds, stream, logits, text_len, mel_len, attn_hard, dur, path,
                       M_max, L_max, sb, sm);
    return ispk_launch_status();
}

}

extern "C" int32_t ispk_mas_f32(const float* logits, const int64_t* text_len, const int64_t* mel_len,
                                int16_t* attn_hard, int64_t* dur, int16_t* path, int32_t B, int32_t M_max,
                                int32_t L_max, int64_t stride_b, int64_t stride_m, ispk_stream_t stream) {
    ISPK_REQUIRE(logits && text_len && mel_len && attn_hard, ISPK_E_NULL, "mas: null pointer argument");
    ISPK_REQUIRE(B >= 0 && M_max >= 1 && L_max >= 1, ISPK_E_SHAPE, "mas: bad shape B=%d M=%d L=%d", B, M_max, L_max);
    ISPK_REQUIRE(L_max <= 512 && M_max <= 4096, ISPK_E_SHAPE, "mas: L_max %d > 512 or M_max %d > 4096", L_max, M_max);
    ISPK_REQUIRE(stride_m >= L_max && stride_b >= (int64_t)M_max * 1, ISPK_E_SHAPE, "mas: bad strides");
    if (B == 0) return 0;
    const int nc = (L_max + 63) / 64;
    const size_t lds = (size_t)((M_max + 31) / 32) * nc * 256 + (((size_t)M_max * 2 + 15) & ~(size_t)15) + (size_t)L_max * 4;
    ISPK_REQUIRE((int64_t)M_max * stride_m * 4 < ((int64_t)1 << 31), ISPK_E_SHAPE,
                 "mas: one utterance's logits (M_max * stride_m floats) must span less than 2 GiB");
    ISPK_REQUIRE(lds <= 160 * 1024, ISPK_E_SHAPE, "mas: M_max=%d x L_max=%d needs %zu B of LDS (> 160 KiB)", M_max,
                 L_max, lds);
    hipStream_t s = reinterpret_cast<hipStream_t>(stream);
#define ISPK_MAS_CASE(NC) \
    case NC:              \
        return launch<NC>(logits, text_len, mel_len, attn_hard, dur, path, B, M_max, L_max, stride_b, stride_m, lds, s);
    switch (nc) {
        ISPK_MAS_CASE(1)
        ISPK_MAS_CASE(2)
        ISPK_MAS_CASE(3)
        ISPK_MAS_CASE(4)
        ISPK_MAS_CASE(5)
        ISPK_MAS_CASE(6)
        ISPK_MAS_CASE(7)
        ISPK_MAS_CASE(8)
    }
#undef ISPK_MAS_CASE
    ISPK_FAIL(ISPK_E_SHAPE, "mas: unsupported chunk count %d", nc);
}
```

Baseline: 17.02 million mel-frames/s.

## Fuse MAS with flow-matching target mixing on the predictor side stream

Adds a MAS kernel variant that, once the per-token durations are known, also writes the log-duration target plus the flow-matching x_t and flow tensors. This removes the separate soft-average and flow_mix launches, and MAS now runs deferred inside the predictor branch on the side stream instead of on the main path. It also adds a fused flow-head kernel that finalizes the loss through an atomic counter, but that path is off by default (fused_finalize=False). The cost is that the whole MAS now sits on the predictor stream's critical path, and the default-off counter-based head adds complexity.

```diff
diff --git a/include/ispk.h b/include/ispk.h
--- a/include/ispk.h
+++ b/include/ispk.h
@@ -23,6 +23,10 @@
 int32_t ispk_mas_f32(const float* logits, const int64_t* text_len, const int64_t* mel_len, int16_t* attn_hard,
                      int64_t* dur, int16_t* path, int32_t B, int32_t M_max, int32_t L_max, int64_t stride_b,
                      int64_t stride_m, ispk_stream_t stream);
+int32_t ispk_mas_flow_front_f32(const float* logits, const int64_t* text_len, const int64_t* mel_len, int16_t* attn_hard,
+                                int64_t* dur, int16_t* path, const float* feats, const float* x0, const float* t, float sigma,
+                                float* targets, float* x_t, float* flow, int32_t B, int32_t M_max, int32_t L_max,
+                                int64_t stride_b, int64_t stride_m, ispk_stream_t stream);
 
 int32_t ispk_layernorm_f32(const float* x, int64_t ldx, const float* gamma, const float* beta, const float* ada_scale,
                            const float* ada_shift, int64_t ada_stride, int32_t rows_per_batch,
@@ -162,6 +166,10 @@
                            const float* W, const float* bias, const float* flow, const float* x0, const uint8_t* mask,
                            float* pred, float* duration, float* loss_ratio, float* loss_mean, float* workspace, int32_t B,
                            int32_t L, int32_t D, int32_t C, ispk_stream_t stream);
+int32_t ispk_flow_head_fused_f32(const float* y, int64_t ldy, const float* norm_gamma, const float* norm_beta, float norm_eps,
+                                 const float* W, const float* bias, const float* flow, const float* x0, const uint8_t* mask,
+                                 float* pred, float* duration, float* loss_ratio, float* loss_mean, float* workspace,
+                                 uint32_t* counter, int32_t B, int32_t L, int32_t D, int32_t C, ispk_stream_t stream);
 int32_t ispk_flow_euler_f32(const float* x_t, const float* velocity, float dt, const uint8_t* mask, float* out, int32_t B,
                             int32_t L, int32_t C, ispk_stream_t stream);
 int32_t ispk_infer_features_f32(const float* pred, const float* duration_target_f32, const int64_t* duration_target_i64,
diff --git a/isp_tts_amd/acoustic/alignment.py b/isp_tts_amd/acoustic/alignment.py
--- a/isp_tts_amd/acoustic/alignment.py
+++ b/isp_tts_amd/acoustic/alignment.py
@@ -137,8 +137,10 @@
                                        attention_prior=attention_prior)
 
     def forward(self, mel: Tensor, enc_text: Tensor, mel_len: Tensor, text_len: Tensor,
-                q_proj: Optional[Tensor] = None, mas_stream=None) -> AlignerOutput:
+                q_proj: Optional[Tensor] = None, mas_stream=None, defer_mas: bool = False) -> AlignerOutput:
         attn_soft, attn_logits = self.attention(mel, enc_text, mel_len, text_len, q_proj=q_proj)
+        if defer_mas:
+            return AlignerOutput(attn_soft=attn_soft, attn_logits=attn_logits, attn_hard=None, attn_hard_duration=None)
         if mas_stream is not None and attn_logits.is_cuda:
             mas_stream.wait_stream(torch.cuda.current_stream())
             with torch.cuda.stream(mas_stream):
diff --git a/isp_tts_amd/acoustic/model.py b/isp_tts_amd/acoustic/model.py
--- a/isp_tts_amd/acoustic/model.py
+++ b/isp_tts_amd/acoustic/model.py
@@ -144,8 +144,9 @@
             q_proj.record_stream(main)
         branch = side if q_proj is not None else None
         hard = not self.temporal_adaptor.soft_duration
+        front = self.temporal_adaptor.use_mas_front(branch, self.compute_dtype, mel.is_cuda)
         aligner_output = self.aligner(mel=mel, enc_text=enc_out.transpose(1, 2).detach(), mel_len=mel_len,
-                                      text_len=text_len, q_proj=q_proj, mas_stream=None if hard else branch)
+                                      text_len=text_len, q_proj=q_proj, mas_stream=None if hard else branch, defer_mas=front)
         if speaker is not None:
             enc_out = runtime.add_speaker(enc_out, self.speaker_embedding.weight, speaker)
         adaptor_output = self.temporal_adaptor(
@@ -153,7 +154,10 @@
             duration_target=aligner_output.attn_hard_duration, alignment=aligner_output.attn_soft,
             pitch_target_dense=pitch, energy_target_dense=energy, noise=flow_noise, time_steps=flow_time,
             enc_len=text_len, predictor_stream=branch, duration_sum=mel_len if branch is not None and not hard else None,
-            qkv_for=self._decoder_first())
+            qkv_for=self._decoder_first(), mas_logits=aligner_output.attn_logits if front else None)
+        if front:
+            attn_hard, attn_hard_duration = self.temporal_adaptor._mas
+            aligner_output = aligner_output._replace(attn_hard=attn_hard, attn_hard_duration=attn_hard_duration)
         dec_len = adaptor_output.dec_lengths
         dec_mask = adaptor_output.dec_mask
         dec_out = self.decoder(adaptor_output.enc_out, mask=dec_mask, key_len=dec_len, out_dtype=self.compute_dtype,
diff --git a/isp_tts_amd/acoustic/temporal_adaptor.py b/isp_tts_amd/acoustic/temporal_adaptor.py
--- a/isp_tts_amd/acoustic/temporal_adaptor.py
+++ b/isp_tts_amd/acoustic/temporal_adaptor.py
@@ -58,6 +58,7 @@
         self.linear_layer = nn.Linear(self.transformer.dim, output_dim, bias=True)
         self.output_dim, self.sigma, self.detach_inputs = output_dim, sigma, detach_inputs
         self.fused_head = True
+        self.fused_finalize = False
         self._cache = StagedWeights()
         self._grids: dict = {}
 
@@ -81,7 +82,7 @@
         return runtime.gemm(c, self._cond_weight(cdt), bias=self.transformer.project_emb.bias, out_dtype=torch.float32)
 
     def forward(self, x: Tensor, targets: Tensor, mask: Optional[Tensor] = None, *, noise: Optional[Tensor] = None,
-                time_steps: Optional[Tensor] = None, key_len: Optional[Tensor] = None):
+                time_steps: Optional[Tensor] = None, key_len: Optional[Tensor] = None, mixed: Optional[tuple] = None):
         cond = x
         have_mask = mask is not None
         if mask is None:
@@ -92,7 +93,11 @@
         x0 = torch.randn_like(x1) if noise is None else noise.to(x1)
         t = torch.rand((x1.shape[0],), dtype=x1.dtype, device=x1.device) if time_steps is None else time_steps.to(x1)
         time_emb = self.time_embedding(t)
-        x_t, flow = runtime.flow_mix(x0, x1, t, self.sigma)
+        if mixed is not None:
+            assert noise is not None and time_steps is not None
+            x_t, flow = mixed
+        else:
+            x_t, flow = runtime.flow_mix(x0, x1, t, self.sigma)
         proj = self._project(x_t, self._cond_projection(cond))
         tr = self.transformer
         head = (self.fused_head and tr.dim == 256 and self.output_dim == 3 and tr.norm.weight is not None and tr.norm.bias is not None
@@ -100,8 +105,9 @@
         out = tr(None, mask=mask, adaptive_condition=time_emb, projected=proj, key_len=key_len if have_mask else None,
                  final_norm=not head).out
         if head:
-            pred, self._duration_estimate, _, loss = runtime.flow_head(out, tr.norm.weight, tr.norm.bias, tr.norm.eps,
-                                                                       self.linear_layer.weight, self.linear_layer.bias, flow, x0, mask)
+            head_fn = runtime.flow_head_fused if self.fused_finalize else runtime.flow_head
+            pred, self._duration_estimate, _, loss = head_fn(out, tr.norm.weight, tr.norm.bias, tr.norm.eps,
+                                                             self.linear_layer.weight, self.linear_layer.bias, flow, x0, mask)
             return pred, {"flow_loss": loss}
         raw = runtime.linear_small(out, self.linear_layer.weight, self.linear_layer.bias)
         pred, self._duration_estimate, _, loss = runtime.flow_finish(raw, flow, x0, mask)
@@ -239,7 +245,9 @@
         self.feature_dim = 3
         self.pitch, self.energy, self.soft_duration = pitch, energy, soft_duration
         self.pitch_idx, self.energy_idx = 1, 2
-        self.predictor = FlowTransformerTemporalModule.init(predictor, input_dim=encoder_dim, output_dim=self.feature_dim)
+        self.mas_front = True
+        self._mas = None
+        self.predictor =FlowTransformerTemporalModule.init(predictor, input_dim=encoder_dim, output_dim=self.feature_dim)
         self.embedding = TransformerTemporalModule.init(embedding, input_dim=self.feature_dim - 1, output_dim=encoder_dim)
 
     def _process_target(self, dense: Tensor, duration_target: Tensor, alignment: Tensor, enc_mask: Tensor) -> Tensor:
@@ -247,14 +255,21 @@
             dense = dense[:, None]
         return self.averager(dense, duration_target, alignment).transpose(1, 2) * enc_mask
 
+    def use_mas_front(self, predictor_stream, compute_dtype: torch.dtype, on_gpu: bool = True) -> bool:
+        return bool(self.mas_front and self.soft_duration and predictor_stream is not None and on_gpu
+                    and compute_dtype == torch.bfloat16 and not torch.is_grad_enabled())
+
     def forward(self, enc_out: Tensor, enc_mask: Tensor, max_dec_len: int, duration_target: Optional[Tensor] = None,
                 alignment: Optional[Tensor] = None, pitch_target_dense: Optional[Tensor] = None,
                 energy_target_dense: Optional[Tensor] = None, *, noise: Optional[Tensor] = None,
                 time_steps: Optional[Tensor] = None, enc_len: Optional[Tensor] = None,
-                predictor_stream=None, duration_sum: Optional[Tensor] = None, qkv_for=None) -> TemporalAdaptorOutput:
-        assert duration_target is not None and (alignment is not None or not self.soft_duration)
+                predictor_stream=None, duration_sum: Optional[Tensor] = None, qkv_for=None,
+                mas_logits: Optional[Tensor] = None) -> TemporalAdaptorOutput:
+        front = mas_logits is not None
+        assert (duration_target is not None) != front and (alignment is not None or not self.soft_duration)
         assert pitch_target_dense is not None and energy_target_dense is not None
         hard = not self.soft_duration
+        assert not front or (self.soft_duration and predictor_stream is not None and enc_out.is_cuda and duration_sum is not None)
         m3 = enc_mask[..., None]
         if enc_len is None:
             enc_len = enc_mask.sum(dim=1)
@@ -288,6 +303,14 @@
             enc_out, dec_lens = decoder_input(enc_out)
 
         def predict():
+            if front:
+                x0 = noise if noise is not None else torch.randn_like(feats)
+                t = time_steps if time_steps is not None else torch.rand((feats.shape[0],), dtype=feats.dtype, device=feats.device)
+                attn_hard, dur, tg, x_t, flow = runtime.mas_flow_front(mas_logits, enc_len, duration_sum, feats, x0, t,
+                                                                       self.predictor.sigma)
+                self._mas = (attn_hard, dur)
+                pred_, losses_ = self.predictor(cond, tg, m3, noise=x0, time_steps=t, key_len=enc_len, mixed=(x_t, flow))
+                return pred_, losses_, self.predictor._duration_estimate
             tg = targets
             if tg is None:
                 tg = runtime.soft_average(alignment, pitch_target_dense, energy_target_dense, duration_target, enc_len)
@@ -298,7 +321,7 @@
             side.wait_event(ready)
             with torch.cuda.stream(side):
                 pred, losses, duration_pred = predict()
-            for t in (cond, feats, alignment, pitch_target_dense, energy_target_dense):
+            for t in (cond, feats, alignment, pitch_target_dense, energy_target_dense, mas_logits):
                 if t is not None:
                     t.record_stream(side)
             if self.predictor_first:
diff --git a/isp_tts_amd/bindings/adaptor.py b/isp_tts_amd/bindings/adaptor.py
--- a/isp_tts_amd/bindings/adaptor.py
+++ b/isp_tts_amd/bindings/adaptor.py
@@ -5,7 +5,7 @@
 
 from .. import runtime as _rt
 
-__all__ = ["mas", "pad_rows", "conv5_padded", "masked_instnorm", "aligner_scores", "soft_average", "flow_mix", "flow_finish",
+__all__ = ["mas", "mas_flow_front", "flow_head_fused", "pad_rows", "conv5_padded", "masked_instnorm", "aligner_scores", "soft_average", "flow_mix", "flow_finish",
            "flow_head", "flow_euler", "infer_features", "infer_features_items", "infer_features_tokens", "embed_tokens", "embed_tokens_qkv", "_speaker_ids", "add_speaker_",
            "add_speaker", "speaker_grad", "time_embedding", "length_regulate", "_hard_durations", "hard_regulate",
            "hard_regulate_bwd", "hard_average"]
@@ -28,6 +28,30 @@
     return hard, dur, path
 
 
+def mas_flow_front(logits: Tensor, text_len: Tensor, mel_len: Tensor, feats: Tensor, x0: Tensor, t: Tensor, sigma: float,
+                   want_path: bool = False):
+    _rt._dev(logits, text_len, mel_len, feats, x0, t)
+    assert logits.dtype == torch.float32 and logits.ndim == 3
+    if logits.stride(2) != 1:
+        logits = logits.contiguous()
+    B, M, L = logits.shape
+    assert feats.dtype == torch.float32 and tuple(feats.shape) == (B, L, 3) and tuple(x0.shape) == (B, L, 3) and t.numel() == B
+    text_len, mel_len = _rt._i64(text_len), _rt._i64(mel_len)
+    fc, x0c, tc = feats.contiguous(), x0.float().contiguous(), t.float().contiguous()
+    hard = torch.empty((B, M, L), dtype=torch.int16, device=logits.device)
+    dur = torch.empty((B, L), dtype=torch.int64, device=logits.device)
+    path = torch.empty((B, M), dtype=torch.int16, device=logits.device) if want_path else None
+    targets, xt, flow = torch.empty_like(fc), torch.empty_like(fc), torch.empty_like(fc)
+    out = (hard, dur, targets, xt, flow, path) if want_path else (hard, dur, targets, xt, flow)
+    if B == 0:
+        return out
+    _rt._launch(f"mas_kernel_flow_front<{(L + 63) // 64}>", 0.0, 6.0 * B * M * L, _rt.lib().ispk_mas_flow_front_f32, logits.data_ptr(),
+                text_len.data_ptr(), mel_len.data_ptr(), hard.data_ptr(), dur.data_ptr(), _rt._ptr(path), fc.data_ptr(), x0c.data_ptr(),
+                tc.data_ptr(), float(sigma), targets.data_ptr(), xt.data_ptr(), flow.data_ptr(), B, M, L, logits.stride(0),
+                logits.stride(1), _rt._stream())
+    return out
+
+
 def pad_rows(x: Tensor, lengths: Tensor, channel_first: bool = False, out_dtype: torch.dtype = torch.float32) -> Tensor:
     _rt._dev(x, lengths)
     assert x.dtype == torch.float32 and x.ndim == 3
@@ -149,6 +173,53 @@
     _rt._launch("flow_head_kernels", 0.0, 4.0 * B * L * D, _rt.lib().ispk_flow_head_f32, y.data_ptr(), y.stride(1), norm_weight.data_ptr(),
                 norm_bias.data_ptr(), float(norm_eps), weight.data_ptr(), bias.data_ptr(), fl.data_ptr(), x0c.data_ptr(), mk.data_ptr(),
                 pred.data_ptr(), dur.data_ptr(), ratio.data_ptr(), loss.data_ptr(), ws.data_ptr(), B, L, D, C, _rt._stream())
+    return pred, dur, ratio, loss
+
+
+_COUNTER_BLOCK = 4096
+_counter_blocks: dict = {}
+_counter_eager: dict = {}
+
+
+def _counter_word(device: torch.device) -> Tensor:
+    device = torch.device(device.type, device.index if device.index is not None else torch.cuda.current_device())
+    capturing = torch.cuda.is_current_stream_capturing()
+    key = (device, torch.cuda.current_stream(device).cuda_stream)
+    if not capturing and key in _counter_eager:
+        return _counter_eager[key]
+    slot = _counter_blocks.get(device)
+    if slot is None or slot[1] == _COUNTER_BLOCK:
+        if capturing:
+            return torch.zeros(1, dtype=torch.int32, device=device)
+        slot = _counter_blocks[device] = [torch.zeros(_COUNTER_BLOCK, dtype=torch.int32, device=device), 0]
+        torch.cuda.current_stream(device).synchronize()
+    word = slot[0][slot[1]:slot[1] + 1]
+    slot[1] += 1
+    if not capturing:
+        _counter_eager[key] = word
+    return word
+
+
+def flow_head_fused(y: Tensor, norm_weight: Tensor, norm_bias: Tensor, norm_eps: float, weight: Tensor, bias: Tensor, flow: Tensor,
+                    x0: Tensor, mask: Tensor):
+    _rt._dev(y, norm_weight, norm_bias, weight, bias, flow, x0, mask)
+    B, L, D = y.shape
+    C = weight.shape[0]
+    assert y.dtype == torch.float32 and y.stride(2) == 1 and y.stride(0) == L * y.stride(1) and weight.shape == (C, D) and weight.is_contiguous()
+    assert mask.dtype == torch.bool and mask.shape == (B, L)
+    fl, x0c, mk = flow.contiguous(), x0.float().contiguous(), mask.contiguous()
+    pred = torch.empty((B, L, C), dtype=torch.float32, device=y.device)
+    dur = torch.empty((B, L), dtype=torch.float32, device=y.device)
+    ratio = torch.empty((B,), dtype=torch.float32, device=y.device)
+    loss = torch.empty((), dtype=torch.float32, device=y.device)
+    if B == 0:
+        return pred, dur, ratio, loss.fill_(float("nan"))
+    ws = torch.empty((2 * B * ((L + 15) // 16),), dtype=torch.float32, device=y.device)
+    word = _counter_word(y.device)
+    _rt._launch("flow_head_fused_kernel", 0.0, 4.0 * B * L * D, _rt.lib().ispk_flow_head_fused_f32, y.data_ptr(), y.stride(1),
+                norm_weight.data_ptr(), norm_bias.data_ptr(), float(norm_eps), weight.data_ptr(), bias.data_ptr(), fl.data_ptr(),
+                x0c.data_ptr(), mk.data_ptr(), pred.data_ptr(), dur.data_ptr(), ratio.data_ptr(), loss.data_ptr(), ws.data_ptr(),
+                word.data_ptr(), B, L, D, C, _rt._stream())
     return pred, dur, ratio, loss
 
 
diff --git a/isp_tts_amd/csrc/aligner.hip b/isp_tts_amd/csrc/aligner.hip
--- a/isp_tts_amd/csrc/aligner.hip
+++ b/isp_tts_amd/csrc/aligner.hip
@@ -1,5 +1,6 @@
 #include "common.h"
 #include "dec_len.h"
+#include "flow_front.h"
 
 namespace {
 
@@ -398,7 +399,7 @@
         }
         const float mk = l < (int)text_len[b] ? 1.0f : 0.0f;
         float* f = feats + ((int64_t)b * L + l) * 3;
-        f[0] = dur ? log1pf((float)dur[(int64_t)b * L + l]) : 0.0f;
+        f[0] = dur ? flow_duration_target(dur[(int64_t)b * L + l]) : 0.0f;
         f[1] = pp / (a + 1e-5f) * mk;
         f[2] = ee / (a + 1e-5f) * mk;
     }
@@ -411,12 +412,7 @@
 #pragma clang fp contract(off)
     const int64_t i = (int64_t)blockIdx.x * 256 + threadIdx.x;
     if (i >= total) return;
-    const float tb = t[i / per_batch], a = x0[i], b = x1[i];
-    const float w0 = 1.0f - s * tb;
-    const float p0 = w0 * a, p1 = tb * b;
-    xt[i] = p0 + p1;
-    const float sa = s * a;
-    flow[i] = b - sa;
+    flow_mix_element(x0[i], x1[i], t[i / per_batch], s, xt[i], flow[i]);
 }
 
 __global__ __launch_bounds__(1024) void flow_finish_kernel(const float* __restrict__ raw, const float* __restrict__ flow,
@@ -475,14 +471,13 @@
 
 
 constexpr int kFhRows = 16;
-__global__ __launch_bounds__(256) void flow_head_kernel(const float* __restrict__ y, int64_t ldy, const float* __restrict__ gamma,
-                                                        const float* __restrict__ beta, float eps, const float* __restrict__ W,
-                                                        const float* __restrict__ bias, const float* __restrict__ flow,
-                                                        const float* __restrict__ x0, const uint8_t* __restrict__ mask,
-                                                        float* __restrict__ pred, float* __restrict__ dur,
-                                                        float* __restrict__ part, int L, int nblk) {
+__device__ __forceinline__ void flow_head_rows(const float* __restrict__ y, int64_t ldy, const float* __restrict__ gamma,
+                                               const float* __restrict__ beta, float eps, const float* __restrict__ W,
+                                               const float* __restrict__ bias, const float* __restrict__ flow,
+                                               const float* __restrict__ x0, const uint8_t* __restrict__ mask,
+                                               float* __restrict__ pred, float* __restrict__ dur, float* __restrict__ part,
+                                               int L, int nblk, float* sp) {
 #pragma clang fp contract(off)
-    __shared__ float sp[4][2];
     const int lane = threadIdx.x & 63, wave = threadIdx.x >> 6;
     const int b = blockIdx.y, blk = blockIdx.x;
     const f32x4 g4 = *reinterpret_cast<const f32x4*>(gamma + 4 * lane), b4 = *reinterpret_cast<const f32x4*>(beta + 4 * lane);
@@ -537,20 +532,29 @@
             }
         }
     }
-    if (lane == 0) { sp[wave][0] = num; sp[wave][1] = den; }
+    if (lane == 0) { sp[wave * 2] = num; sp[wave * 2 + 1] = den; }
     __syncthreads();
     if (threadIdx.x == 0) {
         const int64_t o = ((int64_t)b * nblk + blk) * 2;
-        part[o] = (sp[0][0] + sp[1][0]) + (sp[2][0] + sp[3][0]);
-        part[o + 1] = (sp[0][1] + sp[1][1]) + (sp[2][1] + sp[3][1]);
-    }
-}
-__global__ __launch_bounds__(1024) void flow_head_finalize_kernel(const float* __restrict__ part, int nblk, float* __restrict__ ratio,
-                                                                  float* __restrict__ loss, int B) {
-    __shared__ float sratio[1024];
+        part[o] = (sp[0] + sp[2]) + (sp[4] + sp[6]);
+        part[o + 1] = (sp[1] + sp[3]) + (sp[5] + sp[7]);
+    }
+}
+__global__ __launch_bounds__(256) void flow_head_kernel(const float* __restrict__ y, int64_t ldy, const float* __restrict__ gamma,
+                                                        const float* __restrict__ beta, float eps, const float* __restrict__ W,
+                                                        const float* __restrict__ bias, const float* __restrict__ flow,
+                                                        const float* __restrict__ x0, const uint8_t* __restrict__ mask,
+                                                        float* __restrict__ pred, float* __restrict__ dur,
+                                                        float* __restrict__ part, int L, int nblk) {
+    __shared__ float sp[8];
+    flow_head_rows(y, ldy, gamma, beta, eps, W, bias, flow, x0, mask, pred, dur, part, L, nblk, sp);
+}
+template <int kThreads>
+__device__ __forceinline__ void flow_head_finalize(const float* __restrict__ part, int nblk, float* __restrict__ ratio,
+                                                   float* __restrict__ loss, int B, float* sratio) {
     const int tid = threadIdx.x;
     float s = 0.f;
-    for (int b0 = 0; b0 < B; b0 += 1024) {
+    for (int b0 = 0; b0 < B; b0 += kThreads) {
         const int b = b0 + tid;
         if (b < B) {
             float num = 0.f, den = 0.f;
@@ -564,12 +568,45 @@
         }
         __syncthreads();
         if (tid == 0) {
-            const int n = B - b0 < 1024 ? B - b0 : 1024;
+            const int n = B - b0 < kThreads ? B - b0 : kThreads;
             for (int i = 0; i < n; ++i) s += sratio[i];
         }
         __syncthreads();
     }
     if (loss && tid == 0) loss[0] = s / (float)B;
+}
+__global__ __launch_bounds__(1024) void flow_head_finalize_kernel(const float* __restrict__ part, int nblk, float* __restrict__ ratio,
+                                                                  float* __restrict__ loss, int B) {
+    __shared__ float sratio[1024];
+    flow_head_finalize<1024>(part, nblk, ratio, loss, B, sratio);
+}
+__global__ __launch_bounds__(256) void flow_head_fused_kernel(const float* __restrict__ y, int64_t ldy, const float* __restrict__ gamma,
+                                                              const float* __restrict__ beta, float eps, const float* __restrict__ W,
+                                                              const float* __restrict__ bias, const float* __restrict__ flow,
+                                                              const float* __restrict__ x0, const uint8_t* __restrict__ mask,
+                                                              float* __restrict__ pred, float* __restrict__ dur,
+                                                              float* part, int L, int nblk, float* __restrict__ ratio,
+                                                              float* __restrict__ loss, uint32_t* counter) {
+    __shared__ float sp[256];
+    flow_head_rows(y, ldy, gamma, beta, eps, W, bias, flow, x0, mask, pred, dur, part, L, nblk, sp);
+    asm volatile("s_waitcnt vmcnt(0)" ::: "memory");
+    __syncthreads();
+    if (threadIdx.x == 0) {
+        __builtin_amdgcn_fence(__ATOMIC_RELEASE, "agent");
+        asm volatile("s_waitcnt vmcnt(0)" ::: "memory");
+        const uint32_t ticket = __hip_atomic_fetch_add(counter, 1u, __ATOMIC_RELAXED, __HIP_MEMORY_SCOPE_AGENT);
+        const bool last = ticket == gridDim.x * gridDim.y - 1u;
+        if (last) {
+            __builtin_amdgcn_fence(__ATOMIC_ACQUIRE, "agent");
+            asm volatile("s_waitcnt vmcnt(0)" ::: "memory");
+        }
+        sp[8] = last ? 1.0f : 0.0f;
+    }
+    __syncthreads();
+    if (sp[8] == 0.0f) return;
+    __syncthreads();
+    flow_head_finalize<256>(part, nblk, ratio, loss, (int)gridDim.y, sp);
+    if (threadIdx.x == 0) __hip_atomic_store(counter, 0u, __ATOMIC_RELAXED, __HIP_MEMORY_SCOPE_AGENT);
 }
 
 __global__ __launch_bounds__(256) void flow_euler_kernel(const float* __restrict__ xt, const float* __restrict__ vel, float dt,
@@ -832,6 +869,26 @@
     return ispk_launch_status();
 }
 
+extern "C" int32_t ispk_flow_head_fused_f32(const float* y, int64_t ldy, const float* norm_gamma, const float* norm_beta,
+                                            float norm_eps, const float* W, const float* bias, const float* flow, const float* x0,
+                                            const uint8_t* mask, float* pred, float* duration, float* loss_ratio, float* loss_mean,
+                                            float* workspace, uint32_t* counter, int32_t B, int32_t L, int32_t D, int32_t C,
+                                            ispk_stream_t stream) {
+    ISPK_REQUIRE(y && norm_gamma && norm_beta && W && bias && flow && x0 && mask && pred && duration && loss_ratio && workspace &&
+                     counter,
+                 ISPK_E_NULL, "flow_head_fused: null pointer");
+    ISPK_REQUIRE(D == 256 && C == 3, ISPK_E_UNSUPPORTED, "flow_head_fused: built for dim 256 -> 3 flow channels (got %d -> %d)", D, C);
+    ISPK_REQUIRE(B >= 0 && L >= 1 && B <= 65535 && ldy >= D && ldy % 4 == 0, ISPK_E_SHAPE, "flow_head_fused: bad shape B=%d L=%d", B, L);
+    ISPK_REQUIRE(ispk_aligned(y, 16) && ispk_aligned(norm_gamma, 16) && ispk_aligned(norm_beta, 16) && ispk_aligned(W, 16) &&
+                     ispk_aligned(counter, 4),
+                 ISPK_E_ALIGN, "flow_head_fused: y / gamma / beta / W must be 16-byte aligned, counter 4-byte aligned");
+    if (B == 0) return 0;
+    const int nblk = (L + kFhRows - 1) / kFhRows;
+    hipLaunchKernelGGL(flow_head_fused_kernel, dim3(nblk, B), dim3(256), 0, reinterpret_cast<hipStream_t>(stream), y, ldy, norm_gamma,
+                       norm_beta, norm_eps, W, bias, flow, x0, mask, pred, duration, workspace, L, nblk, loss_ratio, loss_mean, counter);
+    return ispk_launch_status();
+}
+
 extern "C" int32_t ispk_flow_euler_f32(const float* x_t, const float* velocity, float dt, const uint8_t* mask, float* out,
                                        int32_t B, int32_t L, int32_t C, ispk_stream_t stream) {
     ISPK_REQUIRE(x_t && velocity && out, ISPK_E_NULL, "flow_euler: null pointer");
diff --git a/isp_tts_amd/csrc/flow_front.h b/isp_tts_amd/csrc/flow_front.h
--- /dev/null
+++ b/isp_tts_amd/csrc/flow_front.h
@@ -0,0 +1,17 @@
+#pragma once
+#include "common.h"
+
+namespace {
+
+__device__ __forceinline__ float flow_duration_target(int64_t dur) { return log1pf((float)dur); }
+
+__device__ __forceinline__ void flow_mix_element(float x0, float x1, float tb, float s, float& xt, float& flow) {
+#pragma clang fp contract(off)
+    const float w0 = 1.0f - s * tb;
+    const float p0 = w0 * x0, p1 = tb * x1;
+    xt = p0 + p1;
+    const float sa = s * x0;
+    flow = x1 - sa;
+}
+
+}
diff --git a/isp_tts_amd/csrc/mas.hip b/isp_tts_amd/csrc/mas.hip
--- a/isp_tts_amd/csrc/mas.hip
+++ b/isp_tts_amd/csrc/mas.hip
@@ -1,6 +1,7 @@
 #include <stdlib.h>
 
 #include "common.h"
+#include "flow_front.h"
 
 namespace {
 
@@ -36,11 +37,21 @@
                  : "scc");
 }
 
-template <int NC>
-__global__ __launch_bounds__(256) void mas_kernel(const float* __restrict__ logits, const int64_t* __restrict__ text_len,
-                                                  const int64_t* __restrict__ mel_len, int16_t* __restrict__ attn_hard,
-                                                  int64_t* __restrict__ dur, int16_t* __restrict__ path_out, int M_max,
-                                                  int L_max, int64_t stride_b, int64_t stride_m) {
+struct FlowFront {
+    const float* feats;
+    const float* x0;
+    const float* t;
+    float s;
+    float* targets;
+    float* xt;
+    float* flow;
+};
+
+template <int NC, bool kFront>
+__device__ __forceinline__ void mas_body(const float* __restrict__ logits, const int64_t* __restrict__ text_len,
+                                         const int64_t* __restrict__ mel_len, int16_t* __restrict__ attn_hard,
+                                         int64_t* __restrict__ dur, int16_t* __restrict__ path_out, int M_max, int L_max,
+                                         int64_t stride_b, int64_t stride_m, const FlowFront& ff) {
     extern __shared__ __attribute__((aligned(16))) char smem[];
     const int nblk = (M_max + kBlk - 1) / kBlk;
     uint32_t* hist = reinterpret_cast<uint32_t*>(smem);
@@ -186,8 +197,47 @@
     if (dur) {
         int64_t* d = dur + (int64_t)b * L_max;
         const int64_t fix = mel_len[b] - (int64_t)n;
-        for (int jx = tid; jx < L_max; jx += 256) d[jx] = cnt[jx] + (jx == 0 ? fix : 0);
-    }
+        for (int jx = tid; jx < L_max; jx += 256) {
+            const int64_t dv = cnt[jx] + (jx == 0 ? fix : 0);
+            d[jx] = dv;
+            if constexpr (kFront) {
+                const int64_t o = ((int64_t)b * L_max + jx) * 3;
+                const float tb = ff.t[b];
+                const float x1[3] = {flow_duration_target(dv), ff.feats[o + 1], ff.feats[o + 2]};
+#pragma unroll
+                for (int c = 0; c < 3; ++c) {
+                    ff.targets[o + c] = x1[c];
+                    flow_mix_element(ff.x0[o + c], x1[c], tb, ff.s, ff.xt[o + c], ff.flow[o + c]);
+                }
+            }
+        }
+    }
+}
+
+template <int NC>
+__global__ __launch_bounds__(256) void mas_kernel(const float* __restrict__ logits, const int64_t* __restrict__ text_len,
+                                                  const int64_t* __restrict__ mel_len, int16_t* __restrict__ attn_hard,
+                                                  int64_t* __restrict__ dur, int16_t* __restrict__ path_out, int M_max,
+                                                  int L_max, int64_t stride_b, int64_t stride_m) {
+    mas_body<NC, false>(logits, text_len, mel_len, attn_hard, dur, path_out, M_max, L_max, stride_b, stride_m, FlowFront{});
+}
+
+template <int NC>
+__global__ __launch_bounds__(256) void mas_kernel_flow_front(const float* __restrict__ logits, const int64_t* __restrict__ text_len,
+                                                             const int64_t* __restrict__ mel_len, int16_t* __restrict__ attn_hard,
+                                                             int64_t* __restrict__ dur, int16_t* __restrict__ path_out, int M_max,
+                                                             int L_max, int64_t stride_b, int64_t stride_m, FlowFront ff) {
+    mas_body<NC, true>(logits, text_len, mel_len, attn_hard, dur, path_out, M_max, L_max, stride_b, stride_m, ff);
+}
+
+template <int NC>
+int32_t launch_front(const float* logits, const int64_t* text_len, const int64_t* mel_len, int16_t* attn_hard, int64_t* dur,
+                     int16_t* path, int B, int M_max, int L_max, int64_t sb, int64_t sm, size_t lds, const FlowFront& ff,
+                     hipStream_t stream) {
+    ISPK_RESERVE_LDS((&mas_kernel_flow_front<NC>), lds, "mas_flow_front");
+    hipLaunchKernelGGL(mas_kernel_flow_front<NC>, dim3(B), dim3(256), lds, stream, logits, text_len, mel_len, attn_hard, dur, path,
+                       M_max, L_max, sb, sm, ff);
+    return ispk_launch_status();
 }
 
 template <int NC>
@@ -235,3 +285,39 @@
 #undef ISPK_MAS_CASE
     ISPK_FAIL(ISPK_E_SHAPE, "mas: unsupported chunk count %d", nc);
 }
+
+extern "C" int32_t ispk_mas_flow_front_f32(const float* logits, const int64_t* text_len, const int64_t* mel_len,
+                                           int16_t* attn_hard, int64_t* dur, int16_t* path, const float* feats, const float* x0,
+                                           const float* t, float sigma, float* targets, float* x_t, float* flow, int32_t B,
+                                           int32_t M_max, int32_t L_max, int64_t stride_b, int64_t stride_m,
+                                           ispk_stream_t stream) {
+    ISPK_REQUIRE(logits && text_len && mel_len && attn_hard && dur && feats && x0 && t && targets && x_t && flow, ISPK_E_NULL,
+                 "mas_flow_front: null pointer argument");
+    ISPK_REQUIRE(B >= 0 && M_max >= 1 && L_max >= 1, ISPK_E_SHAPE, "mas_flow_front: bad shape B=%d M=%d L=%d", B, M_max, L_max);
+    ISPK_REQUIRE(L_max <= 512 && M_max <= 4096, ISPK_E_SHAPE, "mas_flow_front: L_max %d > 512 or M_max %d > 4096", L_max, M_max);
+    ISPK_REQUIRE(stride_m >= L_max && stride_b >= (int64_t)M_max * 1, ISPK_E_SHAPE, "mas_flow_front: bad strides");
+    if (B == 0) return 0;
+    const int nc = (L_max + 63) / 64;
+    const size_t lds = (size_t)((M_max + 31) / 32) * nc * 256 + (((size_t)M_max * 2 + 15) & ~(size_t)15) + (size_t)L_max * 4;
+    ISPK_REQUIRE((int64_t)M_max * stride_m * 4 < ((int64_t)1 << 31), ISPK_E_SHAPE,
+                 "mas_flow_front: one utterance's logits (M_max * stride_m floats) must span less than 2 GiB");
+    ISPK_REQUIRE(lds <= 160 * 1024, ISPK_E_SHAPE, "mas_flow_front: M_max=%d x L_max=%d needs %zu B of LDS (> 160 KiB)", M_max,
+                 L_max, lds);
+    hipStream_t s = reinterpret_cast<hipStream_t>(stream);
+    const FlowFront ff{feats, x0, t, (float)(1.0 - (double)sigma), targets, x_t, flow};
+#define ISPK_MAS_CASE(NC) \
+    case NC:              \
+        return launch_front<NC>(logits, text_len, mel_len, attn_hard, dur, path, B, M_max, L_max, stride_b, stride_m, lds, ff, s);
+    switch (nc) {
+        ISPK_MAS_CASE(1)
+        ISPK_MAS_CASE(2)
+        ISPK_MAS_CASE(3)
+        ISPK_MAS_CASE(4)
+        ISPK_MAS_CASE(5)
+        ISPK_MAS_CASE(6)
+        ISPK_MAS_CASE(7)
+        ISPK_MAS_CASE(8)
+    }
+#undef ISPK_MAS_CASE
+    ISPK_FAIL(ISPK_E_SHAPE, "mas_flow_front: unsupported chunk count %d", nc);
+}
```

Measured after the change: 17.13 million mel-frames/s (median of 4 runs). About the same (+0.6%).
